# steventan0110/DiffNorm

Measured on AMD Instinct MI355X. Metric: denoising-steps/sec (BxT latents), higher is better.
Workload: dtype f16; 1 GPU; configs[2]: DDIM/DDPM-schedule reverse chain, eps-predictor Model(512, z=128) on [B=32,T=512] latents per GPU, 1000-step cosine schedule, random-init weights; batch_per_gpu=32, frames=512, latent_dim=128, hip_graph=True, half_batch_streams=2, parallelism=batch-sharded x1 (no collective)

## Files before the change

### diffnorm_amd/_lib.py

```python
import ctypes as C
import os

_HERE = os.path.dirname(os.path.abspath(__file__))
LIB_PATH = os.path.join(_HERE, "libdiffnorm_hip.so")

DN_F32, DN_BF16, DN_BF16X3, DN_F16 = 0, 1, 2, 3
EPI_BIAS, EPI_SILU, EPI_GEGLU, EPI_FILM_GATE, EPI_RESADD, EPI_POSEMB, EPI_RELU = range(7)
DN_MAX_TERMS = 8
TAG_FFN_CONV, TAG_WN_DILATED, TAG_FFN_CONV_WGRAD = 1, 2, 3
GEMM_NARROW_STORES, GEMM_NO_RES_PREFETCH, GEMM_RELU, GEMM_TWIN = 1 << 4, 1 << 5, 1 << 6, 1 << 7
GEMM_TAG_SHIFT, GEMM_TILE_SHIFT, GEMM_BAND_SHIFT = 8, 16, 24
GEMM_FAT_STAMPS, GEMM_NO_SHARED_ROWS, GEMM_TAPS_INNER, GEMM_TERM_OUTER = 1 << 20, 1 << 21, 1 << 22, 1 << 23
(TILE_128X128, TILE_256X128, TILE_256X256, TILE_256X352, TILE_ROW, TILE_256X256_W4, TILE_256X256_W8, TILE_256X192,
 TILE_256X128_2WG) = range(1, 10)


class DiffNormHipError(RuntimeError):
    pass


LAYOUT_A_KBLOCKED, LAYOUT_W_KBLOCKED, LAYOUT_OUT_KBLOCKED = 1, 2, 1


class GemmTerm(C.Structure):
    _fields_ = [("A", C.c_void_p), ("W", C.c_void_p), ("lda", C.c_int32), ("shift", C.c_int32),
                ("a_gstride", C.c_int64), ("w_gstride", C.c_int64), ("shift_by_group", C.c_int32),
                ("layout", C.c_int32), ("ldw", C.c_int32), ("pad_ldw_", C.c_int32)]


class GemmParams(C.Structure):
    _fields_ = [("terms", GemmTerm * DN_MAX_TERMS), ("n_terms", C.c_int32), ("dtype", C.c_int32),
                ("M", C.c_int32), ("N", C.c_int32), ("K", C.c_int32), ("T", C.c_int32),
                ("groups", C.c_int32), ("epilogue", C.c_int32), ("bias", C.c_void_p),
                ("bias_gstride", C.c_int64), ("out", C.c_void_p), ("ldo", C.c_int32),
                ("out_dtype", C.c_int32), ("out_gstride", C.c_int64), ("res", C.c_void_p),
                ("ldr", C.c_int32), ("res_dtype", C.c_int32), ("res_gstride", C.c_int64),
                ("gamma_beta", C.c_void_p), ("gb_ld", C.c_int32), ("gb_half", C.c_int32),
                ("gb_gstride", C.c_int64), ("pos_table", C.c_void_p), ("pos_ld", C.c_int32),
                ("flags", C.c_int32), ("lengths", C.c_void_p),
                ("norm_out", C.c_void_p), ("norm_ld", C.c_int32), ("norm_dtype", C.c_int32), ("norm_D", C.c_int32),
                ("norm_gb_ld", C.c_int32), ("norm_gamma", C.c_void_p), ("norm_gb", C.c_void_p),
                ("norm_gb_half", C.c_int32), ("out_layout", C.c_int32),
                ("norm_split", C.c_int32), ("norm_ssq_ld", C.c_int32), ("norm_ssq", C.c_void_p),
                ("row_ssq", C.c_void_p), ("row_ssq_ld", C.c_int32), ("row_ssq_parts", C.c_int32),
                ("row_D", C.c_float), ("row_bias_ld", C.c_int32), ("row_bias", C.c_void_p),
                ("pre_out", C.c_void_p), ("pre_ld", C.c_int32), ("pre_pad_", C.c_int32)]
    pad_ = property(lambda self: self.flags, lambda self, v: setattr(self, "flags", v))


class GemmRoute(C.Structure):
    _fields_ = [(n, C.c_int32) for n in ("tile", "taps_inner", "shared_rows", "band")]


class AdamParams(C.Structure):
    _fields_ = [("lr", C.c_double), ("beta1", C.c_double), ("beta2", C.c_double), ("eps", C.c_double),
                ("weight_decay", C.c_double), ("max_norm", C.c_double), ("step", C.c_int32), ("pad_", C.c_int32),
                ("grad_scale", C.c_double), ("grad_scale_dev", C.c_void_p)]


class AttnParams(C.Structure):
    _fields_ = [("q", C.c_void_p), ("k", C.c_void_p), ("v", C.c_void_p), ("out", C.c_void_p),
                ("ldq", C.c_int32), ("ldk", C.c_int32), ("ldv", C.c_int32), ("ldo", C.c_int32),
                ("B", C.c_int32), ("T", C.c_int32), ("heads", C.c_int32), ("dim_head", C.c_int32),
                ("dtype", C.c_int32), ("Tk", C.c_int32), ("lengths", C.c_void_p),
                ("scale", C.c_float), ("pad2_", C.c_int32), ("lse", C.c_void_p),
                ("dropout_p", C.c_float), ("seed_lo", C.c_uint32), ("seed_hi", C.c_uint32), ("pad3_", C.c_int32)]


class AttnBwdParams(C.Structure):
    _fields_ = [(n, C.c_void_p) for n in ("q", "k", "v", "out", "dout", "dq", "dk", "dv")] + \
               [(n, C.c_int32) for n in ("ldq", "ldk", "ldv", "ldo", "lddo", "lddq", "lddk", "lddv", "B", "T", "heads", "dim_head",
                                         "dtype", "pad_")] + \
               [("lengths", C.c_void_p), ("scale", C.c_float), ("pad2_", C.c_int32), ("lse", C.c_void_p), ("delta", C.c_void_p),
                ("dropout_p", C.c_float), ("seed_lo", C.c_uint32), ("seed_hi", C.c_uint32), ("pad3_", C.c_int32)]


class GaussianStep(C.Structure):
    _fields_ = [("x", C.c_void_p), ("model_out", C.c_void_p), ("noise", C.c_void_p), ("sample", C.c_void_p),
                ("pred_xstart", C.c_void_p), ("t", C.c_void_p), ("table", C.c_void_p), ("N", C.c_int32),
                ("inner", C.c_int32), ("learned_range", C.c_int32), ("clip_denoised", C.c_int32), ("sampler", C.c_int32),
                ("eta", C.c_float), ("predict_xstart", C.c_int32), ("cond_grad", C.c_void_p)]


GD_COLS = 12
DDIM_SCHED_COLS = 5
DPM_COLS = 6


class GaussianMoments(C.Structure):
    _fields_ = [(n, C.c_void_p) for n in ("x", "model_out", "x_start", "t", "table", "mean", "variance", "log_variance", "pred_xstart",
                                          "vb", "reverse_sample")] + [(n, C.c_int32) for n in ("N", "inner", "learned_range", "clip_denoised", "predict_xstart")]


class EpsConfig(C.Structure):
    _fields_ = [(n, C.c_int32) for n in ("dim", "latent", "depth", "heads", "dim_head", "wn_layers",
                                         "wn_stacks", "cond_mult", "dtype", "max_pos", "dim_prompt", "num_latents", "resampler_depth")]

# ... 57 lines not shown
                ("label_smoothing", C.c_float), ("loss_scale", C.c_float), ("stats", C.c_void_p), ("logits_out", C.c_void_p),
                ("recon_out", C.c_void_p), ("ext_dlogits", C.c_void_p), ("attn_dropout", C.c_float),
                ("dropout_seed_lo", C.c_uint32), ("dropout_seed_hi", C.c_uint32), ("pad_", C.c_int32)]


class EpsTrainBatch(C.Structure):
    _fields_ = [(n, C.c_void_p) for n in ("feat", "units", "lengths", "z", "jitter", "true_noise", "times", "sqrt_ac", "sqrt_1mac",
                                          "snr_weight")] + \
               [("beta0", C.c_float), ("B", C.c_int32), ("T", C.c_int32), ("n_units", C.c_int32), ("n_frames", C.c_int32),
                ("timesteps", C.c_int32), ("multitask", C.c_int32), ("label_smoothing", C.c_float), ("recon_weight", C.c_float),
                ("loss_scale", C.c_float), ("stats", C.c_void_p), ("eps_out", C.c_void_p), ("attn_dropout", C.c_float),
                ("dropout_seed_lo", C.c_uint32), ("dropout_seed_hi", C.c_uint32), ("pad_", C.c_int32)]


REPACK_CONVERT, REPACK_KBLOCK, REPACK_COPY, REPACK_SUM = range(4)


class RepackDesc(C.Structure):
    _fields_ = [("src", C.c_int64), ("dst", C.c_void_p), ("kind", C.c_int32), ("mats", C.c_int32), ("rows", C.c_int32), ("K", C.c_int32),
                ("count", C.c_int32), ("pad_", C.c_int32), ("stride", C.c_int64)]


_vp, _i32, _i64, _u64, _sz = C.c_void_p, C.c_int32, C.c_int64, C.c_uint64, C.c_size_t
SYMBOLS = {
    "dn_conv_gemm": (C.c_int, [C.POINTER(GemmParams), _vp]),
    "dn_conv_gemm_route": (C.c_int, [C.POINTER(GemmParams), C.POINTER(GemmRoute)]),
    "dn_conv_gemm_kblocked_ok": (C.c_int, [C.POINTER(GemmParams)]),
    "dn_conv_gemm_tile": (C.c_int, [C.POINTER(GemmParams)]),
    "dn_grad_sumsq": (C.c_int, [_vp, C.c_int64, _vp, _vp, C.c_int32, _vp]),
    "dn_transpose_pad": (C.c_int, [_vp, C.c_int32, C.c_int32, C.c_int32, C.c_int32, C.c_int32, C.c_int32, _vp, C.c_int32, C.c_int32,
                                   C.c_int32, C.c_int32, _vp]),
    "dn_adam_step": (C.c_int, [_vp, _vp, _vp, _vp, C.c_int64, C.POINTER(AdamParams), _vp, _vp, _vp]),
    "dn_adam_step_ema": (C.c_int, [_vp, _vp, _vp, _vp, C.c_int64, C.POINTER(AdamParams), _vp, _vp, _vp, C.c_double, _vp]),
    "dn_ema_update": (C.c_int, [_vp, _vp, C.c_int64, C.c_double, _vp]),
    "dn_profile_start": (C.c_int, [_i32, _i32]),
    "dn_profile_stop": (C.c_int, [C.POINTER(C.c_float), C.POINTER(_i32)]),
    "dn_attention": (C.c_int, [C.POINTER(AttnParams), _vp]),
    "dn_attention_backward": (C.c_int, [C.POINTER(AttnBwdParams), _vp]),
    "dn_time_cond_backward": (C.c_int, [_vp, _i32, _vp, _i32, _vp, _vp, _i32, _vp, _i32, _vp, _vp, _vp, _vp, _vp]),
    "dn_gate_forward": (C.c_int, [_vp, _vp, _vp, _i32, _i32, _i32, _i32, _vp, _i32, _i32, _vp]),
    "dn_gate_backward": (C.c_int, [_vp, _vp, _vp, _i32, _i32, _i32, _i32, _vp, _i32, _i32, _vp, _i32, _vp]),
    "dn_geglu_forward": (C.c_int, [_vp, _vp, _i32, _i32, _i32, _vp]),
    "dn_geglu_backward": (C.c_int, [_vp, _vp, _vp, _i32, _i32, _i32, _vp]),
    "dn_rmsnorm_backward_scratch_bytes": (_sz, [_i32, _i32, _i32]),
    "dn_rmsnorm_backward": (C.c_int, [_vp, _i32, _vp, _i32, _i32, _i32, _i32, _i32, _vp, _vp, _i32, _i32, _vp, _vp, _vp, _i32, _i32,
                                      _vp, _vp, _i32, _vp, _vp]),
    "dn_colsum_scratch_bytes": (_sz, [_i32, _i32, _i32]),
    "dn_colsum": (C.c_int, [_vp, _i32, _i32, _i32, _i32, _i32, _vp, _i32, C.c_float, _i32, _vp, _vp]),
    "dn_posterior_backward": (C.c_int, [_vp, _i32, _vp, _i32, _vp, _i32, _vp, _i32, _i32, _i32, _i32, _i32, _vp, C.c_float, _vp]),
    "dn_lsce_loss_grad": (C.c_int, [_vp, _i32, _vp, _i32, _i32, C.c_float, C.c_float, _vp, _vp, _i32, _i32, _vp]),
    "dn_masked_mse_grad": (C.c_int, [_vp, _i32, _vp, _i32, _i32, _i32, _i32, _vp, C.c_float, _vp, _vp, _i32, _i32, _vp, _i32, _i32, _vp]),
    "dn_vec_sum": (C.c_int, [_vp, _i64, _vp, _i32, _vp, _vp]),
    "dn_vae_train_create": (C.c_int, [C.POINTER(VaeConfig), C.POINTER(_vp)]),
    "dn_vae_train_destroy": (None, [_vp]),
    "dn_vae_train_param_count": (_i64, [_vp]),
    "dn_vae_train_aux_bytes": (_sz, [_vp]),
    "dn_vae_train_offsets": (C.c_int, [_vp, C.POINTER(_i64), _i32]),
    "dn_vae_train_stage_range": (C.c_int, [_vp, _i32, C.POINTER(_i64), C.POINTER(_i64)]),
    "dn_vae_train_bind": (C.c_int, [_vp, _vp, _vp, _vp, _vp]),
    "dn_vae_train_refresh": (C.c_int, [_vp, _vp]),
    "dn_vae_train_workspace_bytes": (_sz, [_vp, _i32, _i32]),
    "dn_vae_train_forward": (C.c_int, [_vp, C.POINTER(VaeTrainBatch), _vp, _sz, _vp]),
    "dn_vae_train_backward": (C.c_int, [_vp, C.POINTER(VaeTrainBatch), _i32, _i32, _vp, _sz, _vp]),
    "dn_cmlm_step": (C.c_int, [_vp, _vp, _vp, _vp, _i32, _i32, _i32, _i32, _i32, _i32, _i32, _vp]),
    "dn_eps_train_create": (C.c_int, [C.POINTER(EpsConfig), C.POINTER(_vp)]),
    "dn_eps_train_destroy": (None, [_vp]),
    "dn_eps_train_param_count": (_i64, [_vp]),
    "dn_eps_train_aux_bytes": (_sz, [_vp]),
    "dn_eps_train_offsets": (C.c_int, [_vp, C.POINTER(_i64), _i32]),
    "dn_eps_train_stage_range": (C.c_int, [_vp, _i32, C.POINTER(_i64), C.POINTER(_i64)]),
    "dn_eps_train_bind": (C.c_int, [_vp, _vp, _vp, _vp, _vp, _vp]),
    "dn_eps_train_refresh": (C.c_int, [_vp, _vp]),
    "dn_eps_train_workspace_bytes": (_sz, [_vp, _vp, _i32, _i32]),
    "dn_eps_train_forward": (C.c_int, [_vp, _vp, C.POINTER(EpsTrainBatch), _vp, _sz, _vp]),
    "dn_eps_train_backward": (C.c_int, [_vp, _vp, C.POINTER(EpsTrainBatch), _i32, _i32, _vp, _sz, _vp]),
    "dn_sum_groups": (C.c_int, [_vp, _i64, _i32, _vp, _i32, _i64, _vp]),
    "dn_rows_times_weight_scratch_bytes": (_sz, [_i32, _i32, _i32]),
    "dn_rows_times_weight": (C.c_int, [_vp, _i32, _i32, _vp, _i32, _i32, _i32, _vp, _vp, _vp]),
    "dn_transpose_weights": (C.c_int, [_vp, _i32, _i32, _i64, _i32, _i32, _vp, _i64, _i32, _i32, _vp]),
    "dn_split_rows": (C.c_int, [_vp, _i64, _vp, _i32, _vp]),
    "dn_transpose_slices": (C.c_int, [_vp, _i32, _i32, _i32, _i32, _i32, _i32, _i32, _i64, _i32, _vp, _i32, _i32, _i32, _i32, _vp]),
    "dn_repack_weights": (C.c_int, [_vp, _vp, _i32, _i32, _vp]),
    "dn_ffn_fold": (C.c_int, [_vp, _vp, _vp, _vp, C.c_int64, C.c_int64, C.c_int64, C.c_int64, _i32, _i32, _i32, _i32, _vp, _vp, _vp]),
    "dn_eps_set_ffn_fold": (C.c_int, [_vp, _vp, _vp]),
    "dn_vae_set_ffn_fold": (C.c_int, [_vp, _vp, _vp]),
    "dn_wgrad_reduce": (C.c_int, [_vp, _i32, _i32, _i32, _i32, _i32, _vp, _i32, _i32, _vp]),
    "dn_conv_weight_grad_tn": (C.c_int, [_vp, _i32, _i32, _vp, _vp, _vp, _i32, _i32, _i32, _i32, _i32, _vp, _vp, _vp]),
    "dn_conv_weight_grad_tn_x3": (C.c_int, [_vp, _i32, _i32, _vp, _vp, _vp, _i32, _i32, _i32, _i32, _i32, _vp, _vp, _vp]),
    "dn_add_broadcast": (C.c_int, [_vp, _vp, _i32, _i32, _i32, _vp]),
    "dn_transpose_pad_f32": (C.c_int, [_vp, _i32, _i32, _i32, _i32, _i32, _i32, _vp, _i32, _i32, _i32, _i32, _vp]),
    "dn_rmsnorm": (C.c_int, [_vp, _i32, _vp, _i32, _i32, _i32, _i32, _i32, _vp, _vp, _i32, _i32, _vp]),
    "dn_time_cond": (C.c_int, [_vp, _i32, _vp, _i32, _vp, _vp, _i32, _vp, _vp, _i32, _i32, _vp]),
    "dn_ddim_step": (C.c_int, [_vp, _vp, _vp, _vp, _i32, _i32, _i32, _i32, _i32, _i32, _vp, _vp, _vp]),
    "dn_q_sample": (C.c_int, [_vp, _vp, _vp, _vp, _i32, _i32, _i32, _i32, _i32, _i32, _vp, _vp, _vp, _vp]),
    "dn_gaussian_step": (C.c_int, [C.POINTER(GaussianStep), _vp]),
    "dn_gaussian_moments": (C.c_int, [C.POINTER(GaussianMoments), _vp]),
    "dn_posterior_sample": (C.c_int, [_vp, _i32, _vp, _i32, _vp, _vp, _i32, _i32, _i32, _i32, _i32, _vp, _vp, _vp]),
    "dn_argmax_units": (C.c_int, [_vp, _i32, _i32, _i32, _i32, _vp, _vp]),
    "dn_randn": (C.c_int, [_vp, _i64, _u64, _u64, _vp]),
    "dn_randn_keyed": (C.c_int, [_vp, _vp, _i32, _i32, _i32, C.c_uint32, _vp]),
    "dn_chain_start": (C.c_int, [_vp, _i32, _vp, _i32, _i32, _i32, _vp, _vp, _vp, _vp, _vp, _vp]),
    "dn_convert_rows": (C.c_int, [_vp, _i32, _i32, _vp, _i32, _i32, _i32, _i32, _vp]),
    "dn_eps_create": (C.c_int, [C.POINTER(EpsConfig), C.POINTER(_vp), _i32, C.POINTER(_vp)]),
    "dn_eps_destroy": (None, [_vp]),
    "dn_eps_workspace_bytes": (_sz, [_vp, _i32, _i32]),
    "dn_eps_forward": (C.c_int, [_vp, _vp, _vp, _vp, _i32, _i32, _i32, _vp, _vp, _sz, _vp]),
    "dn_eps_cond_workspace_bytes": (_sz, [_vp, _i32, _i32, _i32]),
    "dn_eps_forward_cond": (C.c_int, [_vp, _vp, _vp, _vp, _vp, _vp, _vp, _i32, _i32, _i32, _vp, _vp, _sz, _vp]),
    "dn_eps_forward_cond_ex": (C.c_int, [_vp, _vp, _vp, _vp, _vp, _vp, _vp, _i32, _i32, _i32, _vp, _vp, _sz, _i32, _vp, _i32, _i32, _vp]),
    "dn_eps_cond_time_table_workspace_bytes": (_sz, [_vp, _i32]),
    "dn_eps_cond_time_table": (C.c_int, [_vp, _i32, _i32, _vp, _vp, _sz, _vp]),
    "dn_eps_cond_time_table_steps": (C.c_int, [_vp, _vp, _i32, _vp, _vp, _sz, _vp]),
    "dn_eps_weights_changed": (C.c_int, [_vp]),
    "dn_vae_create": (C.c_int, [C.POINTER(VaeConfig), C.POINTER(_vp), _i32, C.POINTER(_vp)]),
    "dn_vae_destroy": (None, [_vp]),
    "dn_vae_workspace_bytes": (_sz, [_vp, _i32, _i32]),
    "dn_vae_encode_params": (C.c_int, [_vp, _vp, _i32, _i32, _vp, _vp, _sz, _vp]),
    "dn_vae_decode": (C.c_int, [_vp, _vp, _vp, _i32, _i32, _vp, _vp, _vp, _vp, _sz, _vp]),
    "dn_ddim_workspace_bytes": (_sz, [_vp, _i32, _i32, _i32]),
    "dn_ddim_loop": (C.c_int, [_vp, _vp, _vp, _i32, _i32, _i32, _i32, _vp, _i32, _i32, _vp, _sz, _vp]),
    "dn_ddpm_loop": (C.c_int, [_vp, _vp, _vp, _i32, _i32, _i32, _i32, _vp, _i32, _i32, C.c_uint64, _vp, _i32, _vp, _sz, _vp]),
    "dn_ddim_sched_workspace_bytes": (_sz, [_vp, _i32, _i32, _i32]),
    "dn_ddim_sched_check": (C.c_int, [_vp, _i32, _i32]),
    "dn_ddim_sched_loop": (C.c_int, [_vp, _vp, _vp, _i32, _i32, _vp, _vp, _i32, _i32, _i32, C.c_uint64, _vp, _i32, _vp, _sz, _vp]),
    "dn_dpm2m_step": (C.c_int, [_vp, _vp, _vp, _i64, _vp, _vp, _vp]),
    "dn_ddim_sched_step": (C.c_int, [_vp, _vp, _i64, _vp, _vp, _vp, _i32, C.c_uint64, _vp, _vp]),
    "dn_ddim_sched_step_keyed": (C.c_int, [_vp, _vp, _vp, _i32, _i32, _i32, _vp, _vp, _vp, _vp]),
    "dn_ddim_sched_loop_keyed": (C.c_int, [_vp, _vp, _vp, _i32, _i32, _vp, _vp, _i32, _i32, _vp, _i32, _vp, _sz, _vp]),
    "dn_ddpm_loop_keyed": (C.c_int, [_vp, _vp, _vp, _i32, _i32, _i32, _i32, _vp, _i32, _i32, _vp, _i32, _vp, _sz, _vp]),
    "dn_guided_ddim_loop_keyed": (C.c_int, [_vp, _vp, _vp, _vp, _vp, _i32, _i32, _i32, C.c_float, _vp, _vp, _i32, _i32, _vp, _i32, _vp, _sz,
                                            _vp]),
    "dn_dpm_workspace_bytes": (_sz, [_vp, _i32, _i32, _i32]),
    "dn_dpm_loop": (C.c_int, [_vp, _vp, _vp, _i32, _i32, _vp, _vp, _i32, _i32, _i32, _vp, _sz, _vp]),
    "dn_gaussian_workspace_bytes": (_sz, [_vp, _i32, _i32, _i32]),
    "dn_gaussian_loop": (C.c_int, [_vp, _vp, _vp, _i32, _i32, _vp, _vp, _i32, _i32, _i32, _i32, C.c_float, C.c_uint64, _vp, _i32, _vp, _sz,
                                   _vp]),
    "dn_gaussian_loop_keyed": (C.c_int, [_vp, _vp, _vp, _i32, _i32, _vp, _vp, _i32, _i32, _i32, _i32, C.c_float, _vp, _i32, _vp, _sz, _vp]),
    "dn_gaussian_sched_step": (C.c_int, [_vp, _vp, _i64, _vp, _vp, _i32, _i32, _i32, C.c_float, C.c_uint64, _vp, _vp]),
    "dn_gaussian_sched_step_keyed": (C.c_int, [_vp, _vp, _vp, _i32, _i32, _i32, _vp, _vp, _vp, _i32, _i32, _i32, C.c_float, _vp]),
    "dn_guided_ddim_workspace_bytes": (_sz, [_vp, _i32, _i32, _i32, _i32, _i32]),
    "dn_guided_ddim_loop": (C.c_int, [_vp, _vp, _vp, _vp, _vp, _i32, _i32, _i32, C.c_float, _vp, _vp, _i32, _i32, _i32, C.c_uint64, _vp, _i32,
                                      _vp, _sz, _vp]),
    "dn_guided_dpm_workspace_bytes": (_sz, [_vp, _i32, _i32, _i32, _i32, _i32]),
    "dn_guided_dpm_loop": (C.c_int, [_vp, _vp, _vp, _vp, _vp, _i32, _i32, _i32, C.c_float, _vp, _vp, _i32, _i32, _i32, _vp, _sz, _vp]),
    "dn_cfg_combine": (C.c_int, [_vp, C.c_float, _i64, _vp, _vp]),
    "dn_nar_create": (C.c_int, [C.POINTER(NarConfig), C.POINTER(_vp), _i32, C.POINTER(_vp)]),
    "dn_nar_destroy": (None, [_vp]),
    "dn_nar_workspace_bytes": (_sz, [_vp, _i32, _i32, _i32]),
    "dn_nar_cross_kv_bytes": (_sz, [_vp, _i32, _i32]),
    "dn_nar_cross_kv": (C.c_int, [_vp, _vp, _i32, _i32, _vp, _vp, _sz, _vp]),
    "dn_nar_predict_lengths": (C.c_int, [_vp, _vp, _vp, _i32, _i32, _vp, _vp, _sz, _vp]),
    "dn_nar_decoder_forward": (C.c_int, [_vp, _vp, _vp, _vp, _i32, _i32, _i32, _vp, _vp, _sz, _vp]),
    "dn_nar_encoder_create": (C.c_int, [_vp, _vp, _i32, _vp]),
    "dn_nar_encoder_destroy": (None, [_vp]),
    "dn_nar_encoder_out_frames": (_i32, [_i32]),
    "dn_nar_encoder_workspace_bytes": (_sz, [_vp, _i32, _i32]),
    "dn_nar_encoder_forward": (C.c_int, [_vp, _vp, _vp, _i32, _i32, _vp, _vp, _vp, _sz, _vp]),
    "dn_rel_attention": (C.c_int, [C.POINTER(RelAttnParams), _vp]),
    "dn_glu_dwconv": (C.c_int, [_vp, _vp, _vp, _vp, _i32, _i32, _i32, _i32, _i32, _vp]),
    "dn_conformer_encoder_create": (C.c_int, [_vp, _vp, _i32, _vp]),
    "dn_conformer_encoder_destroy": (None, [_vp]),
    "dn_conformer_encoder_workspace_bytes": (_sz, [_vp, _i32, _i32]),
    "dn_conformer_encoder_forward": (C.c_int, [_vp, _vp, _vp, _i32, _i32, _vp, _vp, _vp, _sz, _vp]),
    "dn_last_error": (C.c_char_p, []),
    "dn_version": (C.c_int, []),
    "dn_cmlm_step_dev": (C.c_int, [_vp, _vp, _vp, _vp, _i32, _i32, _i32, _vp, _i32, _i32, _i32, _vp]),
    "dn_nar_null_cross_bytes": (_sz, [_vp]),
    "dn_nar_null_cross": (C.c_int, [_vp, _i32, _vp, _sz, _vp]),
# ... 102 lines not shown
```

### diffnorm_amd/csrc/engine.h

```cpp
#pragma once
#include <stddef.h>
#include <stdint.h>
#include <string.h>

#include "../../include/diffnorm_hip.h"

namespace dn {

inline int round_up(int x, int m) { return (x + m - 1) / m * m; }
inline int padk(int c) { return round_up(c, 64); }
inline int padn(int c) { return round_up(c, 128); }

inline const void* eoff(const void* p, size_t elems, int es) { return static_cast<const char*>(p) + elems * es; }
inline void* eoff(void* p, size_t elems, int es) { return static_cast<char*>(p) + elems * es; }
inline int esize(int dtype) { return dtype == DN_BF16 || dtype == DN_F16 ? 2 : 4; }
inline int side_dtype(int dtype) { return dtype == DN_BF16X3 ? DN_F32 : dtype; }
inline int ew_grid(int64_t n) {
  const int64_t b = (n + 255) / 256;
  return (int)(b > 4096 ? 4096 : b);
}

#define DN_TRY(expr)          \
  do {                        \
    int rc__ = (expr);        \
    if (rc__ != DN_OK) return rc__; \
  } while (0)

inline DnGemmParams gemm_base(int dtype, int M, int N, int K, int T, int32_t flags = 0) {
  DnGemmParams p;
  memset(&p, 0, sizeof(p));
  p.flags = flags;
  p.dtype = dtype;
  p.M = M; p.N = N; p.K = K; p.T = T;
  p.groups = 1;
  p.n_terms = 1;
  p.epilogue = DN_EPI_BIAS;
  p.out_dtype = dtype;
  p.res_dtype = dtype == DN_BF16X3 ? DN_F32 : dtype;
  return p;
}

struct Arena {
  char* base;
  size_t off, cap;
  void* take(size_t bytes) {
    size_t a = (off + 255) & ~size_t(255);
    off = a + bytes;
    if (!base) return reinterpret_cast<void*>(a + 256);
    return off <= cap ? base + a : nullptr;
  }
};

struct WavenetW {
  int cin, cout, stacks, layers;
  const void *init_W, *conv_W, *res_W, *skip_W, *final_W, *conv_Wkb, *res_Wkb;
  const float *init_b, *conv_b, *res_b, *skip_b, *final_b;
};
constexpr int kWavenetTensors = 12;

struct TransformerW {
  int dim, depth, heads, dim_head, inner;
  const void *qkv_W, *out_W, *ffin_W, *ffconv_W, *ffout_W, *pred_W, *ffconv_Wkb, *ffin_Wkb, *qkv_Wkb;
  const float *ffin_b, *ffconv_b, *ffout_b, *g1, *g2, *pred_gamma;
  const void* fold_W;
  const float* fold_b;
  int fold_default;
};
constexpr int kTransformerTensors = 15;

struct WgTnGroups {
  int groups;
  int64_t dy_gstride, x_gstride, grad_gstride;
  int shift_by_group;
};
int wgrad_tn_launch(const void* dy, int lddy, int cout, const void* const* x, const int* ldx, const int* shift, int n_taps, int cin, int B, int T,
                    int slices, float* part, float* grad, void* stream, int tag, const WgTnGroups* grp);
constexpr int WGRAD_TN_X3_DEFAULT = 1;
int wgrad_tn_x3_launch(const void* dy, int lddy, int cout, const void* const* x, const int* ldx, const int* shift, int n_taps, int cin, int B, int T,
                       int slices, float* part, float* grad, void* stream, int tag, const WgTnGroups* grp);

struct StepKey {
  const void *ws, *x, *len, *coef;
  const void *prompt, *plen;
  const void* keys;
  uint64_t seed;
  int32_t B, T, Tp, n_steps;
  int32_t flags;
  int32_t opt_gen;
  uint32_t scale_bits;
  uint32_t eta_bits;
  uint16_t ancestral, clip, scheduled, eta, dpm;
  uint16_t generic;
  uint16_t injected;
  uint16_t reserved;
};
static_assert(sizeof(StepKey) == 7 * sizeof(void*) + 8 + 8 * 4 + 8 * 2, "StepKey has no padding: copies of a key compare equal too");
struct StepGraph {
  void* exec;
  StepKey key;
};

struct SchedNoise {
  const float* noise;
  int64_t noise_row;
  uint64_t seed;
  const uint64_t* keys;
  int64_t row_quads;
};
inline SchedNoise sched_noise(const float* noise, int64_t noise_row, uint64_t seed, const uint64_t* keys, int64_t row_quads) {
  return keys ? SchedNoise{nullptr, 0, 0, keys, row_quads} : SchedNoise{noise, noise_row, seed, nullptr, 0};
}
enum SchedRule { SCHED_DDIM, SCHED_DPM2M, SCHED_GAUSSIAN };
struct SchedStep {
  int rule;
  float* x;
  int64_t elem0, n_elem;
  const float* eps;
  int guided;
  float scale;
  float* xin;
  const float* coef;
  const int32_t *steps, *counter;
  int eta_on;
  float* hist;
  int n_steps, sampler, clip;
  float eta;
  SchedNoise src;
};
int sched_step_launch(const char* who, const SchedStep& d, void* stream);

}

int dn_ddpm_step_launch(float* x, const float* eps, int M, int C, int T, const float* table, const int32_t* t, int clip, const float* noise,
                        int64_t noise_row, int t_top, uint64_t seed, const uint64_t* keys, int b0, void* stream);
int dn_gaussian_sched_args(const char* who, int32_t n_steps, int32_t sampler, float eta);

struct DnEps {
  DnEpsConfig cfg;
  const float *w_freq, *tc_W, *tc_b, *cond_b, *init_b, *final_b, *pos_table;
  const void *cond_W, *init_W, *final_W;
  dn::WavenetW wn;
  dn::TransformerW tf;
  int n_cond;
  int n_row;
  const float *tpc_W, *tpc_b, *null_pc, *lat_pos, *rffin_b, *rffout_b, *rnorm_g, *proj_b;
  const void *null_tok, *proj_W, *rq_W, *rkv_W, *rout_W, *rffin_W, *rffout_W, *cq_W, *ckv_W, *cout_W;
  dn::StepGraph loop_graph, guided_graph;
// ... 16 lines not shown
```

### diffnorm_amd/csrc/engine.hip

```cpp
#include <algorithm>
#include <functional>
#include <new>
#include <stdlib.h>
#include <string.h>

#include "common.h"
#include "engine.h"

using namespace dn;

namespace {

inline bool fuse_norm_enabled(int Dp, int dtype) {
  const bool on = option_or(OPT_FUSE_NORM, 0) != 0;
  return on && Dp <= 512 && dtype != DN_BF16X3;
}

inline bool split_norm_enabled(int Dp, int dtype) {
  return option_or(OPT_NO_SPLIT_NORM, 0) == 0 && Dp % 64 == 0 && !fuse_norm_enabled(Dp, dtype);
}

int kblock_mode() {
  const int v = option(OPT_KBLOCK);
  return v == DN_OPT_UNSET ? -1 : (v != 0 ? 1 : 0);
// ... 14 lines not shown

int run_wavenet(const WavenetW& w, int dtype, const void* in, int M, int T, const float* gb, int gb_ld, const WaveBufs& wb,
                DnGemmParams fin, hipStream_t s, int32_t gemm_flags = 0) {
  const int es = esize(dtype);
  const int cinp = padk(w.cin), cp = padk(w.cout), cn = padn(w.cout), L = w.layers, S = w.stacks;
  const size_t mat = (size_t)cn * cp;
  const int64_t plane = (int64_t)M * cp;
  bool kb = false;
  if (kblock_mode() != 0 && dn::dn_is16(dtype) && w.conv_Wkb && w.res_Wkb) {
    DnGemmParams q = gemm_base(dtype, M, cp, cp, T, gemm_flags);
    q.groups = L;
    const int t_res = dn_conv_gemm_tile(&q);
    q.n_terms = 3; q.epilogue = DN_EPI_FILM_GATE;
    kb = kblock_mode() == 1 || (t_res == DN_TILE_256X256 && dn_conv_gemm_tile(&q) == DN_TILE_256X256);
  }
  const int a_layout = kb ? (DN_LAYOUT_A_KBLOCKED | DN_LAYOUT_W_KBLOCKED) : 0;
  {
    DnGemmParams p = gemm_base(dtype, M, cp, cinp, T, gemm_flags);
    p.n_terms = 3;
    for (int j = 0; j < 3; ++j) {
      p.terms[j].A = in; p.terms[j].lda = cinp; p.terms[j].shift = 2 - j;
      p.terms[j].W = eoff(w.init_W, (size_t)j * cn * cinp, es);
    }
    p.bias = w.init_b; p.out = wb.hw; p.ldo = cp;
    p.out_layout = kb ? DN_LAYOUT_OUT_KBLOCKED : 0;
    DN_TRY(dn_conv_gemm(&p, s));
  }
  for (int st = 0; st < S; ++st) {
    const void* in_s = st == 0 ? wb.hw : ((st - 1) & 1 ? wb.blk1 : wb.blk0);
    const int64_t a_gs = st == 0 ? 0 : plane;
    void* out_s = (st & 1) ? wb.blk1 : wb.blk0;
    {
      DnGemmParams p = gemm_base(dtype, M, cp, cp, T, gemm_flags);
      p.groups = L;
      p.terms[0].A = in_s; p.terms[0].lda = cp; p.terms[0].a_gstride = a_gs;
      p.terms[0].W = eoff(kb ? w.res_Wkb : w.res_W, (size_t)st * L * mat, es); p.terms[0].w_gstride = (int64_t)mat;
      p.terms[0].layout = a_layout;
      p.bias = w.res_b + (size_t)st * L * cp; p.bias_gstride = cp;
      p.out = wb.resb; p.ldo = cp; p.out_gstride = plane; p.out_dtype = side_dtype(dtype);
      DN_TRY(dn_conv_gemm(&p, s));
    }
    {
      DnGemmParams p = gemm_base(dtype, M, cp, cp, T, gemm_flags);
      p.groups = L;
      p.n_terms = 3;
      for (int j = 0; j < 3; ++j) {
        p.terms[j].A = in_s; p.terms[j].lda = cp; p.terms[j].a_gstride = a_gs;
        p.terms[j].shift = 2 - j; p.terms[j].shift_by_group = 1;
        p.terms[j].W = eoff(kb ? w.conv_Wkb : w.conv_W, ((size_t)st * L * 3 + j) * mat, es); p.terms[j].w_gstride = (int64_t)(3 * mat);
        p.terms[j].layout = a_layout;
      }
      p.bias = w.conv_b + (size_t)st * L * cp; p.bias_gstride = cp;
      p.epilogue = DN_EPI_FILM_GATE;
      p.res = wb.resb; p.ldr = cp; p.res_gstride = plane; p.res_dtype = side_dtype(dtype);
      if (gb) {
        p.gamma_beta = gb + (size_t)st * L * 2 * cp; p.gb_ld = gb_ld; p.gb_half = cp; p.gb_gstride = 2 * cp;
      }
      p.out = out_s; p.ldo = cp; p.out_gstride = plane;
      p.out_layout = kb && st + 1 < S ? DN_LAYOUT_OUT_KBLOCKED : 0;
      p.flags |= DN_TAG_WN_DILATED << DN_GEMM_TAG_SHIFT;
      DN_TRY(dn_conv_gemm(&p, s));
    }
  }
  const void* last = ((S - 1) & 1) ? wb.blk1 : wb.blk0;
  {
    DnGemmParams p = gemm_base(dtype, M, cp, cp, T, gemm_flags);
    p.n_terms = L;
    for (int i = 0; i < L; ++i) {
      p.terms[i].A = eoff(last, (size_t)i * plane, es); p.terms[i].lda = cp;
      p.terms[i].W = eoff(w.skip_W, (size_t)i * mat, es);
    }
    p.bias = w.skip_b; p.out = wb.sk; p.ldo = cp;
    DN_TRY(dn_conv_gemm(&p, s));
  }
  fin.dtype = dtype; fin.M = M; fin.K = cp; fin.T = T; fin.groups = 1; fin.n_terms = 1; fin.flags |= gemm_flags;
  fin.terms[0].A = wb.sk; fin.terms[0].lda = cp; fin.terms[0].W = w.final_W;
  fin.bias = w.final_b;
  return dn_conv_gemm(&fin, s);
}

struct TfBufs { void *xn, *qkv, *ao, *gg, *fc; float* ssq; };
inline int ssq_ld(int Dp) { const int n = Dp / 64; return n <= 8 ? 8 : (n + 3) / 4 * 4; }

inline int ffn_fold_mode(const TransformerW& w) { return w.fold_W && w.fold_b ? option_or(OPT_FFN_FOLD, w.fold_default) : 0; }

TfBufs plan_tf(const TransformerW& w, int M, int es, Arena& ar) {
  const int hd = w.heads * w.dim_head;
  TfBufs b;
  b.xn = ar.take((size_t)M * padk(w.dim) * es);
  b.qkv = ar.take((size_t)M * 3 * hd * es);
  b.ao = ar.take((size_t)M * hd * es);
  b.gg = ar.take((size_t)M * padk(w.inner) * es);
  b.fc = ffn_fold_mode(w) ? nullptr : ar.take((size_t)M * padk(w.inner) * es);
  b.ssq = (float*)ar.take((size_t)M * ssq_ld(padk(w.dim)) * 4);
  return b;
}

void set_split_norm(DnGemmParams& p, const TfBufs& tb, int Dp, int D, int dtype, const float* gamma, const float* gb, int gb_ld) {
  p.norm_out = tb.xn; p.norm_ld = Dp; p.norm_dtype = dtype; p.norm_D = D;
  p.norm_gamma = gamma; p.norm_gb = gb; p.norm_gb_ld = gb_ld; p.norm_gb_half = Dp;
  p.norm_split = 1; p.norm_ssq = tb.ssq; p.norm_ssq_ld = ssq_ld(Dp);
}
void set_row_scale(DnGemmParams& p, const TfBufs& tb, int Dp, int D, const float* rb, int rb_ld) {
  p.row_ssq = tb.ssq; p.row_ssq_ld = ssq_ld(Dp); p.row_ssq_parts = Dp / 64; p.row_D = (float)D;
  p.row_bias = rb; p.row_bias_ld = rb_ld;
}

void set_norm(DnGemmParams& p, void* xn, int Dp, int D, int dtype, const float* gamma, const float* gb, int gb_ld) {
  p.norm_out = xn; p.norm_ld = Dp; p.norm_dtype = dtype; p.norm_D = D;
  p.norm_gamma = gamma; p.norm_gb = gb; p.norm_gb_ld = gb_ld; p.norm_gb_half = Dp;
}

struct NormSrc { const float* gamma; const float* gb; };
NormSrc norm_src(const TransformerW& w, const float* gb, int l, int j, int nj = 2) {
  const int D = w.dim, Dp = padk(D);
  if (l == w.depth) return {w.pred_gamma, nullptr};
  const float* g = j == 0 ? w.g1 : w.g2;
  return {g ? g + (size_t)l * D : nullptr, gb ? gb + (size_t)(nj * l + j) * 2 * Dp : nullptr};
}

struct CrossAttn { const void* q_W; const void* out_W; const void* kv; int n_kv; void* q; };

int run_transformer(const TransformerW& w, int dtype, float* xres, int B, int T, const int32_t* lengths, const float* gb, int gb_ld,
                    const float* rb, int rb_ld, const TfBufs& tb, void* pred, int pred_ld, int pred_dtype, bool xn_ready, hipStream_t s,
                    const CrossAttn* cx = nullptr, int32_t gemm_flags = 0) {
  const int es = esize(dtype), M = B * T;
  const int D = w.dim, Dp = padk(D), Dn = padn(D), hd = w.heads * w.dim_head, ip = padk(w.inner), in_n = padn(w.inner);
  const bool fuse = fuse_norm_enabled(Dp, dtype);
  const bool split = split_norm_enabled(Dp, dtype);
  const int nj = cx ? 3 : 2, rb_layer = 3 * hd + (cx ? hd : 0) + 2 * ip;
  bool scaled = split && xn_ready;
  auto standalone_norm = [&](int l, int j) -> int {
    const NormSrc ns = norm_src(w, gb, l, j, nj);
    return dn_rmsnorm(xres, Dp, tb.xn, Dp, dtype, M, D, T, ns.gamma, ns.gb, gb_ld, Dp, s);
  };
  if (!((fuse || split) && xn_ready)) DN_TRY(standalone_norm(0, 0));
  const int mid2 = dn::dn_is16(dtype) && M >= 2048 ? option_or(OPT_MID2, 0) : 0;
  bool geglu_kb = false;
  static const bool geglu_kb_off = getenv("DN_GEGLU_KB") && atoi(getenv("DN_GEGLU_KB")) == 0;
  if (!geglu_kb_off && split && !fuse && kblock_mode() != 0 && dn::dn_is16(dtype) && w.ffin_Wkb && Dp % 32 == 0) {
    DnGemmParams q = gemm_base(dtype, M, ip, Dp, T, gemm_flags);
    q.epilogue = DN_EPI_GEGLU;
    if (mid2 & 2) q.flags |= DN_TILE_256X128_2WG << DN_GEMM_TILE_SHIFT;
    const int gt = dn_conv_gemm_tile(&q);
    geglu_kb = kblock_mode() == 1 || gt == DN_TILE_256X256 || gt == DN_TILE_256X128_2WG;
  }
  bool qkv_kb = false;
  static const bool qkv_kb_off = getenv("DN_QKV_KB") && atoi(getenv("DN_QKV_KB")) == 0;
  if (!qkv_kb_off && split && !fuse && kblock_mode() != 0 && dn::dn_is16(dtype) && w.qkv_Wkb && Dp % 32 == 0) {
    DnGemmParams q = gemm_base(dtype, M, 3 * hd, Dp, T, gemm_flags);
    if (mid2 & 1) q.flags |= DN_TILE_256X128_2WG << DN_GEMM_TILE_SHIFT;
    const int qt = dn_conv_gemm_tile(&q);
    qkv_kb = kblock_mode() == 1 || qt == DN_TILE_256X256 || qt == DN_TILE_256X128_2WG;
  }
  const int fold = ffn_fold_mode(w);
  const bool qkv_192 = option_or(OPT_QKV_192, 0) != 0 && dn::dn_is16(dtype) && (3 * hd) % 192 == 0 && M >= 2048;
  for (int l = 0; l < w.depth; ++l) {
    {
      DnGemmParams p = gemm_base(dtype, M, 3 * hd, Dp, T, gemm_flags);
      p.terms[0].A = tb.xn; p.terms[0].lda = Dp; p.terms[0].W = eoff(w.qkv_W, (size_t)l * padn(3 * hd) * Dp, es);
      if (qkv_kb && l >= 1) {
        p.terms[0].W = eoff(w.qkv_Wkb, (size_t)l * padn(3 * hd) * Dp, es);
        p.terms[0].layout = DN_LAYOUT_A_KBLOCKED | DN_LAYOUT_W_KBLOCKED;
      }
      p.out = tb.qkv; p.ldo = 3 * hd; p.out_dtype = side_dtype(dtype);
      if (qkv_192) p.flags |= DN_TILE_256X192 << DN_GEMM_TILE_SHIFT;
      else if (mid2 & 1) p.flags |= DN_TILE_256X128_2WG << DN_GEMM_TILE_SHIFT;
      if (scaled) set_row_scale(p, tb, Dp, D, rb ? rb + (size_t)l * rb_layer : nullptr, rb_ld);
      DN_TRY(dn_conv_gemm(&p, s));
    }
    {
      DnAttnParams a;
      memset(&a, 0, sizeof(a));
      a.q = tb.qkv; a.k = eoff(tb.qkv, hd, es); a.v = eoff(tb.qkv, 2 * hd, es); a.out = tb.ao;
      a.ldq = a.ldk = a.ldv = 3 * hd; a.ldo = hd;
      a.B = B; a.T = T; a.heads = w.heads; a.dim_head = w.dim_head; a.dtype = dtype; a.lengths = lengths;
      a.scale = 1.0f / sqrtf((float)w.dim_head);
      DN_TRY(dn_attention(&a, s));
    }
    {
      DnGemmParams p = gemm_base(dtype, M, Dp, hd, T, gemm_flags);
      p.terms[0].A = tb.ao; p.terms[0].lda = hd; p.terms[0].W = eoff(w.out_W, (size_t)l * Dn * hd, es);
      p.epilogue = DN_EPI_RESADD; p.res = xres; p.ldr = Dp; p.out = xres; p.ldo = Dp; p.out_dtype = DN_F32;
      const NormSrc ns = norm_src(w, gb, l, 1, nj);
      if (fuse) set_norm(p, tb.xn, Dp, D, dtype, ns.gamma, ns.gb, gb_ld);
      else if (split) set_split_norm(p, tb, Dp, D, dtype, ns.gamma, ns.gb, gb_ld);
      if (geglu_kb && !cx) p.norm_split = 2;
      DN_TRY(dn_conv_gemm(&p, s));
    }
    if (!fuse && !split) DN_TRY(standalone_norm(l, 1));
    scaled = split;
    if (cx) {
      {
        DnGemmParams p = gemm_base(dtype, M, hd, Dp, T, gemm_flags);
        p.terms[0].A = tb.xn; p.terms[0].lda = Dp; p.terms[0].W = eoff(cx->q_W, (size_t)l * padn(hd) * Dp, es);
        p.out = cx->q; p.ldo = hd; p.out_dtype = side_dtype(dtype);
        if (scaled) set_row_scale(p, tb, Dp, D, rb ? rb + (size_t)l * rb_layer + 3 * hd : nullptr, rb_ld);
        DN_TRY(dn_conv_gemm(&p, s));
      }
      {
        const void* kv = eoff(cx->kv, (size_t)l * B * cx->n_kv * 2 * hd, esize(side_dtype(dtype)));
        DnAttnParams a;
        memset(&a, 0, sizeof(a));
        a.q = cx->q; a.k = kv; a.v = eoff(kv, hd, esize(side_dtype(dtype))); a.out = tb.ao;
        a.ldq = hd; a.ldk = a.ldv = 2 * hd; a.ldo = hd;
        a.B = B; a.T = T; a.Tk = cx->n_kv; a.heads = w.heads; a.dim_head = w.dim_head; a.dtype = dtype; a.lengths = nullptr;
        a.scale = 1.0f / sqrtf((float)w.dim_head);
        DN_TRY(dn_attention(&a, s));
      }
      {
        DnGemmParams p = gemm_base(dtype, M, Dp, hd, T, gemm_flags);
        p.terms[0].A = tb.ao; p.terms[0].lda = hd; p.terms[0].W = eoff(cx->out_W, (size_t)l * Dn * hd, es);
        p.epilogue = DN_EPI_RESADD; p.res = xres; p.ldr = Dp; p.out = xres; p.ldo = Dp; p.out_dtype = DN_F32;
        const NormSrc ns = norm_src(w, gb, l, 2, nj);
        if (fuse) set_norm(p, tb.xn, Dp, D, dtype, ns.gamma, ns.gb, gb_ld);
        else if (split) set_split_norm(p, tb, Dp, D, dtype, ns.gamma, ns.gb, gb_ld);
        if (geglu_kb) p.norm_split = 2;
        DN_TRY(dn_conv_gemm(&p, s));
      }
      if (!fuse && !split) DN_TRY(standalone_norm(l, 2));
    }
    auto close_residual = [&](DnGemmParams& p) -> int {
      p.epilogue = DN_EPI_RESADD; p.res = xres; p.ldr = Dp; p.out = xres; p.ldo = Dp; p.out_dtype = DN_F32;
      const NormSrc ns = norm_src(w, gb, l + 1, 0, nj);
      if (fuse) set_norm(p, tb.xn, Dp, D, dtype, ns.gamma, ns.gb, gb_ld);
      else if (split) set_split_norm(p, tb, Dp, D, dtype, ns.gamma, ns.gb, gb_ld);
      if (qkv_kb && l + 1 < w.depth) p.norm_split = 2;
      return dn_conv_gemm(&p, s);
    };
    if (fold) {
      {
        DnGemmParams p = gemm_base(dtype, M, ip, Dp, T, gemm_flags);
        p.terms[0].A = tb.xn; p.terms[0].lda = Dp; p.terms[0].W = eoff(w.ffin_W, (size_t)l * 2 * ip * Dp, es);
        if (geglu_kb) {
          p.terms[0].W = eoff(w.ffin_Wkb, (size_t)l * 2 * ip * Dp, es);
          p.terms[0].layout = DN_LAYOUT_A_KBLOCKED | DN_LAYOUT_W_KBLOCKED;
        }
        p.bias = w.ffin_b + (size_t)l * 2 * ip;
        p.epilogue = DN_EPI_GEGLU; p.out = tb.gg; p.ldo = ip;
        if (mid2 & 2) p.flags |= DN_TILE_256X128_2WG << DN_GEMM_TILE_SHIFT;
        if (scaled) set_row_scale(p, tb, Dp, D, rb ? rb + (size_t)l * rb_layer + 3 * hd + (cx ? hd : 0) : nullptr, rb_ld);
        DN_TRY(dn_conv_gemm(&p, s));
      }
      DnGemmParams p = gemm_base(dtype, M, Dp, ip, T, gemm_flags);
      p.n_terms = 3;
      for (int j = 0; j < 3; ++j) {
        p.terms[j].A = tb.gg; p.terms[j].lda = ip; p.terms[j].shift = 2 - j;
        p.terms[j].W = eoff(w.fold_W, ((size_t)l * 3 + j) * Dn * ip, es);
      }
      p.bias = w.fold_b + (size_t)l * Dp;
      p.flags |= DN_TAG_FFN_CONV << DN_GEMM_TAG_SHIFT;
      const int fold_tile = fold == 2 ? DN_TILE_256X128 : fold == 3 ? DN_TILE_256X256 : 0;
      if (fold_tile && !fuse) p.flags |= fold_tile << DN_GEMM_TILE_SHIFT;
      DN_TRY(close_residual(p));
    } else {
    DnGemmParams pc = gemm_base(dtype, M, ip, ip, T, gemm_flags);
    pc.n_terms = 3;
    for (int j = 0; j < 3; ++j) {
      pc.terms[j].A = tb.gg; pc.terms[j].lda = ip; pc.terms[j].shift = 2 - j;
      pc.terms[j].W = eoff(w.ffconv_W, ((size_t)l * 3 + j) * in_n * ip, es);
    }
    pc.bias = w.ffconv_b + (size_t)l * ip; pc.out = tb.fc; pc.ldo = ip;
    pc.flags |= DN_TAG_FFN_CONV << DN_GEMM_TAG_SHIFT;
    const int conv_tile = dn_conv_gemm_tile(&pc);
    const bool kblocked = kblock_mode() != 0 && dn::dn_is16(dtype) && w.ffconv_Wkb &&
                          (kblock_mode() == 1 || conv_tile == DN_TILE_256X352 || conv_tile == DN_TILE_256X256);
    if (kblocked)
      for (int j = 0; j < 3; ++j) {
        pc.terms[j].W = eoff(w.ffconv_Wkb, ((size_t)l * 3 + j) * in_n * ip, es);
        pc.terms[j].layout = DN_LAYOUT_A_KBLOCKED | DN_LAYOUT_W_KBLOCKED;
      }
    {
      DnGemmParams p = gemm_base(dtype, M, ip, Dp, T, gemm_flags);
      p.terms[0].A = tb.xn; p.terms[0].lda = Dp; p.terms[0].W = eoff(w.ffin_W, (size_t)l * 2 * ip * Dp, es);
      if (geglu_kb) {
        p.terms[0].W = eoff(w.ffin_Wkb, (size_t)l * 2 * ip * Dp, es);
        p.terms[0].layout = DN_LAYOUT_A_KBLOCKED | DN_LAYOUT_W_KBLOCKED;
      }
      p.bias = w.ffin_b + (size_t)l * 2 * ip;
      p.epilogue = DN_EPI_GEGLU; p.out = tb.gg; p.ldo = ip;
      if (mid2 & 2) p.flags |= DN_TILE_256X128_2WG << DN_GEMM_TILE_SHIFT;
      p.out_layout = kblocked ? DN_LAYOUT_OUT_KBLOCKED : 0;
      if (scaled) set_row_scale(p, tb, Dp, D, rb ? rb + (size_t)l * rb_layer + 3 * hd + (cx ? hd : 0) : nullptr, rb_ld);
      DN_TRY(dn_conv_gemm(&p, s));
    }
    DN_TRY(dn_conv_gemm(&pc, s));
    {
      DnGemmParams p = gemm_base(dtype, M, Dp, ip, T, gemm_flags);
      p.terms[0].A = tb.fc; p.terms[0].lda = ip; p.terms[0].W = eoff(w.ffout_W, (size_t)l * Dn * ip, es);
      p.bias = w.ffout_b + (size_t)l * Dp;
      DN_TRY(close_residual(p));
    }
    }
    if (!fuse && !split) DN_TRY(standalone_norm(l + 1, 0));
  }
  DnGemmParams p = gemm_base(dtype, M, Dp, Dp, T, gemm_flags);
  p.terms[0].A = tb.xn; p.terms[0].lda = Dp; p.terms[0].W = w.pred_W;
  p.out = pred; p.ldo = pred_ld; p.out_dtype = pred_dtype;
  if (pred_ld < Dp) p.N = pred_ld;
  if (split) set_row_scale(p, tb, Dp, D, nullptr, 0);
  return dn_conv_gemm(&p, s);
}

const void* const* take_wavenet(WavenetW& w, const void* const* t) {
  w.init_W = t[0]; w.init_b = (const float*)t[1]; w.conv_W = t[2]; w.conv_b = (const float*)t[3];
  w.res_W = t[4]; w.res_b = (const float*)t[5]; w.skip_W = t[6]; w.skip_b = (const float*)t[7];
  w.final_W = t[8]; w.final_b = (const float*)t[9];
  w.conv_Wkb = t[10]; w.res_Wkb = t[11];
  return t + kWavenetTensors;
}

const void* const* take_transformer(TransformerW& w, const void* const* t) {
  w.qkv_W = t[0]; w.out_W = t[1]; w.ffin_W = t[2]; w.ffin_b = (const float*)t[3]; w.ffconv_W = t[4];
  w.ffconv_b = (const float*)t[5]; w.ffout_W = t[6]; w.ffout_b = (const float*)t[7];
  w.g1 = (const float*)t[8]; w.g2 = (const float*)t[9]; w.pred_gamma = (const float*)t[10]; w.pred_W = t[11];
  w.ffconv_Wkb = t[12]; w.ffin_Wkb = t[13]; w.qkv_Wkb = t[14];
  return t + kTransformerTensors;
}

int check_dims(const char* who, int dtype, int dim, int heads, int dim_head, int layers) {
  DN_CHECK_ARG(dtype == DN_F32 || dtype == DN_BF16 || dtype == DN_BF16X3 || dtype == DN_F16, "%s: bad dtype %d", who, dtype);
  DN_CHECK_ARG(dim > 0 && dim % 4 == 0, "%s: dim=%d must be a positive multiple of 4", who, dim);
  DN_CHECK_ARG((heads * dim_head) % 64 == 0, "%s: heads*dim_head=%d must be a multiple of 64", who, heads * dim_head);
  DN_CHECK_ARG(layers >= 1 && layers <= DN_MAX_TERMS, "%s: wavenet layers=%d must be in 1..%d", who, layers, DN_MAX_TERMS);
  return DN_OK;
}

struct EpsBufs {
  float *cond, *gb, *xres;
  void *xin, *h0, *tp, *gbh;
  WaveBufs wv;
  TfBufs tf;
};

EpsBufs plan_eps(const DnEps* m, int B, int T, int Bt, Arena& ar) {
  const int es = esize(m->cfg.dtype), M = B * T;
  const int C = m->cfg.dim * m->cfg.cond_mult, Dp = padk(m->cfg.dim), zp = padk(m->cfg.latent);
  EpsBufs b;
  b.cond = (float*)ar.take((size_t)Bt * C * 4);
  b.gb = (float*)ar.take((size_t)Bt * m->n_row * 4);
  b.gbh = m->cfg.dtype == DN_F32 ? nullptr : ar.take((size_t)Bt * m->n_cond * es);
  b.xin = ar.take((size_t)M * zp * es);
  b.h0 = ar.take((size_t)M * Dp * es);
  b.wv = plan_wave(m->wn, M, es, ar);
  b.xres = (float*)ar.take((size_t)M * Dp * 4);
  b.tf = plan_tf(m->tf, M, es, ar);
  b.tp = ar.take((size_t)M * Dp * es);
  return b;
}

__global__ void fill_t_kernel(int32_t* t, int n, const int32_t* counter) {
  const int i = blockIdx.x * 256 + threadIdx.x;
  if (i < n) t[i] = *counter;
}
__global__ void set_counter_kernel(int32_t* counter, int v) { *counter = v; }
__global__ void dec_counter_kernel(int32_t* counter) { *counter -= 1; }
__global__ void inc_counter_kernel(int32_t* counter) { *counter += 1; }

}

extern "C" int dn_eps_create(const DnEpsConfig* cfg, const void* const* weights, int32_t n_weights, DnEps** out) {
  DN_CHECK_ARG(cfg && weights && out, "dn_eps_create: null argument");
  const bool cond_model = cfg->dim_prompt > 0;
  const int expect_tensors = kEpsTensors + (cond_model ? kEpsCondTensors : 0);
  DN_CHECK_ARG(n_weights == expect_tensors, "dn_eps_create: expected %d packed tensors, got %d", expect_tensors, n_weights);
  DN_CHECK_ARG(!cond_model || (cfg->dim_prompt % 4 == 0 && cfg->num_latents >= 1 && cfg->resampler_depth >= 1),
               "dn_eps_create: conditional model needs dim_prompt %% 4 == 0, num_latents >= 1, resampler_depth >= 1");
  DN_TRY(check_dims("dn_eps_create", cfg->dtype, cfg->dim, cfg->heads, cfg->dim_head, cfg->wn_layers));
  DN_CHECK_ARG(cfg->dim % 2 == 0 && (cfg->dim * cfg->cond_mult) % 64 == 0, "dn_eps_create: dim*cond_mult must be a multiple of 64");
  DN_CHECK_ARG(cfg->latent % 4 == 0 && cfg->latent > 0, "dn_eps_create: latent=%d must be a multiple of 4", cfg->latent);
  for (int i = 0; i < n_weights; ++i) DN_CHECK_ARG(weights[i] != nullptr, "dn_eps_create: packed tensor %d is null", i);
  DnEps* m = new (std::nothrow) DnEps();
  DN_CHECK_ARG(m != nullptr, "dn_eps_create: out of host memory");
  memset(m, 0, sizeof(*m));
  m->cfg = *cfg;
  const void* const* t = weights;
  m->w_freq = (const float*)t[0]; m->tc_W = (const float*)t[1]; m->tc_b = (const float*)t[2];
  m->cond_W = t[3]; m->cond_b = (const float*)t[4]; m->init_W = t[5]; m->init_b = (const float*)t[6];
  t += 7;
  m->wn.cin = m->wn.cout = cfg->dim; m->wn.stacks = cfg->wn_stacks; m->wn.layers = cfg->wn_layers;
  t = take_wavenet(m->wn, t);
  m->tf.dim = cfg->dim; m->tf.depth = cfg->depth; m->tf.heads = cfg->heads; m->tf.dim_head = cfg->dim_head;
  m->tf.inner = (int)((double)cfg->dim * 4 * 2 / 3);
  t = take_transformer(m->tf, t);
  m->tf.g1 = m->tf.g2 = nullptr;
  m->final_W = t[0]; m->final_b = (const float*)t[1]; m->pos_table = (const float*)t[2];
  m->n_cond = (cfg->wn_stacks * cfg->wn_layers + (cond_model ? 3 : 2) * cfg->depth) * 2 * padk(cfg->dim);
  m->n_row = m->n_cond + cfg->depth * (3 * cfg->heads * cfg->dim_head + 2 * padk(m->tf.inner));
  if (cond_model) {
    const void* const* c = t + 3;
    m->tpc_W = (const float*)c[0]; m->tpc_b = (const float*)c[1]; m->null_pc = (const float*)c[2]; m->null_tok = c[3];
    m->proj_W = c[4]; m->proj_b = (const float*)c[5]; m->lat_pos = (const float*)c[6];
    m->rq_W = c[7]; m->rkv_W = c[8]; m->rout_W = c[9]; m->rffin_W = c[10]; m->rffin_b = (const float*)c[11];
    m->rffout_W = c[12]; m->rffout_b = (const float*)c[13]; m->rnorm_g = (const float*)c[14];
    m->cq_W = c[15]; m->ckv_W = c[16]; m->cout_W = c[17];
  }
  *out = m;
  return DN_OK;
}

extern "C" int dn_eps_set_ffn_fold(DnEps* m, const void* fold_W, const float* fold_b) {
  DN_CHECK_ARG(m && (fold_W != nullptr) == (fold_b != nullptr), "dn_eps_set_ffn_fold: null engine, or one of the two buffers without the other");
  DN_CHECK_ARG(((uintptr_t)fold_W & 127) == 0 && ((uintptr_t)fold_b & 15) == 0, "dn_eps_set_ffn_fold: fold_W 128-byte, fold_b 16-byte aligned");
  m->tf.fold_W = fold_W; m->tf.fold_b = fold_b;
  m->tf.fold_default = m->cfg.dtype == DN_BF16 ? 0 : 1;
  for (StepGraph* g : {&m->loop_graph, &m->guided_graph}) {
    if (g->exec) (void)hipGraphExecDestroy((hipGraphExec_t)g->exec);
    g->exec = nullptr;
  }
  m->table_ws = nullptr;
  return DN_OK;
}

extern "C" void dn_eps_destroy(DnEps* m) {
  if (!m) return;
  for (StepGraph* g : {&m->loop_graph, &m->guided_graph})
    if (g->exec) (void)hipGraphExecDestroy((hipGraphExec_t)g->exec);
  if (m->ev_fork) (void)hipEventDestroy((hipEvent_t)m->ev_fork);
  if (m->ev_join) (void)hipEventDestroy((hipEvent_t)m->ev_join);
  if (m->side_stream) (void)hipStreamDestroy((hipStream_t)m->side_stream);
  delete m;
}

static size_t eps_ws_core(const DnEps* m, int B, int T) {
  Arena ar{nullptr, 0, 0};
  (void)plan_eps(m, B, T, B, ar);
  return ar.off + 256;
}

extern "C" size_t dn_eps_workspace_bytes(const DnEps* m, int32_t B, int32_t T) {
  if (!m || B <= 0 || T <= 0) return 0;
  return eps_ws_core(m, B, T);
}

namespace {

int eps_beta_rows(const DnEps* m, const float* gb, int gb_ld, int n, void* gbh, float* rb, int rb_ld, hipStream_t s) {
  const int Dp = padk(m->cfg.dim), dtype = m->cfg.dtype, es = esize(dtype);
  const TransformerW& w = m->tf;
  const bool cx = m->cfg.dim_prompt > 0;
  const int hd = w.heads * w.dim_head, ip = padk(w.inner), nj = cx ? 3 : 2, rb_layer = 3 * hd + (cx ? hd : 0) + 2 * ip;
  const size_t tf_off = (size_t)m->cfg.wn_stacks * m->cfg.wn_layers * 2 * Dp;
  const void* A = gb;
  int lda = gb_ld;
  if (dtype != DN_F32) {
    DN_TRY(dn_convert_rows(gb, DN_F32, gb_ld, gbh, dtype, m->n_cond, n, m->n_cond, s));
    A = gbh; lda = m->n_cond;
  }
  int col = 0;
  for (int j = 0; j < nj; ++j) {
    const bool last = j == nj - 1;
    const int N = j == 0 ? 3 * hd : (last ? 2 * ip : hd);
    DnGemmParams q = gemm_base(dtype, n, N, Dp, 1);
    q.groups = w.depth;
    q.terms[0].A = eoff(A, tf_off + (size_t)j * 2 * Dp + Dp, es); q.terms[0].lda = lda; q.terms[0].a_gstride = (int64_t)nj * 2 * Dp;
    q.terms[0].W = j == 0 ? w.qkv_W : (last ? w.ffin_W : m->cq_W);
    q.terms[0].w_gstride = j == 0 ? (int64_t)padn(3 * hd) * Dp : (last ? (int64_t)2 * ip * Dp : (int64_t)padn(hd) * Dp);
    q.out = rb + col; q.ldo = rb_ld; q.out_dtype = DN_F32; q.out_gstride = rb_layer;
    DN_TRY(dn_conv_gemm(&q, s));
    col += N;
  }
  return DN_OK;
}

int eps_cond_rows(const DnEps* m, const int32_t* times, int n, float* cond, float* gb, void* gbh, hipStream_t s) {
  const int D = m->cfg.dim, C = D * m->cfg.cond_mult, Dp = padk(D), dtype = m->cfg.dtype, es = esize(dtype);
  DN_TRY(dn_time_cond(times, n, m->w_freq, D / 2, m->tc_W, m->tc_b, C, cond, nullptr, DN_F32, C, s));
  DnGemmParams p = gemm_base(DN_F32, n, m->n_cond, C, 1);
  p.terms[0].A = cond; p.terms[0].lda = C; p.terms[0].W = m->cond_W;
  p.bias = m->cond_b; p.out = gb; p.ldo = m->n_row; p.out_dtype = DN_F32;
  DN_TRY(dn_conv_gemm(&p, s));
  if (!split_norm_enabled(Dp, dtype)) return DN_OK;
  return eps_beta_rows(m, gb, m->n_row, n, gbh, gb + m->n_cond, m->n_row, s);
}

int eps_core(const DnEps* m, const float* x, const float* gb, int gb_ld, const int32_t* lengths, int B, int T, float* eps_out,
             const EpsBufs& b, hipStream_t s, int32_t gemm_flags = 0) {
  const DnEpsConfig& c = m->cfg;
  const int dtype = c.dtype, M = B * T;
  const int D = c.dim, Dp = padk(D), z = c.latent, zp = padk(z);
  DN_TRY(dn_convert_rows(x, DN_F32, z, b.xin, dtype, zp, M, z, s));
  {
    DnGemmParams p = gemm_base(dtype, M, Dp, zp, T, gemm_flags);
    p.terms[0].A = b.xin; p.terms[0].lda = zp; p.terms[0].W = m->init_W;
    p.bias = m->init_b; p.out = b.h0; p.ldo = Dp;
    DN_TRY(dn_conv_gemm(&p, s));
  }
  {
    DnGemmParams fin = gemm_base(dtype, M, Dp, Dp, T, gemm_flags);
    fin.epilogue = DN_EPI_POSEMB; fin.pos_table = m->pos_table; fin.pos_ld = Dp; fin.lengths = lengths;
    fin.out = b.xres; fin.ldo = Dp; fin.out_dtype = DN_F32;
    const float* gb0 = gb + (size_t)c.wn_stacks * c.wn_layers * 2 * Dp;
    if (fuse_norm_enabled(Dp, dtype)) set_norm(fin, b.tf.xn, Dp, D, dtype, nullptr, gb0, gb_ld);
// ... 867 lines not shown
  };
  return guided_loop(m, x, lengths, prompt, prompt_lengths, B, T, Tp, cond_scale, steps, coef, n_steps, timesteps, flags, workspace,
                     workspace_bytes, stream, d);
}

extern "C" int dn_guided_ddim_loop(DnEps* m, float* x, const int32_t* lengths, const float* prompt, const int32_t* prompt_lengths, int32_t B,
                                   int32_t T, int32_t Tp, float cond_scale, const int32_t* steps, const float* coef, int32_t n_steps,
                                   int32_t timesteps, int32_t eta_on, uint64_t seed, const float* noise, int32_t flags, void* workspace,
                                   size_t workspace_bytes, void* stream) {
  return guided_ddim_loop("dn_guided_ddim_loop", m, x, lengths, prompt, prompt_lengths, B, T, Tp, cond_scale, steps, coef, n_steps, timesteps,
                          eta_on, seed, noise, nullptr, flags, workspace, workspace_bytes, stream);
}

extern "C" int dn_guided_ddim_loop_keyed(DnEps* m, float* x, const int32_t* lengths, const float* prompt, const int32_t* prompt_lengths,
                                         int32_t B, int32_t T, int32_t Tp, float cond_scale, const int32_t* steps, const float* coef,
                                         int32_t n_steps, int32_t timesteps, const uint64_t* keys, int32_t flags, void* workspace,
                                         size_t workspace_bytes, void* stream) {
  DN_TRY(check_keys("dn_guided_ddim_loop_keyed", m, keys));
  return guided_ddim_loop("dn_guided_ddim_loop_keyed", m, x, lengths, prompt, prompt_lengths, B, T, Tp, cond_scale, steps, coef, n_steps,
                          timesteps, 1, 0, nullptr, keys, flags, workspace, workspace_bytes, stream);
}

extern "C" size_t dn_guided_dpm_workspace_bytes(const DnEps* m, int32_t B, int32_t T, int32_t Tp, int32_t n_steps, int32_t guided) {
  return guided_ws_bytes(m, B, T, Tp, n_steps, guided, true, DN_DPM_COLS);
}

extern "C" int dn_guided_dpm_loop(DnEps* m, float* x, const int32_t* lengths, const float* prompt, const int32_t* prompt_lengths, int32_t B,
                                  int32_t T, int32_t Tp, float cond_scale, const int32_t* steps, const float* coef, int32_t n_steps,
                                  int32_t timesteps, int32_t flags, void* workspace, size_t workspace_bytes, void* stream) {
  GuidedDesc d = {"dn_guided_dpm_loop", "dn_guided_dpm_workspace_bytes", "dn_dpm_loop", DN_DPM_COLS, true, step_kind(0, nullptr), nullptr};
  d.kind.dpm = 1;
  d.update = [](const GuidedBufs& g, float* xb, float* xin, int64_t n_elem, int guided, float scale, hipStream_t st) {
    SchedStep u = {SCHED_DPM2M, xb, 0, n_elem, g.both, guided, scale, xin};
    u.coef = g.coef; u.counter = g.counter; u.hist = g.hist;
    return sched_step_launch("dn_guided_dpm_loop", u, st);
  };
  return guided_loop(m, x, lengths, prompt, prompt_lengths, B, T, Tp, cond_scale, steps, coef, n_steps, timesteps, flags, workspace,
                     workspace_bytes, stream, d);
}

extern "C" int dn_vae_create(const DnVaeConfig* cfg, const void* const* weights, int32_t n_weights, DnVae** out) {
  DN_CHECK_ARG(cfg && weights && out, "dn_vae_create: null argument");
  DN_CHECK_ARG(cfg->n_mults >= 1 && cfg->n_mults <= 4, "dn_vae_create: n_mults=%d", cfg->n_mults);
  const int expect = 2 * cfg->n_mults * kWavenetTensors + kTransformerTensors + 2;
  DN_CHECK_ARG(n_weights == expect, "dn_vae_create: expected %d packed tensors, got %d", expect, n_weights);
  DN_TRY(check_dims("dn_vae_create", cfg->dtype, cfg->dim, cfg->heads, cfg->dim_head, cfg->layers));
  DN_CHECK_ARG(cfg->vocab % 4 == 0 && cfg->z % 4 == 0, "dn_vae_create: vocab and z must be multiples of 4");
  for (int i = 0; i < n_weights; ++i) DN_CHECK_ARG(weights[i] != nullptr, "dn_vae_create: packed tensor %d is null", i);
  DnVae* m = new (std::nothrow) DnVae();
  DN_CHECK_ARG(m != nullptr, "dn_vae_create: out of host memory");
  memset(m, 0, sizeof(*m));
  m->cfg = *cfg;
  m->n_wave = cfg->n_mults;
  const void* const* t = weights;
  int cur = cfg->dim;
  for (int n = 0; n < m->n_wave; ++n) {
    WavenetW& w = m->enc[n];
    w.cin = cur; w.cout = cur / cfg->mults[n]; w.stacks = cfg->stacks; w.layers = cfg->layers;
    cur = w.cout;
    t = take_wavenet(w, t);
  }
  DN_CHECK_ARG(cur == 2 * cfg->z, "dn_vae_create: encoder width %d != 2*z (%d)", cur, 2 * cfg->z);
  for (int n = 0; n < m->n_wave; ++n) {
    WavenetW& w = m->dec[n];
    const int mult = cfg->mults[m->n_wave - 1 - n];
    w.cout = cur * mult; w.cin = n == 0 ? cur / 2 : cur; w.stacks = cfg->stacks; w.layers = cfg->layers;
    cur = w.cout;
    t = take_wavenet(w, t);
  }
  DN_CHECK_ARG(cur == cfg->dim, "dn_vae_create: decoder width %d != dim %d", cur, cfg->dim);
  m->tf.dim = cfg->dim; m->tf.depth = cfg->depth; m->tf.heads = cfg->heads; m->tf.dim_head = cfg->dim_head;
  m->tf.inner = (int)((double)cfg->dim * 4 * 2 / 3);
  t = take_transformer(m->tf, t);
  m->lm_W = t[0]; m->lm_b = (const float*)t[1];
  *out = m;
  return DN_OK;
}

extern "C" void dn_vae_destroy(DnVae* m) { delete m; }

extern "C" int dn_vae_set_ffn_fold(DnVae* m, const void* fold_W, const float* fold_b) {
  DN_CHECK_ARG(m && (fold_W != nullptr) == (fold_b != nullptr), "dn_vae_set_ffn_fold: null engine, or one of the two buffers without the other");
  DN_CHECK_ARG(((uintptr_t)fold_W & 127) == 0 && ((uintptr_t)fold_b & 15) == 0, "dn_vae_set_ffn_fold: fold_W 128-byte, fold_b 16-byte aligned");
  m->tf.fold_W = fold_W; m->tf.fold_b = fold_b;
  m->tf.fold_default = m->cfg.dtype == DN_BF16 ? 0 : 1;
  return DN_OK;
}

namespace {
struct VaeBufs {
  void *in_act, *mid[2];
  WaveBufs wv[4];
  float *xres, *recon, *logits;
  void* pred_act;
  TfBufs tf;
};

VaeBufs plan_vae_enc(const DnVae* m, int M, Arena& ar) {
  const int es = esize(m->cfg.dtype);
  VaeBufs b;
  memset(&b, 0, sizeof(b));
  b.in_act = ar.take((size_t)M * padk(m->cfg.dim) * es);
  int widest = 0;
  for (int n = 0; n < m->n_wave; ++n) widest = widest > m->enc[n].cout ? widest : m->enc[n].cout;
  b.mid[0] = ar.take((size_t)M * padk(widest) * es);
  b.mid[1] = ar.take((size_t)M * padk(widest) * es);
  for (int n = 0; n < m->n_wave; ++n) b.wv[n] = plan_wave(m->enc[n], M, es, ar);
  return b;
}

VaeBufs plan_vae_dec(const DnVae* m, int M, bool need_recon, bool need_logits, Arena& ar) {
  const int es = esize(m->cfg.dtype), Dp = padk(m->cfg.dim);
  VaeBufs b;
  memset(&b, 0, sizeof(b));
  b.in_act = ar.take((size_t)M * padk(m->cfg.z) * es);
  b.mid[0] = ar.take((size_t)M * Dp * es);
  b.mid[1] = ar.take((size_t)M * Dp * es);
  for (int n = 0; n < m->n_wave; ++n) b.wv[n] = plan_wave(m->dec[n], M, es, ar);
  b.xres = (float*)ar.take((size_t)M * Dp * 4);
  b.tf = plan_tf(m->tf, M, es, ar);
  b.recon = need_recon ? (float*)ar.take((size_t)M * Dp * 4) : nullptr;
  b.pred_act = ar.take((size_t)M * Dp * es);
  b.logits = need_logits ? (float*)ar.take((size_t)M * m->cfg.vocab * 4) : nullptr;
  return b;
}
}

extern "C" size_t dn_vae_workspace_bytes(const DnVae* m, int32_t B, int32_t T) {
  if (!m || B <= 0 || T <= 0) return 0;
  Arena a{nullptr, 0, 0}, d{nullptr, 0, 0};
  (void)plan_vae_enc(m, B * T, a);
  (void)plan_vae_dec(m, B * T, true, true, d);
  return (a.off > d.off ? a.off : d.off) + 256;
}

extern "C" int dn_vae_encode_params(DnVae* m, const float* feat, int32_t B, int32_t T, float* params, void* workspace,
                                    size_t workspace_bytes, void* stream) {
  DN_CHECK_ARG(m && feat && params && workspace && B > 0 && T > 0, "dn_vae_encode_params: bad argument");
  DN_CHECK_ARG(((uintptr_t)workspace & 255) == 0, "dn_vae_encode_params: workspace must be 256-byte aligned");
  hipStream_t s = (hipStream_t)stream;
  const int dtype = m->cfg.dtype, M = B * T;
  Arena ar{(char*)workspace, 0, workspace_bytes};
  VaeBufs b = plan_vae_enc(m, M, ar);
  if (ar.off > workspace_bytes) {
    dn_set_error("dn_vae_encode_params: workspace %zu < required %zu", workspace_bytes, ar.off);
    return DN_EWORKSPACE;
  }
  DN_TRY(dn_convert_rows(feat, DN_F32, m->cfg.dim, b.in_act, dtype, padk(m->cfg.dim), M, m->cfg.dim, s));
  const void* cur = b.in_act;
  for (int n = 0; n < m->n_wave; ++n) {
    const WavenetW& w = m->enc[n];
    const bool lastw = n == m->n_wave - 1;
    DnGemmParams fin = gemm_base(dtype, M, lastw ? w.cout : padk(w.cout), padk(w.cout), T);
    if (lastw) {
      fin.out = params; fin.ldo = w.cout; fin.out_dtype = DN_F32;
    } else {
      fin.out = b.mid[n & 1]; fin.ldo = padk(w.cout); fin.out_dtype = dtype;
    }
    DN_TRY(run_wavenet(w, dtype, cur, M, T, nullptr, 0, b.wv[n], fin, s));
    cur = b.mid[n & 1];
  }
  return DN_OK;
}

extern "C" int dn_vae_decode(DnVae* m, const float* latent, const int32_t* lengths, int32_t B, int32_t T, float* recon, float* logits,
                             int32_t* units, void* workspace, size_t workspace_bytes, void* stream) {
  DN_CHECK_ARG(m && latent && lengths && workspace && B > 0 && T > 0, "dn_vae_decode: bad argument");
  DN_CHECK_ARG(((uintptr_t)workspace & 255) == 0, "dn_vae_decode: workspace must be 256-byte aligned");
// ... 39 lines not shown
```

### diffnorm_amd/csrc/gemm_kernels.h

```cpp
#include <math.h>
#include <stdlib.h>

#include <type_traits>

#pragma once
#include "common.h"

#ifndef DN_GEMM_ABL
#define DN_GEMM_ABL 0
#endif

namespace dn {

static __device__ uint4 g_zero_page[8];

constexpr int BN = 128, ROWB = 128;
constexpr int W_TILE_BYTES = BN * ROWB;

typedef const __attribute__((address_space(1))) void* gptr_t;
typedef __attribute__((address_space(3))) void* lptr_t;

__device__ __forceinline__ void glds16(const void* src, uint32_t lds_addr) {
  uint32_t keep;
  asm volatile(
// ... 609 lines not shown
  auto mma_all = [&]() {
    if constexpr (std::is_same<E, BF16X3>::value) {
#pragma unroll
      for (int pass = 0; pass < 3; ++pass)
#pragma unroll
        for (int nt = 0; nt < 4; ++nt)
#pragma unroll
          for (int mt = 0; mt < 4; ++mt)
            mma_kstep<BF16>(acc[nt][mt], wf[pass == 0 ? 0 : 1][nt], af[pass == 1 ? 1 : 0][mt]);
    } else {
#pragma unroll
      for (int ks = 0; ks < 2; ++ks)
#pragma unroll
        for (int nt = 0; nt < 4; ++nt)
#pragma unroll
          for (int mt = 0; mt < 4; ++mt) mma_kstep<E>(acc[nt][mt], wf[ks][nt], af[ks][mt]);
    }
  };

  const RowSsqReq rs_req = row_scale_request<EPI>(p, m0 + wm * 64, lane);
  setup_term(0);
  if constexpr (STAGES == 3) {
    const bool late = __builtin_amdgcn_readfirstlane(wave) >= NWAVES / 2;
    stage(0);
    if (nkt > 1) stage(1);
    if (nkt > 1) pipe_sync<PER_STAGE>(); else pipe_sync<0>();
    __builtin_amdgcn_sched_barrier(0);
    if (late) pipe_sync<63>();
    auto ktile = [&](auto late_c, auto stage_c, int slot, int fill) {
      constexpr bool LATE = decltype(late_c)::value, STAGE = decltype(stage_c)::value;
      if constexpr (!(DN_GEMM_ABL & 4)) load_frags(slot);
      if constexpr (STAGE && !(DN_GEMM_ABL & 1)) stage(fill);
      if constexpr (LATE) pipe_sync<STAGE ? PER_STAGE : 0>(); else pipe_sync<63>();
      __builtin_amdgcn_sched_barrier(0);
      if constexpr (!(DN_GEMM_ABL & 8)) __builtin_amdgcn_s_setprio(1);
      if constexpr (!(DN_GEMM_ABL & 2)) mma_all();
      __builtin_amdgcn_s_setprio(0);
      __builtin_amdgcn_sched_barrier(0);
      if constexpr (LATE) pipe_sync<63>(); else pipe_sync<STAGE ? PER_STAGE : 0>();
      __builtin_amdgcn_sched_barrier(0);
    };
    auto run = [&](auto late_c) {
      int slot = 0, fill = 2, kt = 0;
      auto adv = [&]() { slot = slot == 2 ? 0 : slot + 1; fill = fill == 2 ? 0 : fill + 1; };
      for (; kt + 2 < nkt; ++kt) { ktile(late_c, std::true_type{}, slot, fill); adv(); }
      for (; kt < nkt; ++kt) { ktile(late_c, std::false_type{}, slot, fill); adv(); }
    };
    if (late) run(std::true_type{}); else run(std::false_type{});
    if (!late) pipe_sync<63>();
  } else {
    stage(0);
    int slot = 0;
    for (int kt = 0; kt < nkt; ++kt) {
      pipe_sync<0>();
      if (kt + 1 < nkt) stage(slot ^ 1);
      load_frags(slot);
      mma_all();
      slot ^= 1;
    }
  }

  if constexpr (STAGES != 3) __syncthreads();
  float* ep = reinterpret_cast<float*>(smem) + wave * (64 * EP_LD);
  const float row_scale = row_scale_finish(p, rs_req);
  float sc4[4];
  slab_row_scales(row_scale, lane, sc4);
#pragma unroll
  for (int mt = 0; mt < 4; ++mt)
#pragma unroll
    for (int nt = 0; nt < 4; ++nt)
      *reinterpret_cast<f32x4*>(ep + (mt * 16 + frow) * EP_LD + nt * 16 + fq * 4) = scaled(acc[nt][mt], sc4[mt]);
  asm volatile("s_waitcnt lgkmcnt(0)" ::: "memory");

  if constexpr (EPI == DN_EPI_RESADD)
    wave_epilogue<EPI, std::is_same<E, BF16X3>::value, std::is_same<E, F16>::value>(p, ep, m0 + wm * 64, n0 + wn * 64, g, lane, 64, row_scale >= 0.f ? ROW_PRESCALED : row_scale, pre_res);
  else
    wave_epilogue<EPI, std::is_same<E, BF16X3>::value, std::is_same<E, F16>::value>(p, ep, m0 + wm * 64, n0 + wn * 64, g, lane, 64, row_scale >= 0.f ? ROW_PRESCALED : row_scale);
}

constexpr int ROWB2 = 64;

template <typename E, int EPI, bool TAPS, int BNB = 256, bool HALO = false>
__global__ __launch_bounds__(512, 1) void conv_gemm_big_kernel(const DnGemmParams p) {
  static_assert(!HALO || (TAPS && BNB == 256 && !std::is_same<E, BF16X3>::value), "shared staging: tap-inner order on the 256 x 256 tile");
  extern __shared__ __attribute__((aligned(16))) char smem[];
  if constexpr (std::is_same<E, F16>::value) f16_saturate();
  constexpr int ES = Elem<E>::bytes;
  constexpr int KT = ROWB2 / ES;
  static_assert(BNB == 256 || BNB == 192, "tile width");
  constexpr int BMB = 256, STAGES = 4;
  constexpr int TILE = BNB * ROWB2;
  constexpr int STAGE_BYTES = TILE + 256 * ROWB2;
  constexpr int PER_STAGE = 4;
  constexpr int PER_LATE = BNB == 256 ? 4 : 3;
  constexpr int NTW = BNB / 32;

  const int tid = threadIdx.x;
  const int lane = tid & 63;
  const int wave = __builtin_amdgcn_readfirstlane(tid >> 6);
  const int wm = wave >> 1, wn = wave & 1;
  const int g = blockIdx.y;
  const int np_total = p.N * (EPI == DN_EPI_GEGLU ? 2 : 1);
  const int n_tiles_n = (np_total + BNB - 1) / BNB;
  int logical;
  {
    const int nwg = gridDim.x, bid = blockIdx.x;
    const int xcd = bid & 7, q = nwg >> 3, r = nwg & 7;
    logical = (xcd < r ? xcd * (q + 1) : r * (q + 1) + (xcd - r) * q) + (bid >> 3);
  }
  int mt_, nt_;
  tile_coords(logical, n_tiles_n, (p.M + BMB - 1) / BMB, (p.flags >> DN_GEMM_BAND_SHIFT) & 0xff, mt_, nt_);
  const int m0 = mt_ * BMB;
  const int n0 = nt_ * BNB;
  const int w_rows = (np_total + 127) / 128 * 128;

  const int srow = lane >> 2;
  const int schunk = (lane & 3) ^ (((lane >> 5) & 1) << 1);
  int a_row[2], a_t[2], w_row[2];
#pragma unroll
  for (int i = 0; i < 2; ++i) {
    int m = m0 + wave * 32 + i * 16 + srow;
    m = m < p.M ? m : p.M - 1;
    a_row[i] = m;
    a_t[i] = m % p.T;
    int n = n0 + (BNB == 256 || wave < 4 ? wave * 32 + i * 16 : 128 + (wave - 4) * 16) + srow;
    w_row[i] = n < w_rows ? n : w_rows - 1;
  }
  const int ktiles_per_term = p.K / KT;
  const int nkt = p.n_terms * ktiles_per_term;
  const char* zero_src = reinterpret_cast<const char*>(g_zero_page) + schunk * 16;
  const char* a_ptr[2];
  const char* w_ptr[2];
  int a_inc[2], w_inc = ROWB2;
  int s_term = 0, s_kk = 0;
  auto setup_term = [&](int term) {
    const DnGemmTerm& tm = p.terms[term];
    const int shift = tm.shift_by_group ? tm.shift * (1 << g) : tm.shift;
    const char* A = reinterpret_cast<const char*>(tm.A) + (tm.a_gstride * g) * ES + schunk * 16;
    const char* W = reinterpret_cast<const char*>(tm.W) + (tm.w_gstride * g) * ES + schunk * 16;
    const bool a_kb = tm.layout & DN_LAYOUT_A_KBLOCKED, w_kb = tm.layout & DN_LAYOUT_W_KBLOCKED;
    const int64_t a_rowb = a_kb ? ROWB2 : (int64_t)tm.lda * ES, w_rowb = w_kb ? ROWB2 : (int64_t)(tm.ldw ? tm.ldw : p.K) * ES;
    const int a_step = a_kb ? p.M * ROWB2 : ROWB2;
    w_inc = w_kb ? w_rows * ROWB2 : ROWB2;
#pragma unroll
    for (int i = 0; i < 2; ++i) {
      const bool valid = shift_valid(a_t[i], shift, p.T);
      a_ptr[i] = valid ? A + (int64_t)(a_row[i] - shift) * a_rowb : zero_src;
      a_inc[i] = valid ? a_step : 0;
      w_ptr[i] = W + (int64_t)w_row[i] * w_rowb;
    }
  };
  int tap_shift = 0, tap_shift0 = 0, tap_sstep = 0;
  int64_t tap_delta = 0, tap_delta0 = 0, tap_dstep = 0, tap_woff = 0, tap_wstride = 0;
  int tap_ainc = ROWB2;
  [[maybe_unused]] const char* halo_ptr = nullptr;
  [[maybe_unused]] int halo_inc = 0, halo_rows = 0, a_rdh[3] = {0, 0, 0};
  [[maybe_unused]] uint64_t halo_mask = 0;
  auto setup_taps = [&]() {
    const DnGemmTerm& t0 = p.terms[0];
    const DnGemmTerm& t1 = p.terms[1];
    const int sh0 = t0.shift_by_group ? (t0.shift << g) : t0.shift, sh1 = t1.shift_by_group ? (t1.shift << g) : t1.shift;
    const bool a_kb = t0.layout & DN_LAYOUT_A_KBLOCKED, w_kb = t0.layout & DN_LAYOUT_W_KBLOCKED;
    const int64_t a_rowb = a_kb ? ROWB2 : (int64_t)t0.lda * ES, w_rowb = w_kb ? ROWB2 : (int64_t)(t0.ldw ? t0.ldw : p.K) * ES;
    tap_shift0 = sh0; tap_sstep = sh0 - sh1;
    tap_delta0 = sh0 * a_rowb; tap_dstep = tap_sstep * a_rowb;
    tap_wstride = (int64_t)((intptr_t)t1.W - (intptr_t)t0.W);
    tap_shift = tap_shift0; tap_delta = tap_delta0; tap_woff = 0;
    tap_ainc = a_kb ? p.M * ROWB2 : ROWB2;
    w_inc = w_kb ? w_rows * ROWB2 : ROWB2;
    const char* A = reinterpret_cast<const char*>(t0.A) + (t0.a_gstride * g) * ES + schunk * 16;
    const char* W = reinterpret_cast<const char*>(t0.W) + (t0.w_gstride * g) * ES + schunk * 16;
#pragma unroll
    for (int i = 0; i < 2; ++i) {
      a_ptr[i] = A + (int64_t)a_row[i] * a_rowb;
      w_ptr[i] = W + (int64_t)w_row[i] * w_rowb;
    }
    if constexpr (HALO) {
      halo_rows = (2 * sh1 + 15) / 16 * 16;
      const int per_wave = halo_rows >> 3;
      const int R = wave * per_wave + (lane >> 2);
      const int hchunk = (lane & 3) ^ (((R >> 3) & 1) << 1);
      const bool before = m0 % p.T + R - halo_rows < 0;
      const char* A0 = reinterpret_cast<const char*>(t0.A) + (t0.a_gstride * g) * ES + hchunk * 16;
      halo_ptr = before ? reinterpret_cast<const char*>(g_zero_page) + hchunk * 16 : A0 + (int64_t)(m0 + R - halo_rows) * a_rowb;
      halo_inc = before ? 0 : tap_ainc;
      halo_mask = per_wave >= 16 ? ~0ull : (1ull << (4 * per_wave)) - 1;
#pragma unroll
      for (int t = 0; t < 3; ++t) {
        const int row = halo_rows + wm * 64 + (lane & 15) - (2 - t) * sh1;
        a_rdh[t] = row * ROWB2 + (((lane >> 4) ^ (((row >> 3) & 1) << 1)) << 4);
      }
    }
  };
  const uint32_t lds_base = __builtin_amdgcn_readfirstlane((uint32_t)(uintptr_t)(lptr_t)smem);
  auto stage = [&](int slot) {
    const bool one_w = BNB != 256 && wave >= 4;
    const uint32_t wbase = lds_base + slot * STAGE_BYTES + (one_w ? 8192 + (wave - 4) * 1024 : wave * 2048);
    const uint32_t abase = lds_base + slot * STAGE_BYTES + TILE + wave * 2048;
    if constexpr (TAPS) {
#pragma unroll
      for (int i = 0; i < 2; ++i)
        if (i == 0 || !one_w) glds16(w_ptr[i] + tap_woff, wbase + i * 1024);
#pragma unroll
      for (int i = 0; i < 2; ++i) glds16(a_t[i] >= tap_shift ? a_ptr[i] - tap_delta : zero_src, abase + i * 1024);
      const bool wrap = s_term + 1 == p.n_terms;
      s_term = wrap ? 0 : s_term + 1;
      tap_shift = wrap ? tap_shift0 : tap_shift - tap_sstep;
      tap_delta = wrap ? tap_delta0 : tap_delta - tap_dstep;
      tap_woff = wrap ? 0 : tap_woff + tap_wstride;
      const int ai = wrap ? tap_ainc : 0, wi = wrap ? w_inc : 0;
#pragma unroll
      for (int i = 0; i < 2; ++i) {
        a_ptr[i] += ai;
        w_ptr[i] += wi;
      }
      return;
    }
#pragma unroll
    for (int i = 0; i < 2; ++i)
      if (i == 0 || !one_w) glds16(w_ptr[i], wbase + i * 1024);
#pragma unroll
    for (int i = 0; i < 2; ++i) glds16(a_ptr[i], abase + i * 1024);
    if (++s_kk == ktiles_per_term) {
      s_kk = 0;
      if (++s_term < p.n_terms) setup_term(s_term);
    } else {
#pragma unroll
      for (int i = 0; i < 2; ++i) {
        a_ptr[i] += a_inc[i];
        w_ptr[i] += w_inc;
      }
    }
  };

  f32x4 acc[NTW][4];
#pragma unroll
  for (int i = 0; i < NTW; ++i)
#pragma unroll
    for (int j = 0; j < 4; ++j) acc[i][j] = f32x4{0.f, 0.f, 0.f, 0.f};

  const int frow = lane & 15, fq = lane >> 4;
  const int coff = (fq ^ (((frow >> 3) & 1) << 1)) << 4;
  const int w_rd = (wn * (BNB / 2) + frow) * ROWB2 + coff;
  const int a_rd = TILE + (wm * 64 + frow) * ROWB2 + coff;
  constexpr bool X3 = std::is_same<E, BF16X3>::value;
  using ME = typename std::conditional<X3, BF16, E>::type;
  uint4 wf[NTW], af[4], ah[X3 ? 4 : 1];
  auto load_frags = [&](int slot, auto par_c) {
    constexpr int PAR = decltype(par_c)::value;
    const char* sb = smem + slot * STAGE_BYTES;
#pragma unroll
    for (int i = 0; i < NTW; ++i) wf[i] = *reinterpret_cast<const uint4*>(sb + w_rd + i * 16 * ROWB2);
#pragma unroll
    for (int i = 0; i < 4; ++i) (PAR == 1 ? ah[i] : af[i]) = *reinterpret_cast<const uint4*>(sb + a_rd + i * 16 * ROWB2);
  };
  auto mma_all = [&](auto par_c) {
    constexpr int PAR = decltype(par_c)::value;
    if constexpr (PAR != 1) {
#pragma unroll
      for (int nt = 0; nt < NTW; ++nt)
#pragma unroll
        for (int mt = 0; mt < 4; ++mt) mma_kstep<ME>(acc[nt][mt], wf[nt], af[mt]);
    }
    if constexpr (PAR != 0) {
#pragma unroll
      for (int nt = 0; nt < NTW; ++nt)
#pragma unroll
        for (int mt = 0; mt < 4; ++mt) mma_kstep<ME>(acc[nt][mt], wf[nt], ah[mt]);
    }
  };

  const RowSsqReq rs_req = row_scale_request<EPI>(p, m0 + wm * 64, lane);
  if constexpr (TAPS) setup_taps(); else setup_term(0);
  const bool late = __builtin_amdgcn_readfirstlane(wave) >= 4;
  bool shared_rows = false;
  if constexpr (HALO) {
    const int t_first = m0 % p.T;
    shared_rows = halo_rows <= 128 && (t_first + BMB <= p.T || m0 + (p.T - t_first) >= p.M);
  }
  if constexpr (HALO) {
    if (shared_rows) {
      const uint32_t abase = lds_base + STAGES * TILE;
#pragma unroll
      for (int i = 0; i < 2; ++i) {
        glds16(a_ptr[i], abase + halo_rows * ROWB2 + wave * 2048 + i * 1024);
        a_ptr[i] += tap_ainc;
      }
      glds16_lanes(halo_ptr, abase + wave * (halo_rows >> 3) * ROWB2, halo_mask);
      halo_ptr += halo_inc;
#pragma unroll
      for (int t = 0; t < 3; ++t) {
#pragma unroll
        for (int i = 0; i < 2; ++i) glds16(w_ptr[i] + tap_woff, lds_base + t * TILE + wave * 2048 + i * 1024);
        tap_woff += tap_wstride;
      }
      tap_woff = 0;
#pragma unroll
      for (int i = 0; i < 2; ++i) w_ptr[i] += w_inc;
      pipe_sync<4>();
    }
  }
  if (!shared_rows) {
#pragma unroll
  for (int st = 0; st < STAGES - 1; ++st)
    if (st < nkt) stage(st);
  if (BNB != 256 && __builtin_amdgcn_readfirstlane(wave) >= 4) {
    if (nkt > 2) pipe_sync<2 * PER_LATE>(); else if (nkt > 1) pipe_sync<PER_LATE>(); else pipe_sync<0>();
  } else {
    if (nkt > 2) pipe_sync<2 * PER_STAGE>(); else if (nkt > 1) pipe_sync<PER_STAGE>(); else pipe_sync<0>();
  }
  }
  const float row_scale = row_scale_finish(p, rs_req);
  __builtin_amdgcn_sched_barrier(0);
  if (late) pipe_sync<63>();
  auto ktile = [&](auto late_c, auto stage_c, auto sync_c, int slot, int fill, auto par_c) {
    constexpr bool LATE = decltype(late_c)::value, STAGE = decltype(stage_c)::value;
    constexpr int SYNC = decltype(sync_c)::value;
    if constexpr (!(DN_GEMM_ABL & 4)) load_frags(slot, par_c);
    if constexpr (STAGE && !(DN_GEMM_ABL & 1)) stage(fill);
    if constexpr (LATE) pipe_sync<SYNC>(); else pipe_sync<63>();
    __builtin_amdgcn_sched_barrier(0);
    if constexpr (!(DN_GEMM_ABL & 8)) __builtin_amdgcn_s_setprio(1);
    if constexpr (!(DN_GEMM_ABL & 2)) mma_all(par_c);
    __builtin_amdgcn_s_setprio(0);
    __builtin_amdgcn_sched_barrier(0);
    if constexpr (LATE) pipe_sync<63>(); else pipe_sync<SYNC>();
    __builtin_amdgcn_sched_barrier(0);
  };
  auto run = [&](auto late_c) {
    using std::integral_constant;
    int slot = 0, fill = STAGES - 1, kt = 0;
    auto adv = [&]() { slot = slot == STAGES - 1 ? 0 : slot + 1; fill = fill == STAGES - 1 ? 0 : fill + 1; };
    using P0 = integral_constant<int, 0>;
    constexpr int PER = decltype(late_c)::value ? PER_LATE : PER_STAGE;
    if constexpr (X3) {
      using EV = integral_constant<int, 1>;
      using OD = integral_constant<int, 2>;
      if (nkt >= 4) {
        for (; kt + 4 < nkt; kt += 2) {
          ktile(late_c, std::true_type{}, integral_constant<int, 2 * PER>{}, slot, fill, EV{}); adv();
          ktile(late_c, std::true_type{}, integral_constant<int, 2 * PER>{}, slot, fill, OD{}); adv();
        }
        ktile(late_c, std::true_type{}, integral_constant<int, 2 * PER>{}, slot, fill, EV{}); adv();
        ktile(late_c, std::false_type{}, integral_constant<int, PER>{}, slot, fill, OD{}); adv();
      }
      ktile(late_c, std::false_type{}, integral_constant<int, 0>{}, slot, fill, EV{}); adv();
      ktile(late_c, std::false_type{}, integral_constant<int, 0>{}, slot, fill, OD{});
    } else {
    for (; kt + 3 < nkt; ++kt) { ktile(late_c, std::true_type{}, integral_constant<int, 2 * PER>{}, slot, fill, P0{}); adv(); }
    if (nkt >= 3) { ktile(late_c, std::false_type{}, integral_constant<int, PER>{}, slot, fill, P0{}); adv(); }
    if (nkt >= 2) { ktile(late_c, std::false_type{}, integral_constant<int, 0>{}, slot, fill, P0{}); adv(); }
    ktile(late_c, std::false_type{}, integral_constant<int, 0>{}, slot, fill, P0{});
    }
  };
  constexpr int A_RING = STAGES * TILE, A_SLOT = (256 + 128) * ROWB2;
  [[maybe_unused]] auto ktile_h = [&](auto late_c, auto tap_c, auto stage_c, auto sync_c, int slot, int fill, int aslot) {
    constexpr bool LATE = decltype(late_c)::value, STAGE = decltype(stage_c)::value;
    constexpr int TAP = decltype(tap_c)::value, SYNC = decltype(sync_c)::value;
    {
      const char* sw = smem + slot * TILE;
      const char* sa = smem + A_RING + aslot * A_SLOT + a_rdh[TAP];
#pragma unroll
      for (int i = 0; i < NTW; ++i) wf[i] = *reinterpret_cast<const uint4*>(sw + w_rd + i * 16 * ROWB2);
#pragma unroll
      for (int i = 0; i < 4; ++i) af[i] = *reinterpret_cast<const uint4*>(sa + i * 16 * ROWB2);
    }
    if constexpr (STAGE) {
      const uint32_t wbase = lds_base + fill * TILE + wave * 2048;
#pragma unroll
      for (int i = 0; i < 2; ++i) glds16(w_ptr[i] + tap_woff, wbase + i * 1024);
      if constexpr (TAP == 2) {
        tap_woff = 0;
#pragma unroll
        for (int i = 0; i < 2; ++i) w_ptr[i] += w_inc;
      } else {
        tap_woff += tap_wstride;
      }
      const uint32_t abase = lds_base + A_RING + (aslot ^ 1) * A_SLOT;
      if constexpr (TAP == 0) {
#pragma unroll
        for (int i = 0; i < 2; ++i) {
          glds16(a_ptr[i], abase + halo_rows * ROWB2 + wave * 2048 + i * 1024);
          a_ptr[i] += tap_ainc;
        }
      }
      if constexpr (TAP == 1) {
        glds16_lanes(halo_ptr, abase + wave * (halo_rows >> 3) * ROWB2, halo_mask);
        halo_ptr += halo_inc;
      }
    }
    if constexpr (LATE) pipe_sync<SYNC>(); else pipe_sync<63>();
    __builtin_amdgcn_sched_barrier(0);
    __builtin_amdgcn_s_setprio(1);
    mma_all(std::integral_constant<int, 0>{});
    __builtin_amdgcn_s_setprio(0);
    __builtin_amdgcn_sched_barrier(0);
    if constexpr (LATE) pipe_sync<63>(); else pipe_sync<SYNC>();
    __builtin_amdgcn_sched_barrier(0);
  };
  [[maybe_unused]] auto run_h = [&](auto late_c) {
    using std::integral_constant;
    using T0 = integral_constant<int, 0>; using T1 = integral_constant<int, 1>; using T2 = integral_constant<int, 2>;
    int slot = 0, fill = STAGES - 1, aslot = 0;
    auto adv = [&]() { slot = slot == STAGES - 1 ? 0 : slot + 1; fill = fill == STAGES - 1 ? 0 : fill + 1; };
    const int chunks = ktiles_per_term;
    for (int c = 0; c + 1 < chunks; ++c) {
      ktile_h(late_c, T0{}, std::true_type{}, integral_constant<int, 6>{}, slot, fill, aslot); adv();
      ktile_h(late_c, T1{}, std::true_type{}, integral_constant<int, 7>{}, slot, fill, aslot); adv();
      ktile_h(late_c, T2{}, std::true_type{}, integral_constant<int, 2>{}, slot, fill, aslot); adv();
      aslot ^= 1;
    }
    ktile_h(late_c, T0{}, std::false_type{}, integral_constant<int, 3>{}, slot, fill, aslot); adv();
    ktile_h(late_c, T1{}, std::false_type{}, integral_constant<int, 0>{}, slot, fill, aslot); adv();
    ktile_h(late_c, T2{}, std::false_type{}, integral_constant<int, 0>{}, slot, fill, aslot);
  };
  if (!shared_rows) { if (late) run(std::true_type{}); else run(std::false_type{}); }
  if constexpr (HALO) {
    if (shared_rows) { if (late) run_h(std::true_type{}); else run_h(std::false_type{}); }
  }
  if (!late) pipe_sync<63>();

  float* ep = reinterpret_cast<float*>(smem) + wave * (64 * EP_LD);
  float sc4[4];
  slab_row_scales(row_scale, lane, sc4);
  auto half = [&](auto hc) {
    constexpr int H = decltype(hc)::value;
    constexpr int NTS = NTW - 4 * H < 4 ? NTW - 4 * H : 4;
#pragma unroll
    for (int mt = 0; mt < 4; ++mt)
#pragma unroll
      for (int nt = 0; nt < NTS; ++nt)
        *reinterpret_cast<f32x4*>(ep + (mt * 16 + frow) * EP_LD + nt * 16 + fq * 4) = scaled(acc[H * 4 + nt][mt], sc4[mt]);
    asm volatile("s_waitcnt lgkmcnt(0)" ::: "memory");
    wave_epilogue<EPI, std::is_same<E, BF16X3>::value, std::is_same<E, F16>::value>(p, ep, m0 + wm * 64, n0 + wn * (BNB / 2) + H * 64, g, lane, NTS * 16, row_scale >= 0.f ? ROW_PRESCALED : row_scale);
    asm volatile("s_waitcnt lgkmcnt(0)" ::: "memory");
  };
  half(std::integral_constant<int, 0>{});
  half(std::integral_constant<int, 1>{});
}

constexpr int BNM = 128;
template <typename E, int EPI>
__global__ __launch_bounds__(256, 2) void conv_gemm_mid2_kernel(const DnGemmParams p) {
  extern __shared__ __attribute__((aligned(16))) char smem[];
  static_assert(!std::is_same<E, BF16X3>::value, "split operands pair K-tiles: not on this tile");
  if constexpr (std::is_same<E, F16>::value) f16_saturate();
  constexpr int ES = Elem<E>::bytes;
  constexpr int KT = ROWB2 / ES;
  constexpr int BMM = 256, STAGES = 3;
  constexpr int WT = BNM * ROWB2, STAGE_BYTES = WT + BMM * ROWB2;
  constexpr int PER = 6;

  const int tid = threadIdx.x;
  const int lane = tid & 63;
  const int wave = __builtin_amdgcn_readfirstlane(tid >> 6);
  const int wm = wave >> 1, wn = wave & 1;
  const int g = blockIdx.y;
  const int np_total = p.N * (EPI == DN_EPI_GEGLU ? 2 : 1);
  const int n_tiles_n = (np_total + BNM - 1) / BNM;
  int logical;
  {
    const int nwg = gridDim.x, bid = blockIdx.x;
    const int xcd = bid & 7, q = nwg >> 3, r = nwg & 7;
    logical = (xcd < r ? xcd * (q + 1) : r * (q + 1) + (xcd - r) * q) + (bid >> 3);
  }
  int mt_, nt_;
  tile_coords(logical, n_tiles_n, (p.M + BMM - 1) / BMM, (p.flags >> DN_GEMM_BAND_SHIFT) & 0xff, mt_, nt_);
  const int m0 = mt_ * BMM, n0 = nt_ * BNM;
  const int w_rows = (np_total + 127) / 128 * 128;

  const int srow = lane >> 2;
  const int schunk = (lane & 3) ^ (((lane >> 5) & 1) << 1);
  int a_row[4], a_t[4], w_row[2];
#pragma unroll
  for (int i = 0; i < 4; ++i) {
    int m = m0 + wave * 64 + i * 16 + srow;
    m = m < p.M ? m : p.M - 1;
    a_row[i] = m;
    a_t[i] = m % p.T;
  }
#pragma unroll
  for (int i = 0; i < 2; ++i) {
    const int n = n0 + wave * 32 + i * 16 + srow;
    w_row[i] = n < w_rows ? n : w_rows - 1;
  }
  const int ktiles_per_term = p.K / KT;
  const int nkt = p.n_terms * ktiles_per_term;
  const char* zero_src = reinterpret_cast<const char*>(g_zero_page) + schunk * 16;
  const char* a_ptr[4];
  const char* w_ptr[2];
  int a_inc[4], w_inc = ROWB2;
  int s_term = 0, s_kk = 0;
  auto setup_term = [&](int term) {
    const DnGemmTerm& tm = p.terms[term];
    const int shift = tm.shift_by_group ? tm.shift * (1 << g) : tm.shift;
    const char* A = reinterpret_cast<const char*>(tm.A) + (tm.a_gstride * g) * ES + schunk * 16;
    const char* W = reinterpret_cast<const char*>(tm.W) + (tm.w_gstride * g) * ES + schunk * 16;
    const bool a_kb = tm.layout & DN_LAYOUT_A_KBLOCKED, w_kb = tm.layout & DN_LAYOUT_W_KBLOCKED;
    const int64_t a_rowb = a_kb ? ROWB2 : (int64_t)tm.lda * ES, w_rowb = w_kb ? ROWB2 : (int64_t)(tm.ldw ? tm.ldw : p.K) * ES;
    const int a_step = a_kb ? p.M * ROWB2 : ROWB2;
    w_inc = w_kb ? w_rows * ROWB2 : ROWB2;
#pragma unroll
    for (int i = 0; i < 4; ++i) {
      const bool valid = shift_valid(a_t[i], shift, p.T);
      a_ptr[i] = valid ? A + (int64_t)(a_row[i] - shift) * a_rowb : zero_src;
      a_inc[i] = valid ? a_step : 0;
    }
#pragma unroll
    for (int i = 0; i < 2; ++i) w_ptr[i] = W + (int64_t)w_row[i] * w_rowb;
  };
  const uint32_t lds_base = __builtin_amdgcn_readfirstlane((uint32_t)(uintptr_t)(lptr_t)smem);
  auto stage = [&](int slot) {
    const uint32_t wbase = lds_base + slot * STAGE_BYTES + wave * 2048;
    const uint32_t abase = lds_base + slot * STAGE_BYTES + WT + wave * 4096;
#pragma unroll
    for (int i = 0; i < 2; ++i) glds16(w_ptr[i], wbase + i * 1024);
#pragma unroll
    for (int i = 0; i < 4; ++i) glds16(a_ptr[i], abase + i * 1024);
    if (++s_kk == ktiles_per_term) {
      s_kk = 0;
      if (++s_term < p.n_terms) setup_term(s_term);
// ... 759 lines not shown
  const uint32_t ep_lds = lds_base + (wave * (64 * EP_LD) + frow * EP_LD + fq * 4) * 4;
  constexpr int NHS = (NTW + 3) / 4, MHS = MT / 4;
#pragma unroll 1
  for (int sidx = 0; sidx < MHS * NHS; ++sidx) {
    static_for<MHS * NHS>([&](auto s_c) {
      constexpr int MH = decltype(s_c)::value / NHS, NH = decltype(s_c)::value % NHS;
      constexpr int NTS = NTW - 4 * NH < 4 ? NTW - 4 * NH : 4;
      if (sidx == MH * NHS + NH) {
        if constexpr (WAVES == 8) {
          static_for<4 * NTS>([&](auto i_c) {
            constexpr int mt = decltype(i_c)::value / NTS, nt = decltype(i_c)::value % NTS;
            acc_to_lds<(mt * 16 * EP_LD + nt * 16) * 4>(ep_lds, acc[NH * 4 + nt][MH * 4 + mt]);
          });
        } else {
#pragma unroll
          for (int mt = 0; mt < 4; ++mt)
#pragma unroll
            for (int nt = 0; nt < NTS; ++nt)
              *reinterpret_cast<f32x4*>(ep + (mt * 16 + frow) * EP_LD + nt * 16 + fq * 4) = acc[NH * 4 + nt][MH * 4 + mt];
        }
      }
    });
    const int mh = sidx / NHS, nh = sidx - mh * NHS;
    const int nts = NTW - 4 * nh < 4 ? NTW - 4 * nh : 4;
    asm volatile("s_waitcnt lgkmcnt(0)" ::: "memory");
    int m_slab = m0 + wm * RPW + mh * 64, n_slab = n0 + wn * (16 * NTW) + nh * 64;
    if constexpr (WAVES == 8)
      asm volatile("" : "+s"(m_slab), "+s"(n_slab));
    wave_epilogue<EPI, std::is_same<E, BF16X3>::value, std::is_same<E, F16>::value>(p, ep, m_slab, n_slab, g, lane, nts * 16, -1.f);
    asm volatile("s_waitcnt lgkmcnt(0)" ::: "memory");
  }
}

using Route = DnGemmRoute;

static inline bool terms_are_taps(const DnGemmParams& p) {
  const bool env_taps = option_or(OPT_TAPS_INNER, 1) != 0;
  bool taps = p.n_terms >= 2 && p.n_terms <= 4 && !(p.flags & DN_GEMM_TERM_OUTER) && (env_taps || (p.flags & DN_GEMM_TAPS_INNER));
  for (int i = 0; i < p.n_terms; ++i) taps = taps && p.terms[i].layout == p.terms[0].layout && p.terms[i].shift >= 0;
  for (int i = 1; i < p.n_terms && taps; ++i) {
    const DnGemmTerm &a = p.terms[i], &b = p.terms[i - 1], &t0 = p.terms[0], &t1 = p.terms[1];
    taps = a.A == t0.A && a.lda == t0.lda && a.a_gstride == t0.a_gstride && a.w_gstride == t0.w_gstride &&
           a.shift_by_group == t0.shift_by_group && b.shift - a.shift == t0.shift - t1.shift && t0.shift >= t1.shift &&
           (intptr_t)a.W - (intptr_t)b.W == (intptr_t)t1.W - (intptr_t)t0.W;
  }
  return taps;
}

static inline bool big_taps_share_rows(const DnGemmParams& p, int kt_elems) {
  static const bool env_off = getenv("DN_BIG_HALO") && atoi(getenv("DN_BIG_HALO")) == 0;
  if (env_off || (p.flags & DN_GEMM_NO_SHARED_ROWS) || p.n_terms != 3 || p.K / kt_elems < 2) return false;
  const DnGemmTerm &t0 = p.terms[0], &t1 = p.terms[1], &t2 = p.terms[2];
  return t2.shift == 0 && t1.shift >= 1 && t0.shift == 2 * t1.shift && (t0.shift_by_group || 2 * t1.shift <= 128);
}

static inline bool taps_share_rows(const DnGemmParams& p) {
  static const bool env_off = getenv("DN_FAT_HALO") && atoi(getenv("DN_FAT_HALO")) == 0;
  if (env_off || (p.flags & DN_GEMM_NO_SHARED_ROWS) || p.n_terms != 3 || p.K < 96) return false;
  const DnGemmTerm &t0 = p.terms[0], &t1 = p.terms[1], &t2 = p.terms[2];
  return !t0.shift_by_group && t2.shift == 0 && t1.shift >= 1 && t1.shift <= 8 && t0.shift == 2 * t1.shift;
}

static inline int forced_tile(const DnGemmParams& p) {
  static const int env_tile = getenv("DN_GEMM_TILE") ? atoi(getenv("DN_GEMM_TILE")) : 0;
  const int bits = (p.flags >> DN_GEMM_TILE_SHIFT) & 15;
  return bits ? bits : env_tile;
}

static inline bool routes_to_352(const DnGemmParams& p, int force) {
  if (!dn_is16(p.dtype) || (p.epilogue != DN_EPI_BIAS && p.epilogue != DN_EPI_GEGLU)) return false;
  const int npk = p.N * (p.epilogue == DN_EPI_GEGLU ? 2 : 1);
  if (npk % 352 != 0) return false;
  if (force == DN_TILE_256X352) return true;
  if (force != 0 || p.epilogue != DN_EPI_BIAS) return false;
  const long twin = (p.flags & DN_GEMM_TWIN) ? 2 : 1;
  const long tiles_fat = (long)((p.M + 255) / 256) * (npk / 352) * p.groups * twin;
  const long tiles_big = (long)((p.M + 255) / 256) * ((npk + 255) / 256) * p.groups * twin;
  auto fill = [](long tiles) { const double r = (double)tiles / 256.0; return r / ceil(r); };
  static const bool old_rule = getenv("DN_352_ROUTE") && atoi(getenv("DN_352_ROUTE")) == 0;
  if (old_rule) return tiles_fat / twin >= 100;
  return tiles_fat >= 100 && 1.3 * fill(tiles_fat) >= fill(tiles_big);
}

static inline int choose_tile(const DnGemmParams& p, int force, bool taps) {
  const bool bf = dn_is16(p.dtype);
  if ((p.epilogue == DN_EPI_RESADD || p.epilogue == DN_EPI_POSEMB) && p.norm_out && !p.norm_split && p.dtype != DN_BF16X3) return DN_TILE_ROW;
  bool has_ldw = false;
  for (int i = 0; i < p.n_terms; ++i) has_ldw = has_ldw || p.terms[i].ldw != 0;
  if (p.dtype == DN_F32 && p.M <= 128 && force == 0 && (long)p.N * p.K * p.groups >= (8L << 20)) return DN_TILE_128X128;
  if (has_ldw && p.dtype != DN_BF16X3) {
    const int npw = p.N * (p.epilogue == DN_EPI_GEGLU ? 2 : 1);
    const long tb = (long)((p.M + 255) / 256) * ((npw + 255) / 256) * p.groups, ts = (long)((p.M + 127) / 128) * ((npw + BN - 1) / BN) * p.groups;
    if (force >= DN_TILE_128X128 && force <= DN_TILE_256X256) return force;
    return tb >= 256 ? DN_TILE_256X256 : ts >= 512 ? DN_TILE_256X128 : DN_TILE_128X128;
  }
  if (p.dtype == DN_BF16X3) {
    for (int i = 0; i < p.n_terms; ++i)
      if (p.terms[i].layout != 0) return -1;
    if ((force >= DN_TILE_128X128 && force <= DN_TILE_256X256) || (force == DN_TILE_256X192 && p.epilogue == DN_EPI_BIAS)) return force;
    const int npx = p.N * (p.epilogue == DN_EPI_GEGLU ? 2 : 1);
    const long mt2 = (p.M + 255) / 256, t_big = mt2 * ((npx + 255) / 256) * p.groups, t_mid = mt2 * ((npx + BN - 1) / BN) * p.groups,
               t_small = (long)((p.M + 127) / 128) * ((npx + BN - 1) / BN) * p.groups;
    auto fill2 = [](long tiles, int per_cu) { const double r = (double)tiles / (256.0 * per_cu); return r / ceil(r); };
    const double sb = 1.00 * fill2(t_big, 1), sm = 0.80 * fill2(t_mid, 1), ss = 0.70 * fill2(t_small, 2);
    static const bool use192 = getenv("DN_X3_192") && atoi(getenv("DN_X3_192")) != 0;
    if (p.epilogue == DN_EPI_BIAS && force == 0 && use192) {
      const int c192 = (npx + 191) / 192;
      const double s192 = 0.97 * fill2(mt2 * c192 * p.groups, 1) * npx / (192.0 * c192) / (npx / (256.0 * ((npx + 255) / 256)));
      if (s192 > sb && s192 > sm && s192 > ss) return DN_TILE_256X192;
    }
    if (sb >= sm && sb >= ss) return DN_TILE_256X256;
    return sm > ss ? DN_TILE_256X128 : DN_TILE_128X128;
  }
  if (routes_to_352(p, force)) return DN_TILE_256X352;
  const bool taps_route_by_shape = option_or(OPT_TAPS_INNER, 1) == 2;
  if (force == 0 && (p.epilogue == DN_EPI_BIAS || p.epilogue == DN_EPI_FILM_GATE) && taps_route_by_shape && taps) return DN_TILE_256X256;
  bool kblocked = false;
  for (int i = 0; i < p.n_terms; ++i) kblocked = kblocked || p.terms[i].layout != 0;
  const bool mid2_ok = bf && p.epilogue != DN_EPI_RESADD && p.epilogue != DN_EPI_POSEMB;
  if (kblocked)
    return bf && force == DN_TILE_256X192 && p.epilogue == DN_EPI_BIAS ? DN_TILE_256X192
           : mid2_ok && force == DN_TILE_256X128_2WG                  ? DN_TILE_256X128_2WG
           : bf && (force == 0 || force == DN_TILE_256X256)            ? DN_TILE_256X256
                                                                       : -1;
  if (bf && force == DN_TILE_256X192 && (p.epilogue == DN_EPI_BIAS || (p.epilogue == DN_EPI_RESADD && !(p.norm_out && p.norm_split)))) return DN_TILE_256X192;
  if (mid2_ok && force == DN_TILE_256X128_2WG) return DN_TILE_256X128_2WG;
  if (p.dtype == DN_BF16 && (force == DN_TILE_256X256_W4 || force == DN_TILE_256X256_W8)) return force;
  if (force >= DN_TILE_128X128 && force <= DN_TILE_256X256) return force;

  const int np = p.N * (p.epilogue == DN_EPI_GEGLU ? 2 : 1);
  const long mt256 = (p.M + 255) / 256, mt128 = (p.M + 127) / 128;
  const long tiles_big = mt256 * ((np + 255) / 256) * p.groups;
  const long tiles_mid = mt256 * ((np + BN - 1) / BN) * p.groups;
  const long tiles_small = mt128 * ((np + BN - 1) / BN) * p.groups;
  static const int heur = getenv("DN_GEMM_HEUR") ? atoi(getenv("DN_GEMM_HEUR")) : 1;
  if (heur == 0)
    return tiles_big >= 360 ? DN_TILE_256X256 : tiles_mid >= 192 ? DN_TILE_256X128 : DN_TILE_128X128;
  if (bf && p.epilogue == DN_EPI_GEGLU && tiles_big >= 256 && heur != 3) return DN_TILE_256X256;
  auto fill = [](long tiles, int per_cu) {
    const double rounds = (double)tiles / (256.0 * per_cu);
    return rounds / ceil(rounds);
  };
  const bool multi_long = heur != 4 && (p.epilogue == DN_EPI_BIAS || p.epilogue == DN_EPI_FILM_GATE) && p.n_terms >= 2 && (long)p.K * p.n_terms >= 1024;
  const bool long_taps = multi_long && taps;
  const bool shares = long_taps && big_taps_share_rows(p, 32) && heur != 5;
  const bool long_k = heur == 5 ? long_taps : multi_long;
  const double s_big = 1.00 * fill(tiles_big, 1), s_mid = (shares ? 0.68 : long_k ? 0.78 : 0.90) * fill(tiles_mid, 1),
               s_small = (shares ? 0.60 : long_k ? 0.72 : 0.92) * fill(tiles_small, 2);
  if (bf && (p.epilogue == DN_EPI_BIAS || p.epilogue == DN_EPI_RESADD) && !long_taps && !(p.flags & DN_GEMM_TWIN) && !(p.norm_out && p.norm_split) &&
      (long)p.K * p.n_terms >= 768 && option_or(OPT_TILE_192, 1) != 0) {
    const int c192 = (np + 191) / 192, c256 = (np + 255) / 256;
    const double s_192 = 0.90 * fill(mt256 * c192 * p.groups, 1) * (256.0 * c256) / (192.0 * c192);
    if (s_big >= s_mid && s_big >= s_small && s_192 > s_big) return DN_TILE_256X192;
  }
  if (s_big >= s_mid && s_big >= s_small) return DN_TILE_256X256;
  return s_mid > s_small ? DN_TILE_256X128 : DN_TILE_128X128;
}

static inline int choose_band(const DnGemmParams& p, int tile) {
  static const int env_band = getenv("DN_GEMM_BAND") ? atoi(getenv("DN_GEMM_BAND")) : -1;
  if (env_band >= 0) return env_band < 255 ? env_band : 255;
  const int es = dn_is16(p.dtype) ? 2 : 4;
  const bool two_per_cu = tile == DN_TILE_128X128 || tile == DN_TILE_256X128_2WG;
  const int bm = tile == DN_TILE_128X128 ? 128 : 256, bn = tile == DN_TILE_256X256 ? 256 : 128, conc = 32 * (two_per_cu ? 2 : 1);
  const int np = p.N * (p.epilogue == DN_EPI_GEGLU ? 2 : 1);
  const double w_total = (double)np * p.K * p.n_terms * es;
  if (w_total < 6.0e6) return 1;
  bool same_a = true;
  for (int i = 1; i < p.n_terms; ++i) same_a = same_a && p.terms[i].A == p.terms[0].A;
  const double a_panel = (double)bm * p.K * es * (same_a ? 1 : p.n_terms), w_panel = (double)bn * p.K * p.n_terms * es;
  int band = (int)(sqrt(conc * w_panel / a_panel) + 0.5);
  const int m_tiles = (p.M + bm - 1) / bm;
  band = band < 1 ? 1 : band > m_tiles ? m_tiles : band;
  return band < 255 ? band : 255;
}

static inline Route route(const DnGemmParams& p) {
  const bool taps = terms_are_taps(p);
  Route r;
  r.tile = choose_tile(p, forced_tile(p), taps);
  const bool conv_epi = p.epilogue == DN_EPI_BIAS || p.epilogue == DN_EPI_FILM_GATE;
  const bool big = r.tile == DN_TILE_256X256 && conv_epi && p.dtype != DN_BF16X3;
  const bool fat = r.tile == DN_TILE_256X352 || r.tile == DN_TILE_256X256_W4 || r.tile == DN_TILE_256X256_W8;
  r.taps_inner = taps && (big || fat);
  r.shared_rows = r.taps_inner && (big ? big_taps_share_rows(p, ROWB2 / (dn_is16(p.dtype) ? 2 : 4))
                                       : r.tile == DN_TILE_256X352 && p.epilogue == DN_EPI_BIAS && taps_share_rows(p));
  const int forced_band = (p.flags >> DN_GEMM_BAND_SHIFT) & 0xff;
  const bool banded = (r.tile >= DN_TILE_128X128 && r.tile <= DN_TILE_256X256) || r.tile == DN_TILE_256X128_2WG;
  r.band = banded && forced_band == 0 ? choose_band(p, r.tile) : forced_band;
  return r;
}

template <auto KERNEL>
static int launch_kernel(const DnGemmParams& p, dim3 grid, int threads, int lds, hipStream_t s) {
  static bool attr_done = false;
  if (!attr_done) {
    (void)hipFuncSetAttribute(reinterpret_cast<const void*>(KERNEL), hipFuncAttributeMaxDynamicSharedMemorySize, lds);
    attr_done = true;
  }
  const bool timed = g_prof.cap > 0 && ((p.flags >> DN_GEMM_TAG_SHIFT) & 0xff) == g_prof.tag && g_prof.n < g_prof.cap;
  if (timed) (void)hipEventRecord(g_prof.ev[2 * g_prof.n], s);
  hipLaunchKernelGGL(KERNEL, grid, dim3(threads), lds, s, p);
  if (timed) (void)hipEventRecord(g_prof.ev[2 * g_prof.n++ + 1], s);
  DN_CHECK_LAUNCH("dn_conv_gemm");
  return DN_OK;
}

template <int EPI>
static inline int packed_cols(const DnGemmParams& p) { return p.N * (EPI == DN_EPI_GEGLU ? 2 : 1); }

template <typename E, int EPI, int BM, int STAGES>
static int launch_tile(const DnGemmParams& p, hipStream_t s) {
  constexpr int ring = STAGES * (W_TILE_BYTES + BM * ROWB), slabs = (BM / 32) * 64 * 68 * 4;
  constexpr int lds = ring > slabs ? ring : slabs;
  const dim3 grid(((p.M + BM - 1) / BM) * ((packed_cols<EPI>(p) + BN - 1) / BN), p.groups);
  return launch_kernel<conv_gemm_kernel<E, EPI, BM, STAGES>>(p, grid, BM * 2, lds, s);
}

template <typename E, int EPI, int BNB = 256>
static int launch_big(const DnGemmParams& p, const Route& r, hipStream_t s) {
  constexpr int ring = 4 * (BNB + 256) * ROWB2, slabs = 8 * 64 * EP_LD * 4;
  constexpr int lds = ring > slabs ? ring : slabs;
  const dim3 grid(((p.M + 255) / 256) * ((packed_cols<EPI>(p) + BNB - 1) / BNB), p.groups);
  if constexpr ((EPI == DN_EPI_BIAS || EPI == DN_EPI_FILM_GATE) && !std::is_same<E, BF16X3>::value && BNB == 256) {
    if (r.shared_rows) return launch_kernel<conv_gemm_big_kernel<E, EPI, true, 256, true>>(p, grid, 512, lds, s);
    if (r.taps_inner) return launch_kernel<conv_gemm_big_kernel<E, EPI, true>>(p, grid, 512, lds, s);
  }
  return launch_kernel<conv_gemm_big_kernel<E, EPI, false, BNB>>(p, grid, 512, lds, s);
}

template <typename E, int EPI>
static int launch_mid2(const DnGemmParams& p, hipStream_t s) {
  constexpr int ring = 3 * (BNM + 256) * ROWB2, slabs = 4 * 64 * EP_LD * 4;
  constexpr int lds = ring > slabs ? ring : slabs;
  const dim3 grid(((p.M + 255) / 256) * ((packed_cols<EPI>(p) + BNM - 1) / BNM), p.groups);
  return launch_kernel<conv_gemm_mid2_kernel<E, EPI>>(p, grid, 256, lds, s);
}

template <typename E, int EPI>
static int launch_row(const DnGemmParams& p, hipStream_t s) {
  constexpr int ring = 2 * (512 + 64) * ROWB, slabs = 8 * 64 * EP_LD * 4 + 64 * 8 * 4;
  constexpr int lds = ring > slabs ? ring : slabs;
  return launch_kernel<conv_gemm_row_kernel<E, EPI>>(p, dim3((p.M + 63) / 64, p.groups), 512, lds, s);
}

template <typename E, int EPI, int NTW, int WAVES = 4>
static int launch_fat(const DnGemmParams& p, const Route& r, hipStream_t s) {
  constexpr int BNF = 32 * NTW;
  constexpr int ring = 4 * (BNF + 256) * ROWB2, slabs = WAVES * 64 * EP_LD * 4;
  constexpr int lds = ring > slabs ? ring : slabs;
  const dim3 grid(((p.M + 255) / 256) * ((packed_cols<EPI>(p) + BNF - 1) / BNF), p.groups);
  if constexpr (NTW == 11 && WAVES == 4 && EPI == DN_EPI_BIAS) {
    if (r.shared_rows) return launch_kernel<conv_gemm_fat_kernel<E, EPI, true, NTW, WAVES, true>>(p, grid, 64 * WAVES, lds, s);
  }
  if (r.taps_inner) return launch_kernel<conv_gemm_fat_kernel<E, EPI, true, NTW, WAVES>>(p, grid, 64 * WAVES, lds, s);
  return launch_kernel<conv_gemm_fat_kernel<E, EPI, false, NTW, WAVES>>(p, grid, 64 * WAVES, lds, s);
}

template <typename E, int EPI>
static int launch(const DnGemmParams& p0, hipStream_t s) {
  const Route r = route(p0);
  DN_CHECK_ARG(r.tile > 0, "dn_conv_gemm: K-blocked operands are taken by the 256 x 352 and 256 x 256 tiles only (bf16; forced tile %d)",
               forced_tile(p0));
  DnGemmParams p = p0;
  static const bool no_res_prefetch = getenv("DN_RES_PREFETCH") && atoi(getenv("DN_RES_PREFETCH")) == 0;
  if (no_res_prefetch) p.flags |= DN_GEMM_NO_RES_PREFETCH;
  p.flags = (int32_t)(((uint32_t)p.flags & ~(0xffu << DN_GEMM_BAND_SHIFT)) | ((uint32_t)r.band << DN_GEMM_BAND_SHIFT));
  constexpr bool x3 = std::is_same<E, BF16X3>::value, half = IsHalf<E>::value;
  switch (r.tile) {
    case DN_TILE_256X256: return launch_big<E, EPI>(p, r, s);
    case DN_TILE_256X128: return launch_tile<E, EPI, 256, 3>(p, s);
    case DN_TILE_ROW:
      if constexpr (!x3 && (EPI == DN_EPI_RESADD || EPI == DN_EPI_POSEMB)) return launch_row<E, EPI>(p, s);
      break;
    case DN_TILE_256X352:
      if constexpr (half && (EPI == DN_EPI_BIAS || EPI == DN_EPI_GEGLU)) return launch_fat<E, EPI, 11>(p, r, s);
      break;
    case DN_TILE_256X192:
      if constexpr ((x3 && EPI == DN_EPI_BIAS) || (half && (EPI == DN_EPI_BIAS || EPI == DN_EPI_RESADD))) return launch_big<E, EPI, 192>(p, r, s);
      if constexpr (x3) return launch_big<E, EPI>(p, r, s);
      break;
    case DN_TILE_256X128_2WG:
      if constexpr (half && EPI != DN_EPI_RESADD && EPI != DN_EPI_POSEMB) return launch_mid2<E, EPI>(p, s);
      break;
    case DN_TILE_256X256_W4:
      if constexpr (std::is_same<E, BF16>::value) return launch_fat<E, EPI, 8>(p, r, s);
      break;
    case DN_TILE_256X256_W8:
      if constexpr (std::is_same<E, BF16>::value) return launch_fat<E, EPI, 8, 8>(p, r, s);
      break;
  }
  return launch_tile<E, EPI, 128, 2>(p, s);
}

template <typename E>
static int dispatch_epi(const DnGemmParams& p, hipStream_t s) {
  switch (p.epilogue) {
    case DN_EPI_BIAS: return launch<E, DN_EPI_BIAS>(p, s);
    case DN_EPI_SILU: return launch<E, DN_EPI_SILU>(p, s);
    case DN_EPI_RELU: {
      DnGemmParams q = p;
      q.epilogue = DN_EPI_SILU;
      q.flags |= DN_GEMM_RELU;
      return launch<E, DN_EPI_SILU>(q, s);
    }
    case DN_EPI_GEGLU: return launch<E, DN_EPI_GEGLU>(p, s);
    case DN_EPI_FILM_GATE: return launch<E, DN_EPI_FILM_GATE>(p, s);
    case DN_EPI_RESADD: return launch<E, DN_EPI_RESADD>(p, s);
    case DN_EPI_POSEMB: return launch<E, DN_EPI_POSEMB>(p, s);
  }
  dn_set_error("dn_conv_gemm: unknown epilogue %d", p.epilogue);
  return DN_EINVAL;
}

int gemm_dispatch_bf16(const DnGemmParams& p, hipStream_t s);
int gemm_dispatch_f32(const DnGemmParams& p, hipStream_t s);
int gemm_dispatch_x3(const DnGemmParams& p, hipStream_t s);
int gemm_dispatch_f16(const DnGemmParams& p, hipStream_t s);

}
```

### diffnorm_amd/csrc/repack.hip

```cpp
#include "common.h"

namespace dn {
namespace {

constexpr int kRepackBlocks = 1024;

template <int DT>
__device__ __forceinline__ uint4 to16(const float4& a, const float4& b) {
  if constexpr (DT == DN_F16)
    return make_uint4(pack_f16x2_sat(a.x, a.y), pack_f16x2_sat(a.z, a.w), pack_f16x2_sat(b.x, b.y), pack_f16x2_sat(b.z, b.w));
  else
    return make_uint4(pack_bf16x2(a.x, a.y), pack_bf16x2(a.z, a.w), pack_bf16x2(b.x, b.y), pack_bf16x2(b.z, b.w));
}

template <int DT>
__device__ __forceinline__ void store8(void* dst, int64_t e, const float4& a, const float4& b) {
  if constexpr (DT == DN_F32) {
    float4* p = reinterpret_cast<float4*>(reinterpret_cast<float*>(dst) + e);
    p[0] = a;
    p[1] = b;
  } else if constexpr (DT == DN_BF16X3) {
    uint32_t h0, l0, h1, l1, h2, l2, h3, l3;
    split_pair(a.x, a.y, h0, l0);
    split_pair(a.z, a.w, h1, l1);
    split_pair(b.x, b.y, h2, l2);
    split_pair(b.z, b.w, h3, l3);
    char* p = reinterpret_cast<char*>(dst) + split_byte(e);
    *reinterpret_cast<uint4*>(p) = make_uint4(l0, l1, l2, l3);
    *reinterpret_cast<uint4*>(p + 64) = make_uint4(h0, h1, h2, h3);
  } else {
    *reinterpret_cast<uint4*>(reinterpret_cast<uint16_t*>(dst) + e) = to16<DT>(a, b);
  }
}

template <int DT>
__global__ __launch_bounds__(256) void repack_kernel(const float* __restrict__ master, const DnRepackDesc* __restrict__ descs) {
  const DnRepackDesc d = descs[blockIdx.y];
  const float* __restrict__ src = master + d.src;
  const int64_t n = (int64_t)d.mats * d.rows * d.K;
  const int64_t first = (int64_t)blockIdx.x * 256 + threadIdx.x, step = (int64_t)gridDim.x * 256;
  if (d.kind == DN_REPACK_CONVERT) {
    for (int64_t u = first; u < n / 8; u += step) {
      const float4* p = reinterpret_cast<const float4*>(src + u * 8);
      store8<DT>(d.dst, u * 8, p[0], p[1]);
    }
  } else if (d.kind == DN_REPACK_KBLOCK) {
    if constexpr (DT == DN_BF16 || DT == DN_F16) {
      const int64_t per_mat = (int64_t)d.rows * d.K / 8, per_kb = (int64_t)d.rows * 4;
      for (int64_t u = first; u < n / 8; u += step) {
        const int64_t m = u / per_mat, rem = u - m * per_mat;
        const int64_t kb = rem / per_kb, in_kb = rem - kb * per_kb;
        const int64_t r = in_kb >> 2, q = in_kb & 3;
        const float4* p = reinterpret_cast<const float4*>(src + (m * d.rows + r) * d.K + kb * 32 + q * 8);
        *reinterpret_cast<uint4*>(reinterpret_cast<uint16_t*>(d.dst) + u * 8) = to16<DT>(p[0], p[1]);
      }
    }
  } else if (d.kind == DN_REPACK_COPY) {
    float* __restrict__ out = reinterpret_cast<float*>(d.dst);
    if ((n & 3) == 0 && (reinterpret_cast<uintptr_t>(out) & 15) == 0 && (reinterpret_cast<uintptr_t>(src) & 15) == 0) {
      for (int64_t u = first; u < n / 4; u += step) reinterpret_cast<float4*>(out)[u] = reinterpret_cast<const float4*>(src)[u];
    } else {
      for (int64_t i = first; i < n; i += step) out[i] = src[i];
    }
  } else {
    float4* __restrict__ out = reinterpret_cast<float4*>(d.dst);
    for (int64_t u = first; u < n / 4; u += step) {
      float4 acc = make_float4(0.f, 0.f, 0.f, 0.f);
      for (int j = 0; j < d.count; ++j) {
        const float4 v = *reinterpret_cast<const float4*>(src + j * d.stride + u * 4);
        acc.x += v.x; acc.y += v.y; acc.z += v.z; acc.w += v.w;
      }
      out[u] = acc;
    }
  }
}

struct FoldArgs {
  const float *conv_W, *conv_b, *out_W, *out_b;
  int64_t conv_W_ls, conv_b_ls, out_W_ls, out_b_ls;
  int dim, inner, ip, in_n, Dp, Dn;
  void* W;
  float* b;
};

template <int DT>
__global__ __launch_bounds__(64) void ffn_fold_w_kernel(FoldArgs a) {
  const int u = blockIdx.x * 64 + threadIdx.x, n0 = blockIdx.y * 4, l = blockIdx.z / 3, tap = blockIdx.z % 3;
  if (u * 8 >= a.ip) return;
  const int c = u * 8;
  const float* __restrict__ wc = a.conv_W + l * a.conv_W_ls + (int64_t)tap * a.in_n * a.ip + c;
  const float* __restrict__ wo = a.out_W + l * a.out_W_ls + (int64_t)n0 * a.ip;
  float acc[4][8];
#pragma unroll
  for (int r = 0; r < 4; ++r)
#pragma unroll
    for (int i = 0; i < 8; ++i) acc[r][i] = 0.f;
  for (int k = 0; k < a.inner; ++k) {
    const float4 x0 = *reinterpret_cast<const float4*>(wc + (int64_t)k * a.ip), x1 = *reinterpret_cast<const float4*>(wc + (int64_t)k * a.ip + 4);
    const float x[8] = {x0.x, x0.y, x0.z, x0.w, x1.x, x1.y, x1.z, x1.w};
#pragma unroll
    for (int r = 0; r < 4; ++r) {
      const float w = wo[(int64_t)r * a.ip + k];
#pragma unroll
      for (int i = 0; i < 8; ++i) acc[r][i] = fmaf(w, x[i], acc[r][i]);
    }
  }
#pragma unroll
  for (int r = 0; r < 4; ++r) {
    float v[8];
#pragma unroll
    for (int i = 0; i < 8; ++i) v[i] = (n0 + r < a.dim && c + i < a.inner) ? acc[r][i] : 0.f;
    store8<DT>(a.W, (((int64_t)blockIdx.z * a.Dn) + n0 + r) * a.ip + c, make_float4(v[0], v[1], v[2], v[3]), make_float4(v[4], v[5], v[6], v[7]));
  }
}

__global__ __launch_bounds__(64) void ffn_fold_b_kernel(FoldArgs a) {
  const int n = blockIdx.x * 64 + threadIdx.x, l = blockIdx.y;
  if (n >= a.Dp) return;
  float acc = 0.f;
  if (n < a.dim) {
    const float* __restrict__ wo = a.out_W + l * a.out_W_ls + (int64_t)n * a.ip;
    const float* __restrict__ bc = a.conv_b + l * a.conv_b_ls;
    for (int k = 0; k < a.inner; ++k) acc = fmaf(wo[k], bc[k], acc);
    acc += a.out_b[l * a.out_b_ls + n];
  }
  a.b[(int64_t)l * a.Dp + n] = acc;
}

}
}

extern "C" int dn_repack_weights(const float* master, const DnRepackDesc* descs, int32_t n, int32_t dtype, void* stream) {
  DN_CHECK_ARG(master && descs, "dn_repack_weights: null argument");
  DN_CHECK_ARG(n >= 1 && n <= 65535, "dn_repack_weights: n=%d descriptors (1 .. 65535)", n);
  DN_CHECK_ARG(dtype == DN_F32 || dtype == DN_BF16 || dtype == DN_BF16X3 || dtype == DN_F16, "dn_repack_weights: dtype=%d", dtype);
  DN_CHECK_ARG(((uintptr_t)master & 15) == 0 && ((uintptr_t)descs & 7) == 0, "dn_repack_weights: master 16-byte, descs 8-byte aligned");
  const dim3 grid(dn::kRepackBlocks, n), block(256);
  hipStream_t s = (hipStream_t)stream;
  if (dtype == DN_F32) hipLaunchKernelGGL(dn::repack_kernel<DN_F32>, grid, block, 0, s, master, descs);
  else if (dtype == DN_BF16) hipLaunchKernelGGL(dn::repack_kernel<DN_BF16>, grid, block, 0, s, master, descs);
  else if (dtype == DN_F16) hipLaunchKernelGGL(dn::repack_kernel<DN_F16>, grid, block, 0, s, master, descs);
  else hipLaunchKernelGGL(dn::repack_kernel<DN_BF16X3>, grid, block, 0, s, master, descs);
  DN_CHECK_LAUNCH("dn_repack_weights");
  return DN_OK;
}

extern "C" int dn_ffn_fold(const float* conv_W, const float* conv_b, const float* out_W, const float* out_b, int64_t conv_W_stride,
                           int64_t conv_b_stride, int64_t out_W_stride, int64_t out_b_stride, int32_t depth, int32_t dim, int32_t inner,
                           int32_t dtype, void* fold_W, float* fold_b, void* stream) {
  DN_CHECK_ARG(conv_W && conv_b && out_W && out_b && fold_W && fold_b, "dn_ffn_fold: null argument");
  DN_CHECK_ARG(depth >= 1 && 3 * depth <= 65535 && dim >= 1 && inner >= 1, "dn_ffn_fold: depth=%d dim=%d inner=%d", depth, dim, inner);
  DN_CHECK_ARG(dtype == DN_F32 || dtype == DN_BF16 || dtype == DN_BF16X3 || dtype == DN_F16, "dn_ffn_fold: dtype=%d", dtype);
  DN_CHECK_ARG((conv_W_stride | out_W_stride) % 4 == 0 && (((uintptr_t)conv_W | (uintptr_t)out_W) & 15) == 0 && ((uintptr_t)fold_W & 127) == 0,
               "dn_ffn_fold: the weight sources must be 16-byte aligned (strides multiples of 4), the folded weights 128-byte aligned");
  dn::FoldArgs a;
  a.conv_W = conv_W; a.conv_b = conv_b; a.out_W = out_W; a.out_b = out_b;
  a.conv_W_ls = conv_W_stride; a.conv_b_ls = conv_b_stride; a.out_W_ls = out_W_stride; a.out_b_ls = out_b_stride;
  a.dim = dim; a.inner = inner; a.ip = (inner + 63) / 64 * 64; a.in_n = (inner + 127) / 128 * 128; a.Dp = (dim + 63) / 64 * 64; a.Dn = (dim + 127) / 128 * 128;
  a.W = fold_W; a.b = fold_b;
  const dim3 grid((a.ip / 8 + 63) / 64, a.Dn / 4, 3 * depth), block(64);
  hipStream_t s = (hipStream_t)stream;
  if (dtype == DN_F32) hipLaunchKernelGGL(dn::ffn_fold_w_kernel<DN_F32>, grid, block, 0, s, a);
  else if (dtype == DN_BF16) hipLaunchKernelGGL(dn::ffn_fold_w_kernel<DN_BF16>, grid, block, 0, s, a);
  else if (dtype == DN_F16) hipLaunchKernelGGL(dn::ffn_fold_w_kernel<DN_F16>, grid, block, 0, s, a);
  else hipLaunchKernelGGL(dn::ffn_fold_w_kernel<DN_BF16X3>, grid, block, 0, s, a);
  hipLaunchKernelGGL(dn::ffn_fold_b_kernel, dim3((a.Dp + 63) / 64, depth), block, 0, s, a);
  DN_CHECK_LAUNCH("dn_ffn_fold");
  return DN_OK;
}
```

### diffnorm_amd/engine.py

```python
import ctypes as C
from typing import List, Optional, Sequence

import numpy as np
import torch

from . import _lib, packing


def _dtype_code(dtype) -> int:
    if isinstance(dtype, str):
        names = {"bf16": _lib.DN_BF16, "f32": _lib.DN_F32, "fp32": _lib.DN_F32, "bf16x3": _lib.DN_BF16X3, "f16": _lib.DN_F16, "fp16": _lib.DN_F16}
        if dtype in names:
            return names[dtype]
    elif dtype is torch.bfloat16:
        return _lib.DN_BF16
    elif dtype is torch.float32:
        return _lib.DN_F32
    elif dtype is torch.float16:
        return _lib.DN_F16
    elif isinstance(dtype, int) and dtype in (_lib.DN_F32, _lib.DN_BF16, _lib.DN_BF16X3, _lib.DN_F16):
        return dtype
    raise ValueError(f"unsupported arithmetic dtype {dtype!r} (use 'bf16', 'f16', 'bf16x3' or 'f32')")


# ... 24 lines not shown
        g = torch.cuda.CUDAGraph()
        with torch.cuda.stream(side):
            with torch.cuda.graph(g, stream=side):
                step()
        cur.wait_stream(side)
    return g


class _Engine:
    def __init__(self, device, tensors: List[torch.Tensor]):
        self.device = _require_cuda(device)
        self.lib = _lib.load()
        self.tensors = [t.to(self.device).contiguous() for t in tensors]
        self._table = (C.c_void_p * len(self.tensors))(*[t.data_ptr() for t in self.tensors])
        self._ws: Optional[torch.Tensor] = None
        self.handle = C.c_void_p()

    def _workspace(self, nbytes: int) -> torch.Tensor:
        if self._ws is None or self._ws.numel() < nbytes:
            self._ws = torch.empty(nbytes + 256, dtype=torch.uint8, device=self.device)
        return self._ws

    @staticmethod
    def _aligned(ws: torch.Tensor):
        p = ws.data_ptr()
        a = (p + 255) & ~255
        return a, ws.numel() - (a - p)

    def _aligned_workspace(self, nbytes):
        return self._aligned(self._workspace(int(nbytes)))

    def weight_bytes(self) -> int:
        return sum(t.numel() * t.element_size() for t in self.tensors)

    _kind = None
    _repack = None

    def _repack_descs(self, train_engine):
        key = (tuple(train_engine.offsets), int(train_engine.n_params))
        if self._repack is not None and self._repack[0] == key:
            return self._repack
        plan = packing.repack_plan(train_engine.entries, train_engine.offsets, self.dtype, kind=self._kind)
        if len(plan.shapes) != len(self.tensors):
            raise ValueError(f"refresh_from: the training engine's layout gives {len(plan.shapes)} packed tensors, this engine has {len(self.tensors)}")
        for i, (s, t) in enumerate(zip(plan.shapes, self.tensors)):
            if s is not None and (tuple(t.shape) != tuple(s[0]) or t.dtype != s[1]):
                raise ValueError(f"refresh_from: packed tensor {i} is {tuple(t.shape)} {t.dtype}, the training engine's layout gives {s[0]} {s[1]}")
        descs = (_lib.RepackDesc * len(plan.items))()
        moved = 0
        for d, it in zip(descs, plan.items):
            n = it.mats * it.rows * it.K
            reads = n * max(1, it.count)
            assert 0 <= it.src and it.src + (reads if it.count else n) <= train_engine.n_params, it
            t = self.tensors[it.tensor]
            out_bytes = n * (4 if it.kind in (_lib.REPACK_COPY, _lib.REPACK_SUM) or not packing._is16(self.dtype) else 2)
            assert it.dst_byte + out_bytes <= t.numel() * t.element_size(), it
            dst = t.data_ptr() + it.dst_byte
            assert it.src % 4 == 0, it
            if it.kind in (_lib.REPACK_CONVERT, _lib.REPACK_KBLOCK):
                assert n % 32 == 0 and it.K % 32 == 0 and dst % 128 == 0, it
            elif it.kind == _lib.REPACK_SUM:
                assert it.K % 4 == 0 and it.stride % 4 == 0 and it.mats == it.rows == 1 and dst % 16 == 0, it
            d.src, d.dst, d.kind, d.mats, d.rows, d.K, d.count, d.stride = it.src, dst, it.kind, it.mats, it.rows, it.K, it.count, it.stride
            moved += reads * 4 + out_bytes
        dev = torch.frombuffer(bytearray(bytes(descs)), dtype=torch.uint8).to(self.device)
        self._repack = (key, dev, len(plan.items), moved)
        return self._repack

    def _refresh_from(self, train_engine, source: str = "model"):
        if source not in ("model", "ema"):
            raise ValueError(f"refresh_from: source {source!r} (use 'model' or 'ema')")
        master = train_engine.master if source == "model" else getattr(train_engine, "ema", None)
        if master is None:
            raise ValueError("refresh_from: source 'ema' needs the training engine's EMA (enable_ema(), --store-ema)")
        if master.device != self.device or master.dtype != torch.float32 or not master.is_contiguous() or master.numel() != train_engine.n_params:
            raise ValueError("refresh_from: the training engine's master / EMA buffer must be a contiguous fp32 tensor of n_params elements on this engine's device")
        _, descs, n, _ = self._repack_descs(train_engine)
        with torch.cuda.device(self.device):
            _lib.check(self.lib.dn_repack_weights(master.data_ptr(), descs.data_ptr(), n, self.dtype, _lib.current_stream()), "dn_repack_weights")
        self._fold_from_flat(train_engine, master)

    fold_W: Optional[torch.Tensor] = None
    fold_b: Optional[torch.Tensor] = None

    def _tf_dims(self):
        raise NotImplementedError

    def _fold_call(self, srcs, strides, depth, layer0):
        dim, _, _ = self._tf_dims()
        inner = int(dim * 4 * 2 / 3)
        (_, _), b_shape = packing.ffn_fold_storage(dim, 1, self.dtype)
        w_off = layer0 * self.fold_W[0].numel() * self.fold_W.element_size()
        _lib.check(self.lib.dn_ffn_fold(*srcs, *strides, depth, dim, inner, self.dtype, self.fold_W.data_ptr() + w_off,
                                        self.fold_b.data_ptr() + layer0 * b_shape[1] * 4, _lib.current_stream()), "dn_ffn_fold")

    def _fold_from_state_dict(self, tf_layers, sd):
        dim, depth, attach = self._tf_dims()
        (w_shape, w_dtype), b_shape = packing.ffn_fold_storage(dim, depth, self.dtype)
        with torch.cuda.device(self.device):
            self.fold_W = torch.empty(w_shape, dtype=w_dtype, device=self.device)
            self.fold_b = torch.empty(b_shape, dtype=torch.float32, device=self.device)
            for l, layer in enumerate(tf_layers):
                srcs = [t.to(self.device) for t in packing.ffn_fold_sources(layer, sd)]
                self._fold_call([t.data_ptr() for t in srcs], (0, 0, 0, 0), 1, l)
        _lib.check(attach(self.handle, self.fold_W.data_ptr(), self.fold_b.data_ptr()), "set_ffn_fold")

    def _fold_from_flat(self, train_engine, master):
        if self.fold_W is None:
            return
        _, depth, _ = self._tf_dims()
        offs, strides = packing.ffn_fold_offsets(train_engine.entries, train_engine.offsets)
        with torch.cuda.device(self.device):
            self._fold_call([master.data_ptr() + 4 * o for o in offs], strides, depth, 0)

    def fold_bytes(self) -> int:
        return 0 if self.fold_W is None else sum(t.numel() * t.element_size() for t in (self.fold_W, self.fold_b))

    def refresh_bytes(self) -> int:
        return 0 if self._repack is None else self._repack[3]


class EpsEngine(_Engine):

    def __init__(self, state_dict, cfg, dtype="bf16", device="cuda:0", max_pos: int = 2048):
        self.cfg = cfg
        self.dtype = _dtype_code(dtype)
        super().__init__(device, packing.pack_eps(state_dict, cfg, self.dtype, max_pos))
        self.conditional = getattr(cfg, "dim_prompt", 0) > 0
        c = _lib.EpsConfig(cfg.dim, cfg.latent_dim, cfg.depth, cfg.heads, cfg.dim_head, cfg.wavenet_layers,
                           cfg.wavenet_stacks, cfg.dim_cond_mult, self.dtype, max_pos, getattr(cfg, "dim_prompt", 0),
                           getattr(cfg, "num_latents_m", 0) if self.conditional else 0,
                           getattr(cfg, "resampler_depth", 0) if self.conditional else 0)
        _lib.check(self.lib.dn_eps_create(C.byref(c), self._table, len(self.tensors), C.byref(self.handle)),
                   "dn_eps_create")
        self._fold_from_state_dict(packing._eps_entries(cfg)[2], state_dict)

    def _tf_dims(self):
        return self.cfg.dim, self.cfg.depth, self.lib.dn_eps_set_ffn_fold

    def __del__(self):
        if getattr(self, "handle", None) and self.handle.value:
            self.lib.dn_eps_destroy(self.handle)
            self.handle = None

    _kind = "eps"

    def refresh_from(self, train_engine, source: str = "model"):
        if self.conditional:
            raise NotImplementedError("refresh_from covers the unconditional eps-predictor (the prompt-conditioned model has no training engine)")
        self._refresh_from(train_engine, source)
        _lib.check(self.lib.dn_eps_weights_changed(self.handle), "dn_eps_weights_changed")

    def workspace_bytes(self, B: int, T: int) -> int:
        return int(self.lib.dn_eps_workspace_bytes(self.handle, B, T))

    def forward(self, x: torch.Tensor, times: torch.Tensor, lengths: torch.Tensor, shared_t: bool = False,
                out: Optional[torch.Tensor] = None) -> torch.Tensor:
        B, T, z = x.shape
        assert z == self.cfg.latent_dim
        x = _f32(x, self.device)
        t32, l32 = _i32(times, self.device), _i32(lengths, self.device)
        out = torch.empty_like(x) if out is None else out
        wp, wn = self._aligned_workspace(self.workspace_bytes(B, T))
        with torch.cuda.device(self.device):
            _lib.check(self.lib.dn_eps_forward(self.handle, x.data_ptr(), t32.data_ptr(), l32.data_ptr(), B, T,
                                               int(shared_t), out.data_ptr(), wp, wn, _lib.current_stream()),
                       "dn_eps_forward")
        return out

    def cond_time_table(self, t0: int, n_t: int) -> torch.Tensor:
        n_cond = len(packing.eps_cond_modules(self.cfg)) * 2 * packing.padk(self.cfg.dim)
        table = torch.empty(n_t, n_cond, dtype=torch.float32, device=self.device)
        ws = torch.empty(int(self.lib.dn_eps_cond_time_table_workspace_bytes(self.handle, n_t)) + 256, dtype=torch.uint8, device=self.device)
        wp, wn = self._aligned(ws)
        with torch.cuda.device(self.device):
            _lib.check(self.lib.dn_eps_cond_time_table(self.handle, int(t0), int(n_t), table.data_ptr(), wp, wn, _lib.current_stream()),
                       "dn_eps_cond_time_table")
        return table

    def forward_cond(self, x: torch.Tensor, times: torch.Tensor, lengths: torch.Tensor, prompt: torch.Tensor, prompt_lengths: torch.Tensor,
                     drop: Optional[torch.Tensor] = None, out: Optional[torch.Tensor] = None, reuse_prompt: bool = False,
                     time_table: Optional[torch.Tensor] = None, table_t0: int = 0) -> torch.Tensor:
        B, T, z = x.shape
        Tp = prompt.shape[1]
        x, prompt = _f32(x, self.device), _f32(prompt, self.device)
        t32, l32, p32 = _i32(times, self.device), _i32(lengths, self.device), _i32(prompt_lengths, self.device)
        d32 = torch.zeros(B, dtype=torch.int32, device=self.device) if drop is None else _i32(drop, self.device)
        out = torch.empty_like(x) if out is None else out
        wp, wn = self._aligned_workspace(int(self.lib.dn_eps_cond_workspace_bytes(self.handle, B, T, Tp)))
        with torch.cuda.device(self.device):
            _lib.check(self.lib.dn_eps_forward_cond_ex(self.handle, x.data_ptr(), t32.data_ptr(), l32.data_ptr(), prompt.data_ptr(), p32.data_ptr(),
                                                       d32.data_ptr(), B, T, Tp, out.data_ptr(), wp, wn, int(bool(reuse_prompt)),
                                                       _lib.ptr(time_table), int(table_t0), 0 if time_table is None else time_table.shape[0],
                                                       _lib.current_stream()), "dn_eps_forward_cond")
        return out

    def _guided_inputs(self, lengths, prompt, prompt_lengths):
        B = prompt.shape[0]
        two = lambda t: torch.cat([t, t]).contiguous()
        drop2 = torch.cat([torch.zeros(B, dtype=torch.int32), torch.ones(B, dtype=torch.int32)]).to(self.device)
        return two(_i32(lengths, self.device)), two(_f32(prompt, self.device)), two(_i32(prompt_lengths, self.device)), drop2

    def forward_with_cond_scale(self, x, times, lengths, prompt, prompt_lengths, cond_scale: float = 1.0) -> torch.Tensor:
        B = x.shape[0]
        if cond_scale == 1.0:
            return self.forward_cond(x, times, lengths, prompt, prompt_lengths, torch.zeros(B, dtype=torch.bool))
        x = _f32(x, self.device)
        l2, p2, pl2, drop2 = self._guided_inputs(lengths, prompt, prompt_lengths)
        t2 = torch.cat([_i32(times, self.device)] * 2)
        both = self.forward_cond(torch.cat([x, x]).contiguous(), t2, l2, p2, pl2, drop2)
        out = torch.empty_like(x)
        with torch.cuda.device(self.device):
            _lib.check(self.lib.dn_cfg_combine(both.data_ptr(), float(cond_scale), x.numel(), out.data_ptr(), _lib.current_stream()), "dn_cfg_combine")
        return out

    def guided_ddim_chain(self, x: torch.Tensor, lengths, prompt, prompt_lengths, start_step: int, coef: torch.Tensor, cond_scale: float = 1.0,
                          use_graph: bool = True, hoist: bool = True) -> int:
        from . import ops

        B, T, z = self._loop_x(x)
        guided = cond_scale != 1.0
# ... 180 lines not shown
        table = torch.empty(n, n_cond, dtype=torch.float32, device=self.device)
        ws = torch.empty(int(self.lib.dn_eps_cond_time_table_workspace_bytes(self.handle, n)) + 256, dtype=torch.uint8, device=self.device)
        wp, wn = self._aligned(ws)
        with torch.cuda.device(self.device):
            _lib.check(self.lib.dn_eps_cond_time_table_steps(self.handle, st.data_ptr(), n, table.data_ptr(), wp, wn, _lib.current_stream()),
                       "dn_eps_cond_time_table_steps")
        return table

    def guided_ddim_schedule_loop(self, x: torch.Tensor, lengths, prompt, prompt_lengths, steps: torch.Tensor, coef: torch.Tensor,
                                  cond_scale: float = 1.0, eta: float = 0.0, seed: int = 0, noise: Optional[torch.Tensor] = None,
                                  use_graph: bool = True, timesteps: Optional[int] = None, keys: Optional[torch.Tensor] = None) -> int:
        B, T, z = self._loop_x(x)
        n = self._loop_schedule(steps, coef, _lib.DDIM_SCHED_COLS)
        l32 = self._on_device(lengths, torch.int32)
        pl32 = self._on_device(prompt_lengths, torch.int32)
        p32 = self._on_device(prompt, torch.float32, contiguous=True)
        assert p32.dim() == 3 and p32.shape[0] == B and p32.shape[2] == self.cfg.dim_prompt and l32.shape == (B,) and pl32.shape == (B,)
        Tp = int(p32.shape[1])
        nz = self._loop_noise(noise, (n, B, T, z), "guided_ddim_schedule_loop", eta)
        k64 = self._loop_keys(keys, B, "guided_ddim_schedule_loop", noise, seed, eta)
        self._keep = (l32, pl32, p32, steps, coef, nz, k64)
        wp, wn = self._aligned_workspace(self.lib.dn_guided_ddim_workspace_bytes(self.handle, B, T, Tp, n, int(float(cond_scale) != 1.0)))
        with torch.cuda.device(self.device):
            if k64 is not None:
                return _lib.check(self.lib.dn_guided_ddim_loop_keyed(self.handle, x.data_ptr(), l32.data_ptr(), p32.data_ptr(), pl32.data_ptr(), B,
                                                                     T, Tp, float(cond_scale), steps.data_ptr(), coef.data_ptr(), n,
                                                                     n if timesteps is None else int(timesteps), k64.data_ptr(),
                                                                     _loop_flags(use_graph), wp, wn, _lib.current_stream()),
                                  "dn_guided_ddim_loop_keyed")
            return _lib.check(self.lib.dn_guided_ddim_loop(self.handle, x.data_ptr(), l32.data_ptr(), p32.data_ptr(), pl32.data_ptr(), B, T, Tp,
                                                           float(cond_scale), steps.data_ptr(), coef.data_ptr(), n,
                                                           n if timesteps is None else int(timesteps), int(eta > 0), int(seed) & (2 ** 64 - 1),
                                                           _lib.ptr(nz), _loop_flags(use_graph), wp, wn, _lib.current_stream()),
                              "dn_guided_ddim_loop")

    def guided_dpm_schedule_loop(self, x: torch.Tensor, lengths, prompt, prompt_lengths, steps: torch.Tensor, rows: torch.Tensor,
                                 cond_scale: float = 1.0, use_graph: bool = True, timesteps: Optional[int] = None) -> int:
        B, T, z = self._loop_x(x)
        nt = None if timesteps is None else int(timesteps)
        if not (isinstance(steps, torch.Tensor) and steps.device == self.device):
            host = torch.as_tensor(steps, dtype=torch.int32).contiguous().view(-1)
            if self.lib.dn_ddim_sched_check(host.data_ptr() if host.numel() else None, int(host.numel()),
                                            int(host.numel()) if nt is None else nt) != 0:
                raise ValueError("guided_dpm_schedule_loop: " + (self.lib.dn_last_error() or b"").decode())
            steps = host.to(self.device)
        n = self._loop_schedule(steps, rows, _lib.DPM_COLS)
        l32 = self._on_device(lengths, torch.int32)
        pl32 = self._on_device(prompt_lengths, torch.int32)
        p32 = self._on_device(prompt, torch.float32, contiguous=True)
        assert p32.dim() == 3 and p32.shape[0] == B and p32.shape[2] == self.cfg.dim_prompt and l32.shape == (B,) and pl32.shape == (B,)
        Tp = int(p32.shape[1])
        self._keep = (l32, pl32, p32, steps, rows)
        wp, wn = self._aligned_workspace(self.lib.dn_guided_dpm_workspace_bytes(self.handle, B, T, Tp, n, int(float(cond_scale) != 1.0)))
        with torch.cuda.device(self.device):
            return _lib.check(self.lib.dn_guided_dpm_loop(self.handle, x.data_ptr(), l32.data_ptr(), p32.data_ptr(), pl32.data_ptr(), B, T, Tp,
                                                          float(cond_scale), steps.data_ptr(), rows.data_ptr(), n, n if nt is None else nt,
                                                          _loop_flags(use_graph), wp, wn, _lib.current_stream()), "dn_guided_dpm_loop")


class VaeEngine(_Engine):

    def __init__(self, state_dict, dim: int = 768, latent_dim: int = 128, dtype="bf16", device="cuda:0",
                 depth: int = 6, heads: int = 8, dim_head: int = 96, stacks: int = 2, layers: int = 3,
                 vocab: int = 1004):
        self.dim, self.vocab = dim, vocab
        self.mults = packing.vae_mults(latent_dim)
        z = dim
        for m in self.mults:
            z //= m
        self.z = z // 2
        self.dtype = _dtype_code(dtype)
        super().__init__(device, packing.pack_vae(state_dict, dim, self.mults, depth, heads, dim_head, stacks, layers,
                                                  vocab, self.dtype))
        mults = (C.c_int32 * 4)(*(self.mults + [0] * (4 - len(self.mults))))
        c = _lib.VaeConfig(dim, self.z, depth, heads, dim_head, stacks, layers, vocab, len(self.mults), mults, self.dtype)
        _lib.check(self.lib.dn_vae_create(C.byref(c), self._table, len(self.tensors), C.byref(self.handle)),
                   "dn_vae_create")
        self._tf = (dim, depth)
        self._fold_from_state_dict(packing._vae_entries(dim, self.mults, depth, heads, dim_head, stacks, layers, vocab)[1], state_dict)

    def _tf_dims(self):
        return self._tf[0], self._tf[1], self.lib.dn_vae_set_ffn_fold

    def __del__(self):
        if getattr(self, "handle", None) and self.handle.value:
            self.lib.dn_vae_destroy(self.handle)
            self.handle = None

    _kind = "vae"

    def refresh_from(self, train_engine, source: str = "model"):
        self._refresh_from(train_engine, source)

    def workspace_bytes(self, B: int, T: int) -> int:
        return int(self.lib.dn_vae_workspace_bytes(self.handle, B, T))

    def encode_params(self, feat: torch.Tensor) -> torch.Tensor:
        B, T, _ = feat.shape
        feat = _f32(feat, self.device)
        out = torch.empty(B, T, 2 * self.z, dtype=torch.float32, device=self.device)
        wp, wn = self._aligned_workspace(self.workspace_bytes(B, T))
        with torch.cuda.device(self.device):
            _lib.check(self.lib.dn_vae_encode_params(self.handle, feat.data_ptr(), B, T, out.data_ptr(), wp, wn,
                                                     _lib.current_stream()), "dn_vae_encode_params")
        return out

    def sample_posterior(self, params: torch.Tensor, noise: torch.Tensor, lengths: Optional[torch.Tensor] = None,
                         want_kl: bool = False):
        B, T, _ = params.shape
        noise = _f32(noise, self.device)
        z = torch.empty(B, T, self.z, dtype=torch.float32, device=self.device)
        kl_rows = torch.empty(B, T, dtype=torch.float32, device=self.device) if want_kl else None
        l32 = _i32(lengths, self.device) if lengths is not None else None
        with torch.cuda.device(self.device):
            _lib.check(self.lib.dn_posterior_sample(params.data_ptr(), 2 * self.z, noise.data_ptr(), self.z, z.data_ptr(),
                                                    None, _lib.DN_F32, self.z, B * T, self.z, T, _lib.ptr(l32),
                                                    _lib.ptr(kl_rows), _lib.current_stream()), "dn_posterior_sample")
        if want_kl:
            return z, kl_rows.sum(dim=1) / (T * self.z)
        return z

    def encode(self, feat: torch.Tensor, noise: torch.Tensor) -> torch.Tensor:
        return self.sample_posterior(self.encode_params(feat), noise)

    def decode(self, latent: torch.Tensor, lengths: torch.Tensor, want_recon=True, want_logits=True, want_units=True):
        B, T, _ = latent.shape
        latent = _f32(latent, self.device)
        l32 = _i32(lengths, self.device)
        recon = torch.empty(B, T, self.dim, dtype=torch.float32, device=self.device) if want_recon else None
        logits = torch.empty(B, T, self.vocab, dtype=torch.float32, device=self.device) if want_logits else None
        units = torch.empty(B, T, dtype=torch.int32, device=self.device) if want_units else None
        wp, wn = self._aligned_workspace(self.workspace_bytes(B, T))
        with torch.cuda.device(self.device):
            _lib.check(self.lib.dn_vae_decode(self.handle, latent.data_ptr(), l32.data_ptr(), B, T, _lib.ptr(recon),
                                              _lib.ptr(logits), _lib.ptr(units), wp, wn, _lib.current_stream()),
                       "dn_vae_decode")
        return recon, logits, units
```

### include/diffnorm_hip.h

```cpp
#ifndef DIFFNORM_HIP_H
#define DIFFNORM_HIP_H

#include <stddef.h>
#include <stdint.h>

#ifdef __cplusplus
extern "C" {
#endif

enum { DN_F32 = 0, DN_BF16 = 1, DN_BF16X3 = 2, DN_F16 = 3 };

enum {
  DN_OK = 0,
  DN_EINVAL = -1,
  DN_ELAUNCH = -2,
  DN_EWORKSPACE = -3
};

enum {
  DN_EPI_BIAS = 0,
  DN_EPI_SILU = 1,
  DN_EPI_GEGLU = 2,
  DN_EPI_FILM_GATE = 3,
  DN_EPI_RESADD = 4,
// ... 4 lines not shown
#define DN_MAX_TERMS 8

typedef struct {
  const void* A;
  const void* W;
  int32_t lda;
  int32_t shift;
  int64_t a_gstride;
  int64_t w_gstride;
  int32_t shift_by_group;
  int32_t layout;
  int32_t ldw;
  int32_t pad_ldw_;
} DnGemmTerm;

enum { DN_LAYOUT_A_KBLOCKED = 1, DN_LAYOUT_W_KBLOCKED = 2, DN_LAYOUT_OUT_KBLOCKED = 1 };

typedef struct {
  DnGemmTerm terms[DN_MAX_TERMS];
  int32_t n_terms;
  int32_t dtype;
  int32_t M, N, K;
  int32_t T;
  int32_t groups;
  int32_t epilogue;
  const float* bias;
  int64_t bias_gstride;
  void* out;
  int32_t ldo;
  int32_t out_dtype;
  int64_t out_gstride;
  const void* res;
  int32_t ldr;
  int32_t res_dtype;
  int64_t res_gstride;
  const float* gamma_beta;
  int32_t gb_ld;
  int32_t gb_half;
  int64_t gb_gstride;
  const float* pos_table;
  int32_t pos_ld;
  int32_t flags;
  const int32_t* lengths;
  void* norm_out;
  int32_t norm_ld, norm_dtype, norm_D, norm_gb_ld;
  const float* norm_gamma;
  const float* norm_gb;
  int32_t norm_gb_half;
  int32_t out_layout;
  int32_t norm_split, norm_ssq_ld;
  float* norm_ssq;
  const float* row_ssq;
  int32_t row_ssq_ld, row_ssq_parts;
  float row_D;
  int32_t row_bias_ld;
  const float* row_bias;
  void* pre_out;
  int32_t pre_ld, pre_pad_;
} DnGemmParams;

enum {
  DN_GEMM_NARROW_STORES = 1 << 4,
  DN_GEMM_NO_RES_PREFETCH = 1 << 5,
  DN_GEMM_RELU = 1 << 6,
  DN_GEMM_TWIN = 1 << 7,
  DN_GEMM_TAG_SHIFT = 8,
  DN_GEMM_TILE_SHIFT = 16,
  DN_GEMM_FAT_STAMPS = 1 << 20,
  DN_GEMM_NO_SHARED_ROWS = 1 << 21,
  DN_GEMM_TAPS_INNER = 1 << 22,
  DN_GEMM_TERM_OUTER = 1 << 23,
  DN_GEMM_BAND_SHIFT = 24
};

enum {
  DN_TILE_128X128 = 1,
  DN_TILE_256X128 = 2,
  DN_TILE_256X256 = 3,
  DN_TILE_256X352 = 4,
  DN_TILE_ROW = 5,
  DN_TILE_256X256_W4 = 6,
  DN_TILE_256X256_W8 = 7,
  DN_TILE_256X192 = 8,
  DN_TILE_256X128_2WG = 9
};

int dn_conv_gemm(const DnGemmParams* p, void* stream);

typedef struct {
  int32_t tile;
  int32_t taps_inner;
  int32_t shared_rows;
  int32_t band;
} DnGemmRoute;
int dn_conv_gemm_route(const DnGemmParams* p, DnGemmRoute* route);
int dn_conv_gemm_kblocked_ok(const DnGemmParams* p);
int dn_conv_gemm_tile(const DnGemmParams* p);

enum { DN_TAG_FFN_CONV = 1, DN_TAG_WN_DILATED = 2,
       DN_TAG_FFN_CONV_WGRAD = 3  };

int dn_profile_start(int32_t tag, int32_t max_launches);
int dn_profile_stop(float* avg_ms, int32_t* n_launches);

typedef struct {
  const void* q; const void* k; const void* v; void* out;
  int32_t ldq, ldk, ldv, ldo;
  int32_t B, T, heads, dim_head;
  int32_t dtype;
  int32_t Tk;
  const int32_t* lengths;
  float scale;
  int32_t pad2_;
  float* lse;
  float dropout_p;
  uint32_t seed_lo, seed_hi;
  int32_t pad3_;
} DnAttnParams;

int dn_attention(const DnAttnParams* p, void* stream);

int dn_rmsnorm(const float* x, int32_t ldx, void* y, int32_t ldy, int32_t out_dtype, int32_t M, int32_t D,
               int32_t T, const float* gamma, const float* gamma_beta, int32_t gb_ld, int32_t gb_half,
               void* stream);

int dn_time_cond(const int32_t* times, int32_t B, const float* w_freq, int32_t half, const float* W,
                 const float* bias, int32_t C, float* out, void* out_act, int32_t act_dtype, int32_t ldo,
                 void* stream);

int dn_ddim_step(const float* x, const float* eps, float* x_out, void* x_act, int32_t act_dtype,
                 int32_t ld_act, int32_t M, int32_t C, int32_t ld, int32_t T, const float* coef,
                 const int32_t* t, void* stream);

int dn_q_sample(const float* x, const float* noise, float* out, void* out_act, int32_t act_dtype,
                int32_t ld_act, int32_t M, int32_t C, int32_t ld, int32_t T, const float* coef_a,
                const float* coef_b, const int32_t* t, void* stream);

#define DN_GD_COLS 12
typedef struct {
  const float* x; const float* model_out; const float* noise;
  float* sample; float* pred_xstart;
  const int32_t* t;
  const float* table;
  int32_t N, inner, learned_range, clip_denoised, sampler;
  float eta;
  int32_t predict_xstart;
  const float* cond_grad;
} DnGaussianStep;
int dn_gaussian_step(const DnGaussianStep* p, void* stream);

typedef struct {
  const float* x; const float* model_out; const float* x_start;
  const int32_t* t; const float* table;
  float *mean, *variance, *log_variance, *pred_xstart, *vb, *reverse_sample;
  int32_t N, inner, learned_range, clip_denoised;
  int32_t predict_xstart;
} DnGaussianMoments;
int dn_gaussian_moments(const DnGaussianMoments* p, void* stream);

int dn_posterior_sample(const float* params, int32_t ldp, const float* noise, int32_t ldn, float* z,
                        void* z_act, int32_t act_dtype, int32_t ldz, int32_t M, int32_t Z, int32_t T,
                        const int32_t* lengths, float* kl_rows, void* stream);

int dn_argmax_units(const float* logits, int32_t ld, int32_t M, int32_t V, int32_t offset, int32_t* units,
                    void* stream);

int dn_randn(float* out, int64_t n, uint64_t seed, uint64_t offset, void* stream);
// ... 27 lines not shown
int dn_adam_step_ema(float* param, const float* grad, float* exp_avg, float* exp_avg_sq, int64_t n, const DnAdamParams* hp,
                     const float* sumsq, void* param_bf16, float* ema, double ema_decay, void* stream);
int dn_ema_update(float* ema, const float* param, int64_t n, double decay, void* stream);


typedef struct {
  const void *q, *k, *v, *out, *dout;
  void *dq, *dk, *dv;
  int32_t ldq, ldk, ldv, ldo, lddo, lddq, lddk, lddv;
  int32_t B, T, heads, dim_head;
  int32_t dtype;
  int32_t pad_;
  const int32_t* lengths;
  float scale;
  int32_t pad2_;
  const float* lse;
  float* delta;
  float dropout_p;
  uint32_t seed_lo, seed_hi;
  int32_t pad3_;
} DnAttnBwdParams;
int dn_attention_backward(const DnAttnBwdParams* p, void* stream);

int dn_time_cond_backward(const int32_t* times, int32_t B, const float* w_freq, int32_t half, const float* W, const float* bias, int32_t C,
                          const float* dcond, int32_t ldd, float* ds_scratch, float* dw_freq, float* dW, float* dbias, void* stream);

int dn_gate_forward(const void* h, const void* res, void* out, int32_t dtype, int32_t M, int32_t ld, int32_t T,
                    const float* gamma_beta, int32_t gb_ld, int32_t gb_half, void* stream);
int dn_gate_backward(const void* dout, const void* h, void* dh, int32_t dtype, int32_t M, int32_t ld, int32_t T,
                     const float* gamma_beta, int32_t gb_ld, int32_t gb_half, float* dgb_rows, int32_t dgb_ld, void* stream);

int dn_geglu_forward(const void* pre, void* out, int32_t dtype, int32_t M, int32_t ip, void* stream);
int dn_geglu_backward(const void* dout, const void* pre, void* dpre, int32_t dtype, int32_t M, int32_t ip, void* stream);

size_t dn_rmsnorm_backward_scratch_bytes(int32_t B, int32_t T, int32_t D);
int dn_rmsnorm_backward(const float* x, int32_t ldx, const void* dy, int32_t lddy, int32_t dy_dtype, int32_t B, int32_t T, int32_t D,
                        const float* gamma, const float* gamma_beta, int32_t gb_ld, int32_t gb_half, const float* dres, float* dx,
                        void* dx_act, int32_t act_dtype, int32_t ld_act, float* dgamma, float* dgamma_beta, int32_t dgb_ld,
                        float* scratch, void* stream);

size_t dn_colsum_scratch_bytes(int32_t groups, int32_t rows_per_group, int32_t C);
int dn_colsum(const void* src, int32_t ld, int32_t dtype, int32_t groups, int32_t rows_per_group, int32_t C, float* out,
              int32_t out_ld, float scale, int32_t accumulate, float* scratch, void* stream);

int dn_posterior_backward(const float* params, int32_t ldp, const float* noise, int32_t ldn, const float* dz, int32_t lddz,
                          void* dparams, int32_t act_dtype, int32_t ldo, int32_t M, int32_t Z, int32_t T, const int32_t* lengths,
                          float kl_weight, void* stream);

int dn_lsce_loss_grad(const float* logits, int32_t ld, const int32_t* target, int32_t M, int32_t V, float epsilon, float grad_scale,
                      float* rows, void* dlogits, int32_t act_dtype, int32_t ldd, void* stream);

int dn_masked_mse_grad(const float* pred, int32_t ldp, const float* target, int32_t ldt, int32_t M, int32_t C, int32_t T,
                       const int32_t* lengths, float grad_scale, float* sq_rows, float* dpred, int32_t ldd, int32_t accumulate,
                       void* dpred_act, int32_t act_dtype, int32_t ld_act, void* stream);

int dn_vec_sum(const float* v, int64_t n, float* out, int32_t accumulate, float* scratch, void* stream);

int dn_sum_groups(const void* src, int64_t stride, int32_t count, void* dst, int32_t dtype, int64_t n, void* stream);
size_t dn_rows_times_weight_scratch_bytes(int32_t B, int32_t N, int32_t C);
int dn_rows_times_weight(const float* X, int32_t ldx, int32_t B, const float* W, int32_t ldw, int32_t N, int32_t C, float* out,
                         float* scratch, void* stream);

int dn_transpose_weights(const void* src, int32_t dtype, int32_t count, int64_t src_stride, int32_t R, int32_t Cc, void* dst,
                         int64_t dst_stride, int32_t Rp, int32_t Cp, void* stream);

int dn_split_rows(const float* src, int64_t n, void* dst, int32_t weight_order, void* stream);

enum { DN_REPACK_CONVERT = 0, DN_REPACK_KBLOCK = 1, DN_REPACK_COPY = 2, DN_REPACK_SUM = 3 };
typedef struct {
  int64_t src;
  void* dst;
  int32_t kind;
  int32_t mats;
  int32_t rows, K;
  int32_t count;
  int32_t pad_;
  int64_t stride;
} DnRepackDesc;
int dn_repack_weights(const float* master, const DnRepackDesc* descs, int32_t n, int32_t dtype, void* stream);

int dn_ffn_fold(const float* conv_W, const float* conv_b, const float* out_W, const float* out_b, int64_t conv_W_stride,
                int64_t conv_b_stride, int64_t out_W_stride, int64_t out_b_stride, int32_t depth, int32_t dim, int32_t inner,
                int32_t dtype, void* fold_W, float* fold_b, void* stream);

int dn_transpose_slices(const void* src, int32_t dtype, int32_t ld, int32_t B, int32_t T, int32_t C, int32_t front, int32_t Tp,
                        int64_t cols_total, int32_t chunk, void* dst, int32_t rows, int32_t rows_total, int32_t row0, int32_t weight_order,
                        void* stream);

int dn_wgrad_reduce(const float* part, int32_t slices, int32_t cout, int32_t n_total, int32_t rows_w, int32_t n_taps, float* grad,
                    int32_t Np, int32_t Kp, void* stream);

int dn_add_broadcast(const float* src, float* dst, int32_t C, int32_t ld, int32_t count, void* stream);

int dn_conv_weight_grad_tn(const void* dy, int32_t lddy, int32_t cout, const void* const* x, const int32_t* ldx, const int32_t* shift,
                           int32_t n_taps, int32_t cin, int32_t B, int32_t T, int32_t slices, float* part, float* grad, void* stream);

int dn_conv_weight_grad_tn_x3(const void* dy, int32_t lddy, int32_t cout, const void* const* x, const int32_t* ldx, const int32_t* shift,
                              int32_t n_taps, int32_t cin, int32_t B, int32_t T, int32_t slices, float* part, float* grad, void* stream);

int dn_transpose_pad_f32(const float* src, int32_t ld, int32_t B, int32_t T, int32_t C, int32_t front, int32_t Tp, float* dst,
                         int32_t rows, int32_t rows_total, int32_t row0, int32_t chunk, void* stream);


typedef struct {
  int32_t dim, latent, depth, heads, dim_head, wn_layers, wn_stacks, cond_mult;
  int32_t dtype;
  int32_t max_pos;
  int32_t dim_prompt, num_latents, resampler_depth;
} DnEpsConfig;

typedef struct {
  int32_t dim, z, depth, heads, dim_head, stacks, layers, vocab;
  int32_t n_mults; int32_t mults[4];
  int32_t dtype;
} DnVaeConfig;

typedef struct DnEps DnEps;
typedef struct DnVae DnVae;

int dn_eps_create(const DnEpsConfig* cfg, const void* const* weights, int32_t n_weights, DnEps** out);
void dn_eps_destroy(DnEps* m);
size_t dn_eps_workspace_bytes(const DnEps* m, int32_t B, int32_t T);
int dn_eps_forward(DnEps* m, const float* x, const int32_t* t, const int32_t* lengths, int32_t B, int32_t T,
                   int32_t shared_t, float* eps_out, void* workspace, size_t workspace_bytes, void* stream);

size_t dn_eps_cond_workspace_bytes(const DnEps* m, int32_t B, int32_t T, int32_t Tp);
int dn_eps_forward_cond(DnEps* m, const float* x, const int32_t* t, const int32_t* lengths, const float* prompt,
                        const int32_t* prompt_lengths, const int32_t* drop, int32_t B, int32_t T, int32_t Tp, float* eps_out,
                        void* workspace, size_t workspace_bytes, void* stream);
#define DN_COND_REUSE_PROMPT 1
int dn_eps_forward_cond_ex(DnEps* m, const float* x, const int32_t* t, const int32_t* lengths, const float* prompt,
                           const int32_t* prompt_lengths, const int32_t* drop, int32_t B, int32_t T, int32_t Tp, float* eps_out,
                           void* workspace, size_t workspace_bytes, int32_t flags, const float* time_table, int32_t table_t0,
                           int32_t table_n, void* stream);
size_t dn_eps_cond_time_table_workspace_bytes(const DnEps* m, int32_t n_t);
int dn_eps_cond_time_table(DnEps* m, int32_t t0, int32_t n_t, float* table, void* workspace, size_t workspace_bytes, void* stream);
int dn_eps_cond_time_table_steps(DnEps* m, const int32_t* steps, int32_t n_steps, float* table, void* workspace, size_t workspace_bytes,
                                 void* stream);

int dn_eps_weights_changed(DnEps* m);
int dn_eps_set_ffn_fold(DnEps* m, const void* fold_W, const float* fold_b);

int dn_vae_create(const DnVaeConfig* cfg, const void* const* weights, int32_t n_weights, DnVae** out);
void dn_vae_destroy(DnVae* m);
int dn_vae_set_ffn_fold(DnVae* m, const void* fold_W, const float* fold_b);
size_t dn_vae_workspace_bytes(const DnVae* m, int32_t B, int32_t T);
int dn_vae_encode_params(DnVae* m, const float* feat, int32_t B, int32_t T, float* params, void* workspace,
                         size_t workspace_bytes, void* stream);
int dn_vae_decode(DnVae* m, const float* latent, const int32_t* lengths, int32_t B, int32_t T, float* recon,
                  float* logits, int32_t* units, void* workspace, size_t workspace_bytes, void* stream);

enum { DN_LOOP_GRAPH = 1,
       DN_LOOP_SPLIT2 = 2,
       DN_LOOP_KEEP_TABLE = 4  };
size_t dn_ddim_workspace_bytes(const DnEps* m, int32_t B, int32_t T, int32_t start_step);
int dn_ddim_loop(DnEps* m, float* x, const int32_t* lengths, int32_t B, int32_t T, int32_t start_step,
                 int32_t max_evals, const float* coef, int32_t timesteps, int32_t flags, void* workspace,
                 size_t workspace_bytes, void* stream);

int dn_ddpm_loop(DnEps* m, float* x, const int32_t* lengths, int32_t B, int32_t T, int32_t start_step, int32_t max_evals,
                 const float* table, int32_t timesteps, int32_t clip_denoised, uint64_t seed, const float* noise, int32_t flags,
                 void* workspace, size_t workspace_bytes, void* stream);

int dn_ddpm_loop_keyed(DnEps* m, float* x, const int32_t* lengths, int32_t B, int32_t T, int32_t start_step, int32_t max_evals,
                       const float* table, int32_t timesteps, int32_t clip_denoised, const uint64_t* keys, int32_t flags,
                       void* workspace, size_t workspace_bytes, void* stream);

#define DN_DDIM_SCHED_COLS 5
size_t dn_ddim_sched_workspace_bytes(const DnEps* m, int32_t B, int32_t T, int32_t n_steps);
int dn_ddim_sched_check(const int32_t* steps_host, int32_t n_steps, int32_t timesteps);
int dn_ddim_sched_loop(DnEps* m, float* x, const int32_t* lengths, int32_t B, int32_t T, const int32_t* steps, const float* coef,
                       int32_t n_steps, int32_t timesteps, int32_t eta_on, uint64_t seed, const float* noise, int32_t flags,
                       void* workspace, size_t workspace_bytes, void* stream);

int dn_ddim_sched_loop_keyed(DnEps* m, float* x, const int32_t* lengths, int32_t B, int32_t T, const int32_t* steps, const float* coef,
                             int32_t n_steps, int32_t timesteps, const uint64_t* keys, int32_t flags, void* workspace,
                             size_t workspace_bytes, void* stream);
int dn_ddim_sched_step(float* x, const float* eps, int64_t n, const float* coef, const int32_t* steps, const int32_t* step_index,
                       int32_t eta_on, uint64_t seed, const float* noise, void* stream);
int dn_ddim_sched_step_keyed(float* x, const float* eps, const uint64_t* keys, int32_t B, int32_t T, int32_t Z, const float* coef,
                             const int32_t* steps, const int32_t* step_index, void* stream);

#define DN_DPM_COLS 6
int dn_dpm2m_step(float* x, const float* eps, float* hist, int64_t n, const float* coef, const int32_t* step_index, void* stream);
size_t dn_dpm_workspace_bytes(const DnEps* m, int32_t B, int32_t T, int32_t n_steps);
int dn_dpm_loop(DnEps* m, float* x, const int32_t* lengths, int32_t B, int32_t T, const int32_t* steps, const float* coef, int32_t n_steps,
                int32_t timesteps, int32_t flags, void* workspace, size_t workspace_bytes, void* stream);

size_t dn_gaussian_workspace_bytes(const DnEps* m, int32_t B, int32_t T, int32_t n_steps);
int dn_gaussian_loop(DnEps* m, float* x, const int32_t* lengths, int32_t B, int32_t T, const int32_t* steps, const float* table,
                     int32_t n_steps, int32_t timesteps, int32_t sampler, int32_t clip_denoised, float eta, uint64_t seed,
                     const float* noise, int32_t flags, void* workspace, size_t workspace_bytes, void* stream);
int dn_gaussian_loop_keyed(DnEps* m, float* x, const int32_t* lengths, int32_t B, int32_t T, const int32_t* steps, const float* table,
                           int32_t n_steps, int32_t timesteps, int32_t sampler, int32_t clip_denoised, float eta, const uint64_t* keys,
                           int32_t flags, void* workspace, size_t workspace_bytes, void* stream);
int dn_gaussian_sched_step(float* x, const float* eps, int64_t n, const float* table, const int32_t* step_index, int32_t n_steps,
                           int32_t sampler, int32_t clip_denoised, float eta, uint64_t seed, const float* noise, void* stream);
int dn_gaussian_sched_step_keyed(float* x, const float* eps, const uint64_t* keys, int32_t B, int32_t T, int32_t Z, const float* table,
                                 const int32_t* steps, const int32_t* step_index, int32_t n_steps, int32_t sampler, int32_t clip_denoised,
                                 float eta, void* stream);

size_t dn_guided_ddim_workspace_bytes(const DnEps* m, int32_t B, int32_t T, int32_t Tp, int32_t n_steps, int32_t guided);
int dn_guided_ddim_loop(DnEps* m, float* x, const int32_t* lengths, const float* prompt, const int32_t* prompt_lengths, int32_t B, int32_t T,
                        int32_t Tp, float cond_scale, const int32_t* steps, const float* coef, int32_t n_steps, int32_t timesteps,
                        int32_t eta_on, uint64_t seed, const float* noise, int32_t flags, void* workspace, size_t workspace_bytes,
                        void* stream);

int dn_guided_ddim_loop_keyed(DnEps* m, float* x, const int32_t* lengths, const float* prompt, const int32_t* prompt_lengths, int32_t B,
                              int32_t T, int32_t Tp, float cond_scale, const int32_t* steps, const float* coef, int32_t n_steps,
                              int32_t timesteps, const uint64_t* keys, int32_t flags, void* workspace, size_t workspace_bytes,
                              void* stream);

size_t dn_guided_dpm_workspace_bytes(const DnEps* m, int32_t B, int32_t T, int32_t Tp, int32_t n_steps, int32_t guided);
int dn_guided_dpm_loop(DnEps* m, float* x, const int32_t* lengths, const float* prompt, const int32_t* prompt_lengths, int32_t B, int32_t T,
                       int32_t Tp, float cond_scale, const int32_t* steps, const float* coef, int32_t n_steps, int32_t timesteps,
                       int32_t flags, void* workspace, size_t workspace_bytes, void* stream);

typedef struct DnVaeTrain DnVaeTrain;
typedef struct {
  const float* feat;
  const int32_t* units;
  const int32_t* lengths;
  const float* noise;
  int32_t B, T;
  int32_t ntokens;
  float w_lsce, w_mse, w_kl;
  float label_smoothing;
  float loss_scale;
// ... 230 lines not shown
```

Before: 230.9 denoising-steps/s.

## Add shared-row 256x128 tile for folded FFN conv GEMM with K-blocked weights

Adds a 256x128 shared-row, tap-inner variant of the big conv GEMM kernel, which stages one weight row per wave, and routes the folded FFN conv (residual-add epilogue) to it. The route applies when the problem is fp16/bf16, Dp is at most 512 and there are enough tiles; this becomes the new fp16 default. When the tile is selected, the fold step also writes a K-blocked copy of the folded weights, and the GEGLU GEMM writes its output K-blocked, so both operands load in the blocked layout. The goal is better reuse of A rows across the three taps and better occupancy for narrow N, at the cost of extra weight memory and a new kernel path.

```diff
diff --git a/diffnorm_amd/_lib.py b/diffnorm_amd/_lib.py
--- a/diffnorm_amd/_lib.py
+++ b/diffnorm_amd/_lib.py
@@ -12,7 +12,7 @@
 GEMM_TAG_SHIFT, GEMM_TILE_SHIFT, GEMM_BAND_SHIFT = 8, 16, 24
 GEMM_FAT_STAMPS, GEMM_NO_SHARED_ROWS, GEMM_TAPS_INNER, GEMM_TERM_OUTER = 1 << 20, 1 << 21, 1 << 22, 1 << 23
 (TILE_128X128, TILE_256X128, TILE_256X256, TILE_256X352, TILE_ROW, TILE_256X256_W4, TILE_256X256_W8, TILE_256X192,
- TILE_256X128_2WG) = range(1, 10)
+ TILE_256X128_2WG, TILE_256X128_SR) = range(1, 11)
 
 
 class DiffNormHipError(RuntimeError):
@@ -236,8 +236,11 @@
     "dn_transpose_slices": (C.c_int, [_vp, _i32, _i32, _i32, _i32, _i32, _i32, _i32, _i64, _i32, _vp, _i32, _i32, _i32, _i32, _vp]),
     "dn_repack_weights": (C.c_int, [_vp, _vp, _i32, _i32, _vp]),
     "dn_ffn_fold": (C.c_int, [_vp, _vp, _vp, _vp, C.c_int64, C.c_int64, C.c_int64, C.c_int64, _i32, _i32, _i32, _i32, _vp, _vp, _vp]),
+    "dn_ffn_fold_kblocked": (C.c_int, [_vp, _vp, _vp, _vp, C.c_int64, C.c_int64, C.c_int64, C.c_int64, _i32, _i32, _i32, _i32, _vp, _vp, _vp, _vp]),
     "dn_eps_set_ffn_fold": (C.c_int, [_vp, _vp, _vp]),
     "dn_vae_set_ffn_fold": (C.c_int, [_vp, _vp, _vp]),
+    "dn_eps_set_ffn_fold_kblocked": (C.c_int, [_vp, _vp]),
+    "dn_vae_set_ffn_fold_kblocked": (C.c_int, [_vp, _vp]),
     "dn_wgrad_reduce": (C.c_int, [_vp, _i32, _i32, _i32, _i32, _i32, _vp, _i32, _i32, _vp]),
     "dn_conv_weight_grad_tn": (C.c_int, [_vp, _i32, _i32, _vp, _vp, _vp, _i32, _i32, _i32, _i32, _i32, _vp, _vp, _vp]),
     "dn_conv_weight_grad_tn_x3": (C.c_int, [_vp, _i32, _i32, _vp, _vp, _vp, _i32, _i32, _i32, _i32, _i32, _vp, _vp, _vp]),
diff --git a/diffnorm_amd/csrc/engine.h b/diffnorm_amd/csrc/engine.h
--- a/diffnorm_amd/csrc/engine.h
+++ b/diffnorm_amd/csrc/engine.h
@@ -63,6 +63,7 @@
   const void *qkv_W, *out_W, *ffin_W, *ffconv_W, *ffout_W, *pred_W, *ffconv_Wkb, *ffin_Wkb, *qkv_Wkb;
   const float *ffin_b, *ffconv_b, *ffout_b, *g1, *g2, *pred_gamma;
   const void* fold_W;
+  const void* fold_Wkb;
   const float* fold_b;
   int fold_default;
 };
diff --git a/diffnorm_amd/csrc/engine.hip b/diffnorm_amd/csrc/engine.hip
--- a/diffnorm_amd/csrc/engine.hip
+++ b/diffnorm_amd/csrc/engine.hip
@@ -120,7 +120,16 @@
 struct TfBufs { void *xn, *qkv, *ao, *gg, *fc; float* ssq; };
 inline int ssq_ld(int Dp) { const int n = Dp / 64; return n <= 8 ? 8 : (n + 3) / 4 * 4; }
 
+enum { FOLD_OFF = 0, FOLD_TABLE = 1, FOLD_256X128 = 2, FOLD_256X256 = 3, FOLD_SR = 4, FOLD_ROUTED = 5 };
 inline int ffn_fold_mode(const TransformerW& w) { return w.fold_W && w.fold_b ? option_or(OPT_FFN_FOLD, w.fold_default) : 0; }
+
+constexpr bool kFoldSrRouted = true;
+inline bool fold_route(int dtype, int M, int Dp, int ip, int32_t gemm_flags) {
+  if (!kFoldSrRouted || !dn::dn_is16(dtype) || Dp > 512 || 3L * ip < 1024) return false;
+  if (option_or(OPT_TAPS_INNER, 1) == 2) return true;
+  const long twin = (gemm_flags & DN_GEMM_TWIN) ? 2 : 1;
+  return (long)((M + 255) / 256) * ((Dp + 127) / 128) * twin >= 256;
+}
 
 TfBufs plan_tf(const TransformerW& w, int M, int es, Arena& ar) {
   const int hd = w.heads * w.dim_head;
@@ -192,6 +201,27 @@
     qkv_kb = kblock_mode() == 1 || qt == DN_TILE_256X256 || qt == DN_TILE_256X128_2WG;
   }
   const int fold = ffn_fold_mode(w);
+  int fold_tile = fold == FOLD_256X128 ? DN_TILE_256X128 : fold == FOLD_256X256 ? DN_TILE_256X256 : fold == FOLD_SR ? DN_TILE_256X128_SR : 0;
+  if (fold == FOLD_ROUTED && fold_route(dtype, M, Dp, ip, gemm_flags)) fold_tile = DN_TILE_256X128_SR;
+  auto fold_params = [&](int l) {
+    DnGemmParams p = gemm_base(dtype, M, Dp, ip, T, gemm_flags);
+    p.n_terms = 3;
+    for (int j = 0; j < 3; ++j) {
+      p.terms[j].A = tb.gg; p.terms[j].lda = ip; p.terms[j].shift = 2 - j;
+      p.terms[j].W = eoff(w.fold_W, ((size_t)l * 3 + j) * Dn * ip, es);
+    }
+    p.bias = w.fold_b + (size_t)l * Dp;
+    p.flags |= DN_TAG_FFN_CONV << DN_GEMM_TAG_SHIFT;
+    if (fold_tile && !fuse) p.flags |= fold_tile << DN_GEMM_TILE_SHIFT;
+    return p;
+  };
+  bool fold_kb = false;
+  if (fold && fold_tile == DN_TILE_256X128_SR && !fuse && w.fold_Wkb && kblock_mode() != 0 && dn::dn_is16(dtype)) {
+    DnGemmParams q = fold_params(0);
+    q.epilogue = DN_EPI_RESADD;
+    if (split) { q.norm_out = tb.xn; q.norm_split = 1; }
+    fold_kb = dn_conv_gemm_tile(&q) == DN_TILE_256X128_SR;
+  }
   const bool qkv_192 = option_or(OPT_QKV_192, 0) != 0 && dn::dn_is16(dtype) && (3 * hd) % 192 == 0 && M >= 2048;
   for (int l = 0; l < w.depth; ++l) {
     {
@@ -277,19 +307,16 @@
         p.bias = w.ffin_b + (size_t)l * 2 * ip;
         p.epilogue = DN_EPI_GEGLU; p.out = tb.gg; p.ldo = ip;
         if (mid2 & 2) p.flags |= DN_TILE_256X128_2WG << DN_GEMM_TILE_SHIFT;
+        p.out_layout = fold_kb ? DN_LAYOUT_OUT_KBLOCKED : 0;
         if (scaled) set_row_scale(p, tb, Dp, D, rb ? rb + (size_t)l * rb_layer + 3 * hd + (cx ? hd : 0) : nullptr, rb_ld);
         DN_TRY(dn_conv_gemm(&p, s));
       }
-      DnGemmParams p = gemm_base(dtype, M, Dp, ip, T, gemm_flags);
-      p.n_terms = 3;
-      for (int j = 0; j < 3; ++j) {
-        p.terms[j].A = tb.gg; p.terms[j].lda = ip; p.terms[j].shift = 2 - j;
-        p.terms[j].W = eoff(w.fold_W, ((size_t)l * 3 + j) * Dn * ip, es);
-      }
-      p.bias = w.fold_b + (size_t)l * Dp;
-      p.flags |= DN_TAG_FFN_CONV << DN_GEMM_TAG_SHIFT;
-      const int fold_tile = fold == 2 ? DN_TILE_256X128 : fold == 3 ? DN_TILE_256X256 : 0;
-      if (fold_tile && !fuse) p.flags |= fold_tile << DN_GEMM_TILE_SHIFT;
+      DnGemmParams p = fold_params(l);
+      if (fold_kb)
+        for (int j = 0; j < 3; ++j) {
+          p.terms[j].W = eoff(w.fold_Wkb, ((size_t)l * 3 + j) * Dn * ip, es);
+          p.terms[j].layout = DN_LAYOUT_A_KBLOCKED | DN_LAYOUT_W_KBLOCKED;
+        }
       DN_TRY(close_residual(p));
     } else {
     DnGemmParams pc = gemm_base(dtype, M, ip, ip, T, gemm_flags);
@@ -440,13 +467,24 @@
 extern "C" int dn_eps_set_ffn_fold(DnEps* m, const void* fold_W, const float* fold_b) {
   DN_CHECK_ARG(m && (fold_W != nullptr) == (fold_b != nullptr), "dn_eps_set_ffn_fold: null engine, or one of the two buffers without the other");
   DN_CHECK_ARG(((uintptr_t)fold_W & 127) == 0 && ((uintptr_t)fold_b & 15) == 0, "dn_eps_set_ffn_fold: fold_W 128-byte, fold_b 16-byte aligned");
-  m->tf.fold_W = fold_W; m->tf.fold_b = fold_b;
-  m->tf.fold_default = m->cfg.dtype == DN_BF16 ? 0 : 1;
+  m->tf.fold_W = fold_W; m->tf.fold_b = fold_b; m->tf.fold_Wkb = nullptr;
+  m->tf.fold_default = m->cfg.dtype == DN_BF16 ? FOLD_OFF : FOLD_ROUTED;
   for (StepGraph* g : {&m->loop_graph, &m->guided_graph}) {
     if (g->exec) (void)hipGraphExecDestroy((hipGraphExec_t)g->exec);
     g->exec = nullptr;
   }
   m->table_ws = nullptr;
+  return DN_OK;
+}
+
+extern "C" int dn_eps_set_ffn_fold_kblocked(DnEps* m, const void* fold_Wkb) {
+  DN_CHECK_ARG(m && (!fold_Wkb || (m->tf.fold_W && dn::dn_is16(m->cfg.dtype))) && ((uintptr_t)fold_Wkb & 127) == 0,
+               "dn_eps_set_ffn_fold_kblocked: null engine, no folded weights attached, not a 2-byte arithmetic, or fold_Wkb not 128-byte aligned");
+  m->tf.fold_Wkb = fold_Wkb;
+  for (StepGraph* g : {&m->loop_graph, &m->guided_graph}) {
+    if (g->exec) (void)hipGraphExecDestroy((hipGraphExec_t)g->exec);
+    g->exec = nullptr;
+  }
   return DN_OK;
 }
 
@@ -1480,8 +1518,15 @@
 extern "C" int dn_vae_set_ffn_fold(DnVae* m, const void* fold_W, const float* fold_b) {
   DN_CHECK_ARG(m && (fold_W != nullptr) == (fold_b != nullptr), "dn_vae_set_ffn_fold: null engine, or one of the two buffers without the other");
   DN_CHECK_ARG(((uintptr_t)fold_W & 127) == 0 && ((uintptr_t)fold_b & 15) == 0, "dn_vae_set_ffn_fold: fold_W 128-byte, fold_b 16-byte aligned");
-  m->tf.fold_W = fold_W; m->tf.fold_b = fold_b;
-  m->tf.fold_default = m->cfg.dtype == DN_BF16 ? 0 : 1;
+  m->tf.fold_W = fold_W; m->tf.fold_b = fold_b; m->tf.fold_Wkb = nullptr;
+  m->tf.fold_default = m->cfg.dtype == DN_BF16 ? FOLD_OFF : FOLD_ROUTED;
+  return DN_OK;
+}
+
+extern "C" int dn_vae_set_ffn_fold_kblocked(DnVae* m, const void* fold_Wkb) {
+  DN_CHECK_ARG(m && (!fold_Wkb || (m->tf.fold_W && dn::dn_is16(m->cfg.dtype))) && ((uintptr_t)fold_Wkb & 127) == 0,
+               "dn_vae_set_ffn_fold_kblocked: null engine, no folded weights attached, not a 2-byte arithmetic, or fold_Wkb not 128-byte aligned");
+  m->tf.fold_Wkb = fold_Wkb;
   return DN_OK;
 }
 
diff --git a/diffnorm_amd/csrc/gemm_kernels.h b/diffnorm_amd/csrc/gemm_kernels.h
--- a/diffnorm_amd/csrc/gemm_kernels.h
+++ b/diffnorm_amd/csrc/gemm_kernels.h
@@ -715,16 +715,17 @@
 
 template <typename E, int EPI, bool TAPS, int BNB = 256, bool HALO = false>
 __global__ __launch_bounds__(512, 1) void conv_gemm_big_kernel(const DnGemmParams p) {
-  static_assert(!HALO || (TAPS && BNB == 256 && !std::is_same<E, BF16X3>::value), "shared staging: tap-inner order on the 256 x 256 tile");
+  static_assert(!HALO || (TAPS && (BNB == 256 || BNB == 128) && !std::is_same<E, BF16X3>::value), "shared staging: tap-inner order on the 256 x 256 and 256 x 128 tiles");
   extern __shared__ __attribute__((aligned(16))) char smem[];
   if constexpr (std::is_same<E, F16>::value) f16_saturate();
   constexpr int ES = Elem<E>::bytes;
   constexpr int KT = ROWB2 / ES;
-  static_assert(BNB == 256 || BNB == 192, "tile width");
+  static_assert(BNB == 256 || BNB == 192 || BNB == 128, "tile width");
   constexpr int BMB = 256, STAGES = 4;
   constexpr int TILE = BNB * ROWB2;
   constexpr int STAGE_BYTES = TILE + 256 * ROWB2;
-  constexpr int PER_STAGE = 4;
+  constexpr int WPW = BNB == 128 ? 1 : 2;
+  constexpr int PER_STAGE = WPW + 2;
   constexpr int PER_LATE = BNB == 256 ? 4 : 3;
   constexpr int NTW = BNB / 32;
 
@@ -756,7 +757,7 @@
     m = m < p.M ? m : p.M - 1;
     a_row[i] = m;
     a_t[i] = m % p.T;
-    int n = n0 + (BNB == 256 || wave < 4 ? wave * 32 + i * 16 : 128 + (wave - 4) * 16) + srow;
+    int n = n0 + (BNB == 128 ? wave * 16 : BNB == 256 || wave < 4 ? wave * 32 + i * 16 : 128 + (wave - 4) * 16) + srow;
     w_row[i] = n < w_rows ? n : w_rows - 1;
   }
   const int ktiles_per_term = p.K / KT;
@@ -827,8 +828,8 @@
   };
   const uint32_t lds_base = __builtin_amdgcn_readfirstlane((uint32_t)(uintptr_t)(lptr_t)smem);
   auto stage = [&](int slot) {
-    const bool one_w = BNB != 256 && wave >= 4;
-    const uint32_t wbase = lds_base + slot * STAGE_BYTES + (one_w ? 8192 + (wave - 4) * 1024 : wave * 2048);
+    const bool one_w = BNB == 128 || (BNB != 256 && wave >= 4);
+    const uint32_t wbase = lds_base + slot * STAGE_BYTES + (BNB == 128 ? wave * 1024 : one_w ? 8192 + (wave - 4) * 1024 : wave * 2048);
     const uint32_t abase = lds_base + slot * STAGE_BYTES + TILE + wave * 2048;
     if constexpr (TAPS) {
 #pragma unroll
@@ -924,13 +925,13 @@
 #pragma unroll
       for (int t = 0; t < 3; ++t) {
 #pragma unroll
-        for (int i = 0; i < 2; ++i) glds16(w_ptr[i] + tap_woff, lds_base + t * TILE + wave * 2048 + i * 1024);
+        for (int i = 0; i < WPW; ++i) glds16(w_ptr[i] + tap_woff, lds_base + t * TILE + wave * (WPW * 1024) + i * 1024);
         tap_woff += tap_wstride;
       }
       tap_woff = 0;
 #pragma unroll
-      for (int i = 0; i < 2; ++i) w_ptr[i] += w_inc;
-      pipe_sync<4>();
+      for (int i = 0; i < WPW; ++i) w_ptr[i] += w_inc;
+      pipe_sync<2 * WPW>();
     }
   }
   if (!shared_rows) {
@@ -999,13 +1000,13 @@
       for (int i = 0; i < 4; ++i) af[i] = *reinterpret_cast<const uint4*>(sa + i * 16 * ROWB2);
     }
     if constexpr (STAGE) {
-      const uint32_t wbase = lds_base + fill * TILE + wave * 2048;
-#pragma unroll
-      for (int i = 0; i < 2; ++i) glds16(w_ptr[i] + tap_woff, wbase + i * 1024);
+      const uint32_t wbase = lds_base + fill * TILE + wave * (WPW * 1024);
+#pragma unroll
+      for (int i = 0; i < WPW; ++i) glds16(w_ptr[i] + tap_woff, wbase + i * 1024);
       if constexpr (TAP == 2) {
         tap_woff = 0;
 #pragma unroll
-        for (int i = 0; i < 2; ++i) w_ptr[i] += w_inc;
+        for (int i = 0; i < WPW; ++i) w_ptr[i] += w_inc;
       } else {
         tap_woff += tap_wstride;
       }
@@ -1038,9 +1039,9 @@
     auto adv = [&]() { slot = slot == STAGES - 1 ? 0 : slot + 1; fill = fill == STAGES - 1 ? 0 : fill + 1; };
     const int chunks = ktiles_per_term;
     for (int c = 0; c + 1 < chunks; ++c) {
-      ktile_h(late_c, T0{}, std::true_type{}, integral_constant<int, 6>{}, slot, fill, aslot); adv();
-      ktile_h(late_c, T1{}, std::true_type{}, integral_constant<int, 7>{}, slot, fill, aslot); adv();
-      ktile_h(late_c, T2{}, std::true_type{}, integral_constant<int, 2>{}, slot, fill, aslot); adv();
+      ktile_h(late_c, T0{}, std::true_type{}, integral_constant<int, 2 * WPW + 2>{}, slot, fill, aslot); adv();
+      ktile_h(late_c, T1{}, std::true_type{}, integral_constant<int, 2 * WPW + 3>{}, slot, fill, aslot); adv();
+      ktile_h(late_c, T2{}, std::true_type{}, integral_constant<int, WPW>{}, slot, fill, aslot); adv();
       aslot ^= 1;
     }
     ktile_h(late_c, T0{}, std::false_type{}, integral_constant<int, 3>{}, slot, fill, aslot); adv();
@@ -1069,7 +1070,7 @@
     asm volatile("s_waitcnt lgkmcnt(0)" ::: "memory");
   };
   half(std::integral_constant<int, 0>{});
-  half(std::integral_constant<int, 1>{});
+  if constexpr (NTW > 4) half(std::integral_constant<int, 1>{});
 }
 
 constexpr int BNM = 128;
@@ -1995,6 +1996,10 @@
   return tiles_fat >= 100 && 1.3 * fill(tiles_fat) >= fill(tiles_big);
 }
 
+static inline bool sr_tile_ok(const DnGemmParams& p, bool taps) {
+  return dn_is16(p.dtype) && p.epilogue == DN_EPI_RESADD && !(p.norm_out && !p.norm_split) && taps && big_taps_share_rows(p, 32);
+}
+
 static inline int choose_tile(const DnGemmParams& p, int force, bool taps) {
   const bool bf = dn_is16(p.dtype);
   if ((p.epilogue == DN_EPI_RESADD || p.epilogue == DN_EPI_POSEMB) && p.norm_out && !p.norm_split && p.dtype != DN_BF16X3) return DN_TILE_ROW;
@@ -2026,6 +2031,7 @@
     return sm > ss ? DN_TILE_256X128 : DN_TILE_128X128;
   }
   if (routes_to_352(p, force)) return DN_TILE_256X352;
+  if (force == DN_TILE_256X128_SR && sr_tile_ok(p, taps)) return DN_TILE_256X128_SR;
   const bool taps_route_by_shape = option_or(OPT_TAPS_INNER, 1) == 2;
   if (force == 0 && (p.epilogue == DN_EPI_BIAS || p.epilogue == DN_EPI_FILM_GATE) && taps_route_by_shape && taps) return DN_TILE_256X256;
   bool kblocked = false;
@@ -2095,11 +2101,12 @@
   const bool conv_epi = p.epilogue == DN_EPI_BIAS || p.epilogue == DN_EPI_FILM_GATE;
   const bool big = r.tile == DN_TILE_256X256 && conv_epi && p.dtype != DN_BF16X3;
   const bool fat = r.tile == DN_TILE_256X352 || r.tile == DN_TILE_256X256_W4 || r.tile == DN_TILE_256X256_W8;
-  r.taps_inner = taps && (big || fat);
-  r.shared_rows = r.taps_inner && (big ? big_taps_share_rows(p, ROWB2 / (dn_is16(p.dtype) ? 2 : 4))
-                                       : r.tile == DN_TILE_256X352 && p.epilogue == DN_EPI_BIAS && taps_share_rows(p));
+  const bool sr = r.tile == DN_TILE_256X128_SR;
+  r.taps_inner = taps && (big || fat || sr);
+  r.shared_rows = r.taps_inner && (sr || (big ? big_taps_share_rows(p, ROWB2 / (dn_is16(p.dtype) ? 2 : 4))
+                                              : r.tile == DN_TILE_256X352 && p.epilogue == DN_EPI_BIAS && taps_share_rows(p)));
   const int forced_band = (p.flags >> DN_GEMM_BAND_SHIFT) & 0xff;
-  const bool banded = (r.tile >= DN_TILE_128X128 && r.tile <= DN_TILE_256X256) || r.tile == DN_TILE_256X128_2WG;
+  const bool banded = (r.tile >= DN_TILE_128X128 && r.tile <= DN_TILE_256X256) || r.tile == DN_TILE_256X128_2WG || sr;
   r.band = banded && forced_band == 0 ? choose_band(p, r.tile) : forced_band;
   return r;
 }
@@ -2140,6 +2147,14 @@
     if (r.taps_inner) return launch_kernel<conv_gemm_big_kernel<E, EPI, true>>(p, grid, 512, lds, s);
   }
   return launch_kernel<conv_gemm_big_kernel<E, EPI, false, BNB>>(p, grid, 512, lds, s);
+}
+
+template <typename E, int EPI>
+static int launch_sr(const DnGemmParams& p, hipStream_t s) {
+  constexpr int ring = 4 * 128 * ROWB2 + 2 * (256 + 128) * ROWB2, unshared = 4 * (128 + 256) * ROWB2, slabs = 8 * 64 * EP_LD * 4;
+  constexpr int lds = slabs > ring && slabs > unshared ? slabs : ring > unshared ? ring : unshared;
+  const dim3 grid(((p.M + 255) / 256) * ((p.N + 127) / 128), p.groups);
+  return launch_kernel<conv_gemm_big_kernel<E, EPI, true, 128, true>>(p, grid, 512, lds, s);
 }
 
 template <typename E, int EPI>
@@ -2196,6 +2211,9 @@
     case DN_TILE_256X128_2WG:
       if constexpr (half && EPI != DN_EPI_RESADD && EPI != DN_EPI_POSEMB) return launch_mid2<E, EPI>(p, s);
       break;
+    case DN_TILE_256X128_SR:
+      if constexpr (half && EPI == DN_EPI_RESADD) return launch_sr<E, EPI>(p, s);
+      break;
     case DN_TILE_256X256_W4:
       if constexpr (std::is_same<E, BF16>::value) return launch_fat<E, EPI, 8>(p, r, s);
       break;
diff --git a/diffnorm_amd/csrc/repack.hip b/diffnorm_amd/csrc/repack.hip
--- a/diffnorm_amd/csrc/repack.hip
+++ b/diffnorm_amd/csrc/repack.hip
@@ -80,6 +80,7 @@
   int64_t conv_W_ls, conv_b_ls, out_W_ls, out_b_ls;
   int dim, inner, ip, in_n, Dp, Dn;
   void* W;
+  void* Wkb;
   float* b;
 };
 
@@ -111,6 +112,9 @@
 #pragma unroll
     for (int i = 0; i < 8; ++i) v[i] = (n0 + r < a.dim && c + i < a.inner) ? acc[r][i] : 0.f;
     store8<DT>(a.W, (((int64_t)blockIdx.z * a.Dn) + n0 + r) * a.ip + c, make_float4(v[0], v[1], v[2], v[3]), make_float4(v[4], v[5], v[6], v[7]));
+    if constexpr (DT == DN_BF16 || DT == DN_F16) {
+      if (a.Wkb) store8<DT>(a.Wkb, ((((int64_t)blockIdx.z * (a.ip / 32)) + (c >> 5)) * a.Dn + n0 + r) * 32 + (c & 31), make_float4(v[0], v[1], v[2], v[3]), make_float4(v[4], v[5], v[6], v[7]));
+    }
   }
 }
 
@@ -148,16 +152,25 @@
 extern "C" int dn_ffn_fold(const float* conv_W, const float* conv_b, const float* out_W, const float* out_b, int64_t conv_W_stride,
                            int64_t conv_b_stride, int64_t out_W_stride, int64_t out_b_stride, int32_t depth, int32_t dim, int32_t inner,
                            int32_t dtype, void* fold_W, float* fold_b, void* stream) {
+  return dn_ffn_fold_kblocked(conv_W, conv_b, out_W, out_b, conv_W_stride, conv_b_stride, out_W_stride, out_b_stride, depth, dim, inner, dtype,
+                              fold_W, fold_b, nullptr, stream);
+}
+
+extern "C" int dn_ffn_fold_kblocked(const float* conv_W, const float* conv_b, const float* out_W, const float* out_b, int64_t conv_W_stride,
+                                    int64_t conv_b_stride, int64_t out_W_stride, int64_t out_b_stride, int32_t depth, int32_t dim,
+                                    int32_t inner, int32_t dtype, void* fold_W, float* fold_b, void* fold_Wkb, void* stream) {
   DN_CHECK_ARG(conv_W && conv_b && out_W && out_b && fold_W && fold_b, "dn_ffn_fold: null argument");
   DN_CHECK_ARG(depth >= 1 && 3 * depth <= 65535 && dim >= 1 && inner >= 1, "dn_ffn_fold: depth=%d dim=%d inner=%d", depth, dim, inner);
   DN_CHECK_ARG(dtype == DN_F32 || dtype == DN_BF16 || dtype == DN_BF16X3 || dtype == DN_F16, "dn_ffn_fold: dtype=%d", dtype);
   DN_CHECK_ARG((conv_W_stride | out_W_stride) % 4 == 0 && (((uintptr_t)conv_W | (uintptr_t)out_W) & 15) == 0 && ((uintptr_t)fold_W & 127) == 0,
                "dn_ffn_fold: the weight sources must be 16-byte aligned (strides multiples of 4), the folded weights 128-byte aligned");
+  DN_CHECK_ARG(!fold_Wkb || ((dtype == DN_BF16 || dtype == DN_F16) && ((uintptr_t)fold_Wkb & 127) == 0),
+               "dn_ffn_fold_kblocked: the K-blocked copy is for DN_BF16 / DN_F16 (dtype=%d), 128-byte aligned", dtype);
   dn::FoldArgs a;
   a.conv_W = conv_W; a.conv_b = conv_b; a.out_W = out_W; a.out_b = out_b;
   a.conv_W_ls = conv_W_stride; a.conv_b_ls = conv_b_stride; a.out_W_ls = out_W_stride; a.out_b_ls = out_b_stride;
   a.dim = dim; a.inner = inner; a.ip = (inner + 63) / 64 * 64; a.in_n = (inner + 127) / 128 * 128; a.Dp = (dim + 63) / 64 * 64; a.Dn = (dim + 127) / 128 * 128;
-  a.W = fold_W; a.b = fold_b;
+  a.W = fold_W; a.b = fold_b; a.Wkb = fold_Wkb;
   const dim3 grid((a.ip / 8 + 63) / 64, a.Dn / 4, 3 * depth), block(64);
   hipStream_t s = (hipStream_t)stream;
   if (dtype == DN_F32) hipLaunchKernelGGL(dn::ffn_fold_w_kernel<DN_F32>, grid, block, 0, s, a);
diff --git a/diffnorm_amd/engine.py b/diffnorm_amd/engine.py
--- a/diffnorm_amd/engine.py
+++ b/diffnorm_amd/engine.py
@@ -130,8 +130,12 @@
 
     fold_W: Optional[torch.Tensor] = None
     fold_b: Optional[torch.Tensor] = None
+    fold_Wkb: Optional[torch.Tensor] = None
 
     def _tf_dims(self):
+        raise NotImplementedError
+
+    def _attach_kblocked(self):
         raise NotImplementedError
 
     def _fold_call(self, srcs, strides, depth, layer0):
@@ -139,8 +143,9 @@
         inner = int(dim * 4 * 2 / 3)
         (_, _), b_shape = packing.ffn_fold_storage(dim, 1, self.dtype)
         w_off = layer0 * self.fold_W[0].numel() * self.fold_W.element_size()
-        _lib.check(self.lib.dn_ffn_fold(*srcs, *strides, depth, dim, inner, self.dtype, self.fold_W.data_ptr() + w_off,
-                                        self.fold_b.data_ptr() + layer0 * b_shape[1] * 4, _lib.current_stream()), "dn_ffn_fold")
+        kb = None if self.fold_Wkb is None else self.fold_Wkb.data_ptr() + w_off
+        _lib.check(self.lib.dn_ffn_fold_kblocked(*srcs, *strides, depth, dim, inner, self.dtype, self.fold_W.data_ptr() + w_off,
+                                                 self.fold_b.data_ptr() + layer0 * b_shape[1] * 4, kb, _lib.current_stream()), "dn_ffn_fold")
 
     def _fold_from_state_dict(self, tf_layers, sd):
         dim, depth, attach = self._tf_dims()
@@ -148,10 +153,14 @@
         with torch.cuda.device(self.device):
             self.fold_W = torch.empty(w_shape, dtype=w_dtype, device=self.device)
             self.fold_b = torch.empty(b_shape, dtype=torch.float32, device=self.device)
+            if self.dtype in (_lib.DN_BF16, _lib.DN_F16):
+                self.fold_Wkb = torch.empty((w_shape[0], 3, w_shape[3] // 32, w_shape[2], 32), dtype=w_dtype, device=self.device)
             for l, layer in enumerate(tf_layers):
                 srcs = [t.to(self.device) for t in packing.ffn_fold_sources(layer, sd)]
                 self._fold_call([t.data_ptr() for t in srcs], (0, 0, 0, 0), 1, l)
         _lib.check(attach(self.handle, self.fold_W.data_ptr(), self.fold_b.data_ptr()), "set_ffn_fold")
+        if self.fold_Wkb is not None:
+            _lib.check(self._attach_kblocked()(self.handle, self.fold_Wkb.data_ptr()), "set_ffn_fold_kblocked")
 
     def _fold_from_flat(self, train_engine, master):
         if self.fold_W is None:
@@ -162,7 +171,7 @@
             self._fold_call([master.data_ptr() + 4 * o for o in offs], strides, depth, 0)
 
     def fold_bytes(self) -> int:
-        return 0 if self.fold_W is None else sum(t.numel() * t.element_size() for t in (self.fold_W, self.fold_b))
+        return 0 if self.fold_W is None else sum(t.numel() * t.element_size() for t in (self.fold_W, self.fold_b, self.fold_Wkb) if t is not None)
 
     def refresh_bytes(self) -> int:
         return 0 if self._repack is None else self._repack[3]
@@ -185,6 +194,9 @@
 
     def _tf_dims(self):
         return self.cfg.dim, self.cfg.depth, self.lib.dn_eps_set_ffn_fold
+
+    def _attach_kblocked(self):
+        return self.lib.dn_eps_set_ffn_fold_kblocked
 
     def __del__(self):
         if getattr(self, "handle", None) and self.handle.value:
@@ -531,6 +543,9 @@
     def _tf_dims(self):
         return self._tf[0], self._tf[1], self.lib.dn_vae_set_ffn_fold
 
+    def _attach_kblocked(self):
+        return self.lib.dn_vae_set_ffn_fold_kblocked
+
     def __del__(self):
         if getattr(self, "handle", None) and self.handle.value:
             self.lib.dn_vae_destroy(self.handle)
diff --git a/include/diffnorm_hip.h b/include/diffnorm_hip.h
--- a/include/diffnorm_hip.h
+++ b/include/diffnorm_hip.h
@@ -110,7 +110,8 @@
   DN_TILE_256X256_W4 = 6,
   DN_TILE_256X256_W8 = 7,
   DN_TILE_256X192 = 8,
-  DN_TILE_256X128_2WG = 9
+  DN_TILE_256X128_2WG = 9,
+  DN_TILE_256X128_SR = 10
 };
 
 int dn_conv_gemm(const DnGemmParams* p, void* stream);
@@ -304,6 +305,9 @@
 int dn_ffn_fold(const float* conv_W, const float* conv_b, const float* out_W, const float* out_b, int64_t conv_W_stride,
                 int64_t conv_b_stride, int64_t out_W_stride, int64_t out_b_stride, int32_t depth, int32_t dim, int32_t inner,
                 int32_t dtype, void* fold_W, float* fold_b, void* stream);
+int dn_ffn_fold_kblocked(const float* conv_W, const float* conv_b, const float* out_W, const float* out_b, int64_t conv_W_stride,
+                         int64_t conv_b_stride, int64_t out_W_stride, int64_t out_b_stride, int32_t depth, int32_t dim, int32_t inner,
+                         int32_t dtype, void* fold_W, float* fold_b, void* fold_Wkb, void* stream);
 
 int dn_transpose_slices(const void* src, int32_t dtype, int32_t ld, int32_t B, int32_t T, int32_t C, int32_t front, int32_t Tp,
                         int64_t cols_total, int32_t chunk, void* dst, int32_t rows, int32_t rows_total, int32_t row0, int32_t weight_order,
@@ -362,10 +366,12 @@
 
 int dn_eps_weights_changed(DnEps* m);
 int dn_eps_set_ffn_fold(DnEps* m, const void* fold_W, const float* fold_b);
+int dn_eps_set_ffn_fold_kblocked(DnEps* m, const void* fold_Wkb);
 
 int dn_vae_create(const DnVaeConfig* cfg, const void* const* weights, int32_t n_weights, DnVae** out);
 void dn_vae_destroy(DnVae* m);
 int dn_vae_set_ffn_fold(DnVae* m, const void* fold_W, const float* fold_b);
+int dn_vae_set_ffn_fold_kblocked(DnVae* m, const void* fold_Wkb);
 size_t dn_vae_workspace_bytes(const DnVae* m, int32_t B, int32_t T);
 int dn_vae_encode_params(DnVae* m, const float* feat, int32_t B, int32_t T, float* params, void* workspace,
                          size_t workspace_bytes, void* stream);
```

Measured after the change: 238.8 denoising-steps/s, median of 6. 1.03x the previous value.
